# DallinClark/RealTimeRaytracer

Hardware: AMD Instinct MI355X
Metric: Mrays/sec at 1920x1080 1spp (all rays: primary + shadow) (higher is better)
Workload: dtype f32

## Files before the change

### realtimeraytracer_amd/csrc/kernels/rtr_device.h

```cpp
#pragma once
#include <hip/hip_runtime.h>
#include <stdint.h>
#include "../../../include/rtr_types.h"
#include "../../../include/rtr_math.h"

namespace rtrdev {

struct DeviceTexture { const uint8_t* pixels; uint32_t width, height, channels, _pad; };

constexpr uint32_t kLightTriRecord = 4;

struct DeviceScene {
    const uint4* nodes;
    const RtrBvhGrid* grid;
    const uint4* nodes4;
    uint32_t numNodes4;
    const float4* tris;
    const RtrVertex* vertices;
    const uint32_t* indices;
    const RtrObjectInfo* objects;
    const RtrAreaLightInfo* lights;
    const float4* lightTris;
    const uint32_t* lightTriFirst;
    const float* xforms;
// ... 243 lines not shown
                        if (ALPHA && (__float_as_uint(q2.w) & 1u) && !alpha_pass<STATS>(sc, cu, pr, u, v, st)) continue;
                        bool take;
                        if (FLAT_TAKE) {
                            const bool idLess = (cu < best.custom) | ((cu == best.custom) & (pr < best.prim));
                            take = !found | (t < best.t) | ((t == best.t) & idLess);
                        } else if (!found) take = true;
                        else take = t < best.t || (t == best.t && (cu < best.custom || (cu == best.custom && pr < best.prim)));
                        if (take) {
                            found = true; best.t = t; best.u = u; best.v = v; best.custom = cu; best.prim = pr; best.leaf = cur;
                            limit = t;
                            if (ANY) return true;
                        }
                    }
                }
            }
        }
        if (sp == 0) break;
        --sp; cur = stack[sp * BLOCK];
    }
    if (LIMIT > 0 && over) { best.custom = RTR_STACK_OVERFLOW; best.prim = RTR_MISS; best.t = tmax; best.u = 0.f; best.v = 0.f; best.leaf = 0; return false; }
    return found;
}

#define RTR_PI_F 3.14159265359f
__device__ __forceinline__ float chiGGX(float v) { return v > 0.0f ? 1.0f : 0.0f; }
__device__ __forceinline__ float GGX_Distribution(rtr_v3 n, rtr_v3 h, float alpha) {
    const float NoH = rtr_dot(n, h);
    const float alpha2 = alpha * alpha;
    const float NoH2 = NoH * NoH;
    const float den = rtr_max(rtr_fma(NoH2, alpha2, 1.0f - NoH2), 0.001f);
    return (chiGGX(NoH) * alpha2) / (RTR_PI_F * den * den);
}
__device__ __forceinline__ float GGX_PartialGeometryTerm(rtr_v3 v, rtr_v3 n, rtr_v3 h, float alpha) {
    float VoH2 = rtr_clamp(rtr_dot(v, h), 0.001f, 1.0f);
    const float chi = chiGGX(VoH2 / rtr_clamp(rtr_dot(v, n), 0.001f, 1.0f));
    VoH2 = VoH2 * VoH2;
    const float tan2 = (1.0f - VoH2) / VoH2;
    return (chi * 2.0f) / (1.0f + rtr_sqrt(rtr_fma(alpha * alpha, tan2, 1.0f)));
}
__device__ __forceinline__ rtr_v3 Fresnel_Schlick(float cosT, rtr_v3 F0) {
    const float p = rtr_pow(1.0f - cosT, 5.0f);
    return rtr_mk(rtr_fma(1.0f - F0.x, p, F0.x), rtr_fma(1.0f - F0.y, p, F0.y), rtr_fma(1.0f - F0.z, p, F0.z));
}

#define RTR_LUT_SIZE 64.0f
#define RTR_LUT_SCALE ((RTR_LUT_SIZE - 1.0f) / RTR_LUT_SIZE)
#define RTR_LUT_BIAS (0.5f / RTR_LUT_SIZE)

__device__ __forceinline__ float4 sample_lut(const float* __restrict__ lut, float u, float v) {
    float x = rtr_fma(u, RTR_LUT_SIZE, -0.5f), y = rtr_fma(v, RTR_LUT_SIZE, -0.5f);
    if (!(x >= -1.0e6f && x <= 1.0e6f)) x = 0.0f;
    if (!(y >= -1.0e6f && y <= 1.0e6f)) y = 0.0f;
    const float x0f = __builtin_floorf(x), y0f = __builtin_floorf(y);
    const float fx = x - x0f, fy = y - y0f;
    const int x0 = ((int)x0f) & 63, y0 = ((int)y0f) & 63;
    const int x1 = (x0 + 1) & 63, y1 = (y0 + 1) & 63;
    const float4 t00 = *reinterpret_cast<const float4*>(lut + (y0 * 64 + x0) * 4);
    const float4 t10 = *reinterpret_cast<const float4*>(lut + (y0 * 64 + x1) * 4);
    const float4 t01 = *reinterpret_cast<const float4*>(lut + (y1 * 64 + x0) * 4);
    const float4 t11 = *reinterpret_cast<const float4*>(lut + (y1 * 64 + x1) * 4);
    float4 r;
    { const float a = rtr_fma(t10.x - t00.x, fx, t00.x), b = rtr_fma(t11.x - t01.x, fx, t01.x); r.x = rtr_fma(b - a, fy, a); }
    { const float a = rtr_fma(t10.y - t00.y, fx, t00.y), b = rtr_fma(t11.y - t01.y, fx, t01.y); r.y = rtr_fma(b - a, fy, a); }
    { const float a = rtr_fma(t10.z - t00.z, fx, t00.z), b = rtr_fma(t11.z - t01.z, fx, t01.z); r.z = rtr_fma(b - a, fy, a); }
    { const float a = rtr_fma(t10.w - t00.w, fx, t00.w), b = rtr_fma(t11.w - t01.w, fx, t01.w); r.w = rtr_fma(b - a, fy, a); }
    return r;
}

__device__ __forceinline__ rtr_v3 IntegrateEdgeVec(rtr_v3 v1, rtr_v3 v2) {
    const float x = rtr_dot(v1, v2);
    const float y = rtr_abs(x);
    const float a = rtr_fma(rtr_fma(0.0145206f, y, 0.4965155f), y, 0.8543985f);
    const float b = rtr_fma(4.1616724f + y, y, 3.4175940f);
    const float v = a / b;
    const float theta_sintheta = (x > 0.0f) ? v : 0.5f * (1.0f / rtr_sqrt(rtr_max(rtr_fma(-x, x, 1.0f), 1e-7f))) - v;
    return rtr_scale(rtr_cross(v1, v2), theta_sintheta);
}

__device__ __forceinline__ float LTC_Evaluate(rtr_v3 N, rtr_v3 V, rtr_v3 P, bool identity, float4 t1,
                                              const rtr_v3* points, rtr_v3 lightNormal, bool twoSided,
                                              const float* __restrict__ ltc2) {
    const rtr_v3 T1 = rtr_normalize(rtr_sub(V, rtr_scale(N, rtr_dot(V, N))));
    const rtr_v3 T2 = rtr_cross(N, T1);
    rtr_v3 L[3];
#pragma unroll
    for (int k = 0; k < 3; ++k) {
        const rtr_v3 w = rtr_sub(points[k], P);
        const rtr_v3 q = rtr_mk(rtr_dot(T1, w), rtr_dot(T2, w), rtr_dot(N, w));
        rtr_v3 l;
        if (identity) l = q;
        else l = rtr_mk(rtr_fma(t1.z, q.z, t1.x * q.x), q.y, rtr_fma(t1.w, q.z, t1.y * q.x));
        L[k] = rtr_normalize(l);
    }
    const rtr_v3 dir = rtr_sub(points[0], P);
    const bool behind = rtr_dot(dir, lightNormal) < 0.0f;
    rtr_v3 vsum = IntegrateEdgeVec(L[0], L[1]);
    vsum = rtr_add(vsum, IntegrateEdgeVec(L[1], L[2]));
    vsum = rtr_add(vsum, IntegrateEdgeVec(L[2], L[0]));
    const float len = rtr_length(vsum);
    float z = vsum.z / len;
    if (behind) z = -z;
    const float uvx = rtr_fma(rtr_fma(z, 0.5f, 0.5f), RTR_LUT_SCALE, RTR_LUT_BIAS);
    const float uvy = rtr_fma(len, RTR_LUT_SCALE, RTR_LUT_BIAS);
    const float4 tex = sample_lut(ltc2, uvx, uvy);
    float sum = len * tex.w;
    if (!behind && !twoSided) sum = 0.0f;
    return sum;
}

struct RenderArgs {
    RtrCameraData cam;
    RtrSceneInfo info;
    uint32_t width, height;
    uint32_t spp, numShadowRays;
    uint32_t bandRows, shardIndex, shardCount;
    uint32_t localRows;
    uint32_t tilesPerRow;
    uint32_t maxRaysPerSample;
    uint32_t images;
    uint32_t accumulate, accumulatedFrames;
    uint32_t directRows;
};

__device__ __forceinline__ bool pixel_of(const RenderArgs& ra, uint32_t q, uint32_t& x, uint32_t& lrow, uint32_t& gy) {
    const uint32_t lane = q & 63u, tile = q >> 6;
    const uint32_t tx = tile % ra.tilesPerRow, band8 = tile / ra.tilesPerRow;
    x = tx * 8u + (lane & 7u);
    lrow = band8 * 8u + (lane >> 3);
    const uint32_t lb = lrow / ra.bandRows, r = lrow % ra.bandRows;
    gy = (lb * ra.shardCount + ra.shardIndex) * ra.bandRows + r;
    return x < ra.width && lrow < ra.localRows && gy < ra.height;
}

__device__ __forceinline__ size_t out_index(const RenderArgs& ra, uint32_t px, uint32_t lrow, uint32_t gy) {
    return (size_t)(ra.directRows ? gy : lrow) * ra.width + px;
}

__device__ __forceinline__ rtr_v3 primary_dir(const RenderArgs& ra, uint32_t px, uint32_t py, uint32_t i) {
    const float jx = rtr_random(px + i), jy = rtr_random(px + i * 322u);
    const float offx = ((float)px + jx) - 0.5f, offy = ((float)py + jy) - 0.5f;
    const rtr_v3 pw = rtr_madd(rtr_madd(rtr_ld3(ra.cam.topLeftViewportCorner), rtr_ld3(ra.cam.horizontalViewportDelta), offx),
                               rtr_ld3(ra.cam.verticalViewportDelta), offy);
    return rtr_normalize(rtr_sub(pw, rtr_ld3(ra.cam.position)));
}

struct Accum { rtr_v3 analytic, shadowed, unshadowed, avgNormal, avgPosition; };

struct Surface {
    rtr_v3 hitPoint, hitNormal, viewDir, color, mDiffuse, mSpecular;
    float roughness, metallic, om;
    float4 t1, t2;
};

template <bool SHADE, bool STATS>
__device__ __forceinline__ bool fetch_surface(const DeviceScene& sc, const RenderArgs& ra, const HitRec& h, rtr_v3 rayDir,
                                              bool wantAnalytic, Accum& o, Surface& sf, LocalStats& st) {
    if (h.custom == RTR_MISS) {
        if (SHADE) {
            rtr_v3 sky = rtr_ld3(sc.skyLinear);
            if (sc.hdri.pixels) {
                const rtr_v3 dir = rtr_normalize(rayDir);
                const float hu = rtr_atan2(dir.z, dir.x) / (2.0f * 3.14159265f) + 0.5f;
                float hv = rtr_acos(rtr_clamp(dir.y, -1.0f, 1.0f)) / 3.14159265f;
                hv = 1.0f - hv;
                const float4 tx = sample_tex<STATS>(sc.hdri, hu, hv, st);
                sky = rtr_mk(rtr_to_linear(tx.x), rtr_to_linear(tx.y), rtr_to_linear(tx.z));
            }
            o.analytic = rtr_add(o.analytic, sky); o.unshadowed = rtr_add(o.unshadowed, sky); o.shadowed = rtr_add(o.shadowed, sky);
        }
        return false;
    }
    if (h.custom < sc.numLights) {
        if (SHADE) {
            const rtr_v3 lc = rtr_ld3(sc.lights[h.custom].color);
            o.analytic = rtr_add(o.analytic, lc); o.unshadowed = rtr_add(o.unshadowed, lc); o.shadowed = rtr_add(o.shadowed, lc);
        }
        return false;
    }
    const rtr_v3 camPos = rtr_ld3(ra.cam.position);
    if (STATS) st.hits++;
    const RtrObjectInfo* oi = sc.objects + (h.custom - sc.numLights);
    const uint32_t vOff = oi->vertexOffset, iOff = oi->indexOffset;
    const uint32_t i0 = sc.indices[3u * h.prim + 0u + iOff];
    const uint32_t i1 = sc.indices[3u * h.prim + 1u + iOff];
    const uint32_t i2 = sc.indices[3u * h.prim + 2u + iOff];
    const float4* va = reinterpret_cast<const float4*>(sc.vertices + (i0 + vOff));
    const float4* vb = reinterpret_cast<const float4*>(sc.vertices + (i1 + vOff));
    const float4* vc = reinterpret_cast<const float4*>(sc.vertices + (i2 + vOff));
    const rtr_v3 p0 = f4xyz(va[0]), p1 = f4xyz(vb[0]), p2 = f4xyz(vc[0]);
    const rtr_v3 n0 = f4xyz(va[1]), n1 = f4xyz(vb[1]), n2 = f4xyz(vc[1]);
    const float b0 = 1.0f - h.u - h.v, b1 = h.u, b2 = h.v;
    const rtr_v3 localPos = rtr_madd(rtr_madd(rtr_scale(p0, b0), p1, b1), p2, b2);
    const rtr_v3 hitPoint = rtr_xform_point34(sc.xforms + 12u * h.custom, localPos);
    const rtr_v3 nsum = rtr_madd(rtr_madd(rtr_scale(n0, b0), n1, b1), n2, b2);
    const float* nm = sc.nmats + 12u * h.custom;
    rtr_v3 hitNormal;
    if (rtr_dot(nsum, nsum) > 0.0f) {
        hitNormal = rtr_normalize(rtr_mul33(nm, rtr_normalize(nsum)));
    } else {
        const rtr_v3 g = rtr_cross(rtr_sub(p1, p0), rtr_sub(p2, p0));
        rtr_v3 n = rtr_normalize(rtr_mul33(nm, rtr_normalize(g)));
        if (rtr_dot(n, rayDir) > 0.0f) n = rtr_neg(n);
        hitNormal = n;
    }
    float metallic = oi->metallic;
    float rough = oi->specular;
    rtr_v3 color = rtr_mk(0, 0, 0);
    if (SHADE) {
        rtr_v3 col = rtr_ld3(oi->color);
        if (oi->usesColorMap | oi->usesSpecularMap | oi->usesMetallicMap) {
            const float4 ta = va[2], tb = vb[2], tc = vc[2];
            const float uu = rtr_fma(tc.x, b2, rtr_fma(tb.x, b1, ta.x * b0));
            const float vv = rtr_fma(tc.y, b2, rtr_fma(tb.y, b1, ta.y * b0));
            if (oi->usesColorMap != 0u) { const float4 t = sample_tex<STATS>(sc.textures[oi->colorIndex], uu, vv, st); col = rtr_mk(t.x, t.y, t.z); }
            if (oi->usesSpecularMap != 0u) rough = sample_tex<STATS>(sc.textures[oi->specularIndex], uu, vv, st).x;
            if (oi->usesMetallicMap != 0u) metallic = sample_tex<STATS>(sc.textures[oi->metallicIndex], uu, vv, st).x;
        }
        color = rtr_mk(rtr_to_linear(col.x), rtr_to_linear(col.y), rtr_to_linear(col.z));
    }
    const float roughness = 1.0f - rough;

    const rtr_v3 viewDir = rtr_normalize(rtr_sub(camPos, hitPoint));
    const float om = 1.0f - metallic;
    rtr_v3 mDiffuse = rtr_mk(0, 0, 0), mSpecular = rtr_mk(0, 0, 0);
    float4 t1 = make_float4(1, 0, 0, 1), t2 = make_float4(0, 0, 0, 0);
    if (SHADE) {
        o.avgNormal = rtr_add(o.avgNormal, hitNormal);
        o.avgPosition = rtr_add(o.avgPosition, hitPoint);
        mDiffuse = rtr_scale(color, om);
        mSpecular = rtr_mk(rtr_fma(color.x, metallic, 0.04f * om), rtr_fma(color.y, metallic, 0.04f * om),
                           rtr_fma(color.z, metallic, 0.04f * om));
        if (wantAnalytic) {
            const float dotNV = rtr_clamp(rtr_dot(hitNormal, viewDir), 0.0f, 1.0f);
            const float lu = rtr_fma(roughness, RTR_LUT_SCALE, RTR_LUT_BIAS);
            const float lv = rtr_fma(rtr_sqrt(1.0f - dotNV), RTR_LUT_SCALE, RTR_LUT_BIAS);
            t1 = sample_lut(sc.ltc1, lu, lv);
            t2 = sample_lut(sc.ltc2, lu, lv);
        }
    }
    sf.hitPoint = hitPoint; sf.hitNormal = hitNormal; sf.viewDir = viewDir; sf.color = color;
    sf.mDiffuse = mDiffuse; sf.mSpecular = mSpecular; sf.roughness = roughness; sf.metallic = metallic; sf.om = om;
    sf.t1 = t1; sf.t2 = t2;
    return true;
}

__device__ __forceinline__ rtr_v3 surface_diffuse(float om, rtr_v3 color) {
    return rtr_mk((om * color.x) / RTR_PI_F, (om * color.y) / RTR_PI_F, (om * color.z) / RTR_PI_F);
}
__device__ __forceinline__ rtr_v3 area_sample_contrib(rtr_v3 hitNormal, rtr_v3 viewDir, float roughness, rtr_v3 mSpecular, rtr_v3 currDiffuse,
                                                      rtr_v3 lcol, float lintensity, float pdf, rtr_v3 sampledLightDir, float lightDistance) {
    const rtr_v3 halfVector = rtr_normalize(rtr_add(viewDir, sampledLightDir));
    const float cosTheta = rtr_clamp(rtr_dot(viewDir, halfVector), 0.0f, 1.0f);
    const float Dg = GGX_Distribution(hitNormal, halfVector, roughness);
    const float G = GGX_PartialGeometryTerm(viewDir, hitNormal, halfVector, roughness) *
                    GGX_PartialGeometryTerm(sampledLightDir, hitNormal, halfVector, roughness);
    const rtr_v3 F = Fresnel_Schlick(cosTheta, mSpecular);
    const float NdotV = rtr_max(rtr_dot(hitNormal, viewDir), 0.1f);
    const float NdotL = rtr_max(rtr_dot(hitNormal, sampledLightDir), 0.1f);
    const float den = 4.0f * NdotV * NdotL;
    const rtr_v3 currSpecular = rtr_mk(((Dg * F.x) * G) / den, ((Dg * F.y) * G) / den, ((Dg * F.z) * G) / den);
    const float attenuation = 1.0f / (lightDistance * lightDistance);
    const rtr_v3 BRDF = rtr_add(currSpecular, currDiffuse);
    const rtr_v3 Lr = rtr_mk((((lcol.x * lintensity) * NdotL) * attenuation) * 10.0f, (((lcol.y * lintensity) * NdotL) * attenuation) * 10.0f,
                             (((lcol.z * lintensity) * NdotL) * attenuation) * 10.0f);
    return rtr_mk((BRDF.x * Lr.x) / pdf, (BRDF.y * Lr.y) / pdf, (BRDF.z * Lr.z) / pdf);
}
__device__ __forceinline__ rtr_v3 directional_light_dir() { return rtr_normalize(rtr_mk(-1.0f, 1.0f, -0.5f)); }
__device__ __forceinline__ rtr_v3 directional_contrib(rtr_v3 hitNormal, rtr_v3 viewDir, float roughness, rtr_v3 mSpecular, rtr_v3 currDiffuse) {
    const rtr_v3 directLightDir = directional_light_dir();
    const rtr_v3 directLightColor = rtr_mk(1.0f, 1.0f, 0.5f);
    const float directLightIntensity = 0.2f;
    const rtr_v3 halfVector = rtr_normalize(rtr_add(viewDir, directLightDir));
    const float cosTheta = rtr_clamp(rtr_dot(viewDir, halfVector), 0.0f, 1.0f);
    const float Dg = GGX_Distribution(hitNormal, halfVector, roughness);
    const float G = GGX_PartialGeometryTerm(viewDir, hitNormal, halfVector, roughness) *
                    GGX_PartialGeometryTerm(directLightDir, hitNormal, halfVector, roughness);
    const rtr_v3 F = Fresnel_Schlick(cosTheta, mSpecular);
    const float NdotV = rtr_max(rtr_dot(hitNormal, viewDir), 5.0f);
    const float NdotL = rtr_max(rtr_dot(hitNormal, directLightDir), 0.0001f);
    const float den = 4.0f * NdotV * NdotL;
    const rtr_v3 currSpecular = rtr_mk(((Dg * F.x) * G) / den, ((Dg * F.y) * G) / den, ((Dg * F.z) * G) / den);
    const rtr_v3 BRDF = rtr_add(currSpecular, currDiffuse);
    const rtr_v3 Lr = rtr_mk(((directLightColor.x * directLightIntensity) * NdotL) * 20.0f, ((directLightColor.y * directLightIntensity) * NdotL) * 20.0f,
                             ((directLightColor.z * directLightIntensity) * NdotL) * 20.0f);
    return rtr_mul(BRDF, Lr);
}
struct SamplePair { float r1, r2; };
__device__ __forceinline__ uint32_t light_sample_seed0(uint32_t px, uint32_t py, uint32_t frame) { return px * 733u + py * 1933u + frame; }
__device__ __forceinline__ SamplePair light_sample_pair(uint32_t seed) {
    float r1 = rtr_random(seed), r2 = rtr_random(seed + 100u);
    if (r1 + r2 > 1.0f) { r1 = 1.0f - r1; r2 = 1.0f - r2; }
    return SamplePair{r1, r2};
}
__device__ __forceinline__ rtr_v3 light_sample_at(const rtr_v3* P, SamplePair r) {
    return rtr_madd(rtr_madd(P[0], rtr_sub(P[1], P[0]), r.r1), rtr_sub(P[2], P[0]), r.r2);
}
__device__ __forceinline__ rtr_v3 light_sample_pos(const rtr_v3* P, uint32_t s, uint32_t px, uint32_t py, uint32_t frame) {
    return light_sample_at(P, light_sample_pair(s + light_sample_seed0(px, py, frame)));
}
struct DrawnSamples {
    uint32_t px, py, frame;
    __device__ __forceinline__ SamplePair pair(uint32_t s) const { return light_sample_pair(s + light_sample_seed0(px, py, frame)); }
};

constexpr uint32_t kDirectionalSlot = 0xffffffffu;
#ifndef RTR_INTO_EXPR
#define RTR_INTO_EXPR (rtr_dot(hitNormal, lightVec) < 0.0f)
#endif
template <class Policy, bool STATS, class Samples>
__device__ __forceinline__ void light_loops_from(const DeviceScene& sc, const RenderArgs& ra, const Samples& smp,
                                                 const Surface& sf, uint32_t want, Accum& o, Policy& pol, LocalStats& st) {
    const bool wantAnalytic = (want & 1u) != 0u, wantUnshadowed = (want & 2u) != 0u;
    const rtr_v3 hitPoint = sf.hitPoint, hitNormal = sf.hitNormal, viewDir = sf.viewDir, color = sf.color;
    const rtr_v3 mDiffuse = sf.mDiffuse, mSpecular = sf.mSpecular;
    const float roughness = sf.roughness, om = sf.om;
    const float4 t1 = sf.t1, t2 = sf.t2;
    const rtr_v3 shadowOrigin = rtr_madd(hitPoint, hitNormal, 0.01f);
    const rtr_v3 currDiffuse = surface_diffuse(om, color);

    for (uint32_t li = 0; li < ra.info.numAreaLights; ++li) {
        const RtrAreaLightInfo* L = sc.lights + li;
        if (STATS) st.lightFetch++;
        const rtr_v3 lcol = rtr_ld3(L->color);
        const float lintensity = L->intensity;
        const uint32_t lnt = L->numTriangles;
        const bool twoSided = L->isTwoSided != 0u;
        for (uint32_t ti = 0; ti < lnt; ++ti) {
            if (STATS) st.lightTriFetch++;
            const float4* rec = sc.lightTris + (size_t)(sc.lightTriFirst[li] + ti) * kLightTriRecord;
            const float4 r0 = rec[0], r1 = rec[1], r2 = rec[2], r3 = rec[3];
            rtr_v3 P[3];
            P[0] = rtr_mk(r0.x, r0.y, r0.z); P[1] = rtr_mk(r1.x, r1.y, r1.z); P[2] = rtr_mk(r2.x, r2.y, r2.z);
            const float pdf = r1.w;
            const rtr_v3 lightNormal = rtr_mk(r3.x, r3.y, r3.z);
            if (!twoSided) {
                if (rtr_dot(lightNormal, rtr_sub(hitPoint, P[0])) < 0.0f) continue;
            }
            rtr_v3 shadowedSample = rtr_mk(0, 0, 0), unshadowedSample = rtr_mk(0, 0, 0);
            pol.slots_at((sc.lightTriFirst[li] + ti) * ra.numShadowRays);
            for (uint32_t s = 0; s < ra.numShadowRays; ++s) {
                const rtr_v3 lightSamplePos = light_sample_at(P, smp.pair(s));
                const rtr_v3 lightVec = rtr_sub(lightSamplePos, hitPoint);
                const rtr_v3 sampledLightDir = rtr_normalize(lightVec);
                const float lightDistance = rtr_length(lightVec);
                const bool occ = pol.occluded(shadowOrigin, sampledLightDir, lightDistance - 0.5f, lightVec, RTR_INTO_EXPR);
                if (Policy::kShade && (wantUnshadowed || !occ)) {
                    const float currShadow = occ ? 0.0f : 1.0f;
                    const rtr_v3 contrib = area_sample_contrib(hitNormal, viewDir, roughness, mSpecular, currDiffuse, lcol, lintensity, pdf, sampledLightDir, lightDistance);
                    shadowedSample = rtr_madd(shadowedSample, contrib, currShadow);
                    unshadowedSample = rtr_add(unshadowedSample, contrib);
                }
            }
            if (Policy::kShade) {
                const float ns = (float)ra.numShadowRays;
                shadowedSample = rtr_mk(shadowedSample.x / ns, shadowedSample.y / ns, shadowedSample.z / ns);
                unshadowedSample = rtr_mk(unshadowedSample.x / ns, unshadowedSample.y / ns, unshadowedSample.z / ns);
                if (wantAnalytic) {
                    const float diffuse = LTC_Evaluate(hitNormal, viewDir, hitPoint, true, t1, P, lightNormal, twoSided, sc.ltc2);
                    const float spec = LTC_Evaluate(hitNormal, viewDir, hitPoint, false, t1, P, lightNormal, twoSided, sc.ltc2);
                    const rtr_v3 fres = rtr_mk(rtr_fma(1.0f - mSpecular.x, t2.y, mSpecular.x * t2.x),
                                               rtr_fma(1.0f - mSpecular.y, t2.y, mSpecular.y * t2.x),
                                               rtr_fma(1.0f - mSpecular.z, t2.y, mSpecular.z * t2.x));
                    o.analytic = rtr_add(o.analytic, rtr_mk(((lcol.x * lintensity) * rtr_fma(mDiffuse.x, diffuse, spec * fres.x)) * 5.0f,
                                                            ((lcol.y * lintensity) * rtr_fma(mDiffuse.y, diffuse, spec * fres.y)) * 5.0f,
                                                            ((lcol.z * lintensity) * rtr_fma(mDiffuse.z, diffuse, spec * fres.z)) * 5.0f));
                }
                o.shadowed = rtr_add(o.shadowed, shadowedSample);
                o.unshadowed = rtr_add(o.unshadowed, unshadowedSample);
            }
        }
    }
    const rtr_v3 directLightDir = directional_light_dir();
    if (rtr_dot(hitNormal, directLightDir) <= 0.0f) return;
    pol.slots_at(kDirectionalSlot);
    const bool occ = pol.occluded(shadowOrigin, directLightDir, 10000.0f, directLightDir, false);
    if (Policy::kShade && (wantUnshadowed || wantAnalytic || !occ)) {
        const float currShadow = occ ? 0.0f : 1.0f;
        const rtr_v3 contrib = directional_contrib(hitNormal, viewDir, roughness, mSpecular, currDiffuse);
        o.shadowed = rtr_madd(o.shadowed, contrib, currShadow);
        o.unshadowed = rtr_add(o.unshadowed, contrib);
        o.analytic = rtr_add(o.analytic, contrib);
    }
}
template <class Policy, bool STATS>
__device__ __forceinline__ void light_loops(const DeviceScene& sc, const RenderArgs& ra, uint32_t px, uint32_t py,
                                            const Surface& sf, uint32_t want, Accum& o, Policy& pol, LocalStats& st) {
    light_loops_from<Policy, STATS>(sc, ra, DrawnSamples{px, py, ra.info.frame}, sf, want, o, pol, st);
}

__device__ __forceinline__ void light_tri_record(const RtrAreaLightInfo* L, const RtrVertex* vertices, const uint32_t* indices,
                                                 uint32_t ti, float4* rec) {
    const uint32_t lvOff = L->vertexOffset, liOff = L->indexOffset;
    const uint32_t j0 = indices[ti * 3u + 0u + liOff];
    const uint32_t j1 = indices[ti * 3u + 1u + liOff];
    const uint32_t j2 = indices[ti * 3u + 2u + liOff];
    rtr_v3 P[3];
// ... 89 lines not shown
```

### realtimeraytracer_amd/csrc/kernels/rtr_kernels.h

```cpp
#pragma once
#include <hip/hip_runtime.h>
#include "rtr_device.h"

namespace rtrdev {

#ifndef RTR_SHADOW_FAR_FIRST
#define RTR_SHADOW_FAR_FIRST 1
#endif
#if RTR_SHADOW_FAR_FIRST
#define RTR_ANYHIT_KERNEL_REVISION "r05.3"
#else
#define RTR_ANYHIT_KERNEL_REVISION "r05.3-nearest-first"
#endif

constexpr uint32_t kQueueRegions = 8;
constexpr uint32_t kQueueLenWord = 0;
constexpr uint32_t kPrimaryRedoWord = 2;
constexpr uint32_t kOccludedWord = 3;
constexpr uint32_t kBatchCursorWord = 16;
static_assert(kOccludedWord < kBatchCursorWord && kPrimaryRedoWord < kOccludedWord, "the small counters sit below the first batch cursor");
constexpr uint32_t kQueueLists = kQueueRegions * kQueueRegions;
constexpr uint32_t kQueueListLens = kBatchCursorWord + 16 * kQueueLists;
constexpr uint32_t kPrimaryCursors = kQueueListLens + kQueueLists;
constexpr uint32_t kQueueCtrlWords = kPrimaryCursors + 16 * kQueueRegions;
static_assert(kQueueLists == 64, "k_shadow_gen_oct reserves the batch lists with one lane per list");

constexpr size_t kSpillInts = (size_t)64 * 64 * 256;

struct RayQueue {
    float4*   dt = nullptr;
    uint32_t* slot = nullptr;
    float4*   origin = nullptr;
    uint32_t  slotStride = 0;
    uint32_t  slotMask = 0;
    uint32_t  ownLeaf = 0;
};


struct Workspace {
    float4*   hitTuvp = nullptr;
    uint32_t* hitCustom = nullptr;
    RayQueue  rayQueue;
    uint8_t*  vis = nullptr;
    uint32_t  visFill = 1;
    size_t    visPlaneBytes = 0;
    uint32_t  visPlanes = 0;
    uint32_t* queueCount = nullptr;
    uint2*    batchLists = nullptr;
    uint32_t  listStride = 0;
    uint32_t* overflow = nullptr;
    uint32_t  overflowCap = 0;
    unsigned long long* clk = nullptr;
    int32_t*  spill = nullptr;
    size_t    capPixelSamples = 0;
    size_t    capRays = 0;
};

struct Tunables {
    uint32_t primary_packet = 0;
    uint32_t primary_wide = 0;
    uint32_t primary_persist = 0;
    uint32_t primary_persist_min_rays = 6u << 20;
    uint32_t primary_batch = 64, primary_refill = 24, primary_inner_min = 20, primary_wgs_per_cu = 8;
    uint32_t trace_bvh4 = 1;
    uint32_t trace_batch = 0;
    uint32_t trace_binned = 2;
    uint32_t queue_nt = 1;
    uint32_t trace_wgs_per_cu = 0;
    uint32_t trace_refill = 20, trace_inner_min = 28;
    uint32_t trace_octant_forms = 1;
    uint32_t trace_own_leaf = 1;
    uint32_t trace_top_nodes = 0xffffffffu;
    uint32_t resolve_row_waves = 0;
    uint32_t resolve_compact = 1;
    uint32_t split_priorities = 0;
};
Tunables tunables_from_env();
bool tunable_set(Tunables& t, const char* name, uint32_t value);
bool tunable_get(const Tunables& t, const char* name, uint32_t* value);

hipError_t launch_megakernel(const DeviceScene& sc, const RenderArgs& ra, const FrameOut& fo, int stackEntries,
                             Counters* stats, hipStream_t stream);

hipError_t launch_wavefront(const DeviceScene& sc, const FrameBatch& batch, const Workspace& ws, const Tunables& tun,
                            int stackEntries, Counters* stats, hipStream_t stream, hipEvent_t* ev, uint32_t numCus);

struct OcclusionArgs {
    const float4* rays;
    uint8_t* occluded;
    uint32_t n;
    uint32_t batch;
    uint32_t* ctrl;
    uint32_t* overflow;
    uint32_t overflowCap;
    uint32_t* queue;
    uint2* lists;
    uint32_t listStride;
    const int32_t* startLeaves;
    uint32_t numTris;
};
struct RayMaskArgs {
    const uint8_t* rayMasks = nullptr;
    uint32_t cullMask = 0xffu;
    uint32_t masked = 0;
};
hipError_t launch_occlusion_walk(const DeviceScene& sc, const OcclusionArgs& oa, const Tunables& tun, bool alpha, Counters* stats, hipStream_t stream, uint32_t numCus,
                                 const RayMaskArgs& rm = RayMaskArgs());

hipError_t launch_light_tris(const RtrAreaLightInfo* lights, const RtrVertex* vertices, const uint32_t* indices, const uint32_t* first,
                             uint32_t numLights, float4* out, hipStream_t stream);
hipError_t launch_deinterleave(const uint32_t* gathered, uint32_t* dst, uint32_t width, uint32_t height,
                               uint32_t bandRows, uint32_t shardCount, uint32_t localRows, hipStream_t stream);

}
```

### realtimeraytracer_amd/csrc/kernels/rtr_kernels.hip

```cpp
#include "rtr_kernels.h"

#include <algorithm>
#include <cstdlib>
#include <cstring>

namespace rtrdev {

constexpr int kBlock = 256;

template <bool STATS, int STACK>
struct InlinePolicy {
    static constexpr bool kShade = true;
    __device__ __forceinline__ void slots_at(uint32_t) {}
    const DeviceScene& sc; int32_t* stack; LocalStats& st;
    __device__ __forceinline__ bool occluded(rtr_v3 o, rtr_v3 d, float tmax, rtr_v3, bool) {
        HitRec h;
        return trace<true, STATS, kBlock>(sc, stack, o, d, 0.001f, tmax, h, st);
    }
};

__device__ __forceinline__ uint32_t wave_sum_u32(uint32_t v) {
#pragma unroll
    for (int o = 32; o > 0; o >>= 1) v += __shfl_xor(v, o);
    return v;
}
typedef float rtr_f4 __attribute__((ext_vector_type(4)));
constexpr uint32_t kRayIntoSurface = 0x80000000u;
__device__ __forceinline__ void queue_load(const RayQueue& q, uint32_t ray, rtr_v3& o, rtr_v3& d, float& tmax, uint32_t& slot, uint32_t nt) {
    float4 a;
    if (nt) {
        const rtr_f4 x = __builtin_nontemporal_load(reinterpret_cast<const rtr_f4*>(q.dt + ray));
        a = make_float4(x.x, x.y, x.z, x.w);
        slot = __builtin_nontemporal_load(q.slot + ray);
    } else { a = q.dt[ray]; slot = q.slot[ray]; }
    slot &= ~kRayIntoSurface;
    const float4 og = q.origin[slot & q.slotMask];
    o = rtr_mk(og.x, og.y, og.z); d = rtr_mk(a.x, a.y, a.z); tmax = a.w;
}
__device__ __forceinline__ void queue_store_origin(const RayQueue& q, size_t k, rtr_v3 hitPoint, rtr_v3 hitNormal) {
    const rtr_v3 o = rtr_madd(hitPoint, hitNormal, 0.01f);
    float* p = reinterpret_cast<float*>(q.origin + k);
    p[0] = o.x; p[1] = o.y; p[2] = o.z;
}
__device__ __forceinline__ void origin_leaf_store(float4* rayOrigin, size_t k, int32_t leaf) { reinterpret_cast<int32_t*>(rayOrigin + k)[3] = leaf; }
__device__ __forceinline__ void queue_store(const RayQueue& q, size_t idx, rtr_v3 d, float tmax, uint32_t slot, uint32_t nt, bool into) {
    const uint32_t word = slot | ((into && q.ownLeaf) ? kRayIntoSurface : 0u);
    if (nt) {
        __builtin_nontemporal_store(rtr_f4{d.x, d.y, d.z, tmax}, reinterpret_cast<rtr_f4*>(q.dt + idx));
        __builtin_nontemporal_store(word, q.slot + idx);
    } else { q.dt[idx] = make_float4(d.x, d.y, d.z, tmax); q.slot[idx] = word; }
}

struct CountPolicy {
    static constexpr bool kShade = false;
    __device__ __forceinline__ void slots_at(uint32_t) {}
    uint32_t n;
    __device__ __forceinline__ bool occluded(rtr_v3, rtr_v3, float, rtr_v3, bool) { ++n; return false; }
};

struct EmitPolicy {
    static constexpr bool kShade = false;
    __device__ __forceinline__ void slots_at(uint32_t) {}
    typedef volatile __attribute__((address_space(3))) uint32_t* lds_word;
    RayQueue queue; lds_word waveOffset; uint32_t base; uint32_t slot;
    __device__ __forceinline__ bool occluded(rtr_v3, rtr_v3 d, float tmax, rtr_v3, bool into) {
        const unsigned long long m = __ballot(1);
        const uint32_t prefix = __builtin_amdgcn_mbcnt_hi((uint32_t)(m >> 32), __builtin_amdgcn_mbcnt_lo((uint32_t)m, 0u));
        const uint32_t off = *waveOffset;
        if (prefix == 0) *waveOffset = off + (uint32_t)__popcll(m);
        queue_store(queue, (size_t)(base + off + prefix), d, tmax, slot, 0u, into);
        slot += queue.slotStride;
        return false;
    }
};

__device__ __forceinline__ uint32_t vis_mask32(const uint8_t* __restrict__ vis, uint32_t slot, uint32_t slotStride, uint32_t queries) {
    uint32_t m = 0;
    const uint32_t n = queries < 32u ? queries : 32u;
    for (uint32_t j0 = 0; j0 < n; j0 += 8u) {
        uint32_t b[8];
#pragma unroll
        for (uint32_t j = 0; j < 8u; ++j) { const uint32_t jj = j0 + j < n ? j0 + j : n - 1u; b[j] = vis[slot + jj * slotStride]; }
#pragma unroll
        for (uint32_t j = 0; j < 8u; ++j) m |= (b[j] != 0u && j0 + j < n ? 1u : 0u) << (j0 + j);
    }
    return m;
}

struct LookupPolicy {
    static constexpr bool kShade = true;
    __device__ __forceinline__ void slots_at(uint32_t) {}
    const uint8_t* vis; uint32_t slot, slotStride;
    uint32_t mask, j;
    __device__ __forceinline__ bool occluded(rtr_v3, rtr_v3, float, rtr_v3, bool) {
        const bool occ = j < 32u ? ((mask >> j) & 1u) != 0u : vis[slot] != 0;
        slot += slotStride; ++j;
        return occ;
    }
};

__device__ __forceinline__ uint32_t raw_octant(rtr_v3 r) {
    return (r.x < 0.f ? 1u : 0u) | (r.y < 0.f ? 2u : 0u) | (r.z < 0.f ? 4u : 0u);
}

struct CountOctPolicy {
    static constexpr bool kShade = false;
    __device__ __forceinline__ void slots_at(uint32_t) {}
    unsigned long long lo, hi;
    __device__ __forceinline__ void add(uint32_t oct, uint32_t n) {
        const unsigned long long v = (unsigned long long)n << ((oct & 3u) * 16u);
        if (oct < 4u) lo += v; else hi += v;
    }
    __device__ __forceinline__ bool occluded(rtr_v3, rtr_v3, float, rtr_v3 raw, bool) { add(raw_octant(raw), 1u); return false; }
};

struct EmitOctPolicy {
    static constexpr bool kShade = false;
    __device__ __forceinline__ void slots_at(uint32_t) {}
    typedef volatile __attribute__((address_space(3))) uint32_t* lds_word;
    RayQueue queue; lds_word run; uint32_t slot, nt;
    __device__ __forceinline__ bool occluded(rtr_v3, rtr_v3 d, float tmax, rtr_v3 raw, bool into) {
        const uint32_t oct = raw_octant(raw);
        unsigned long long rem = __ballot(1);
        while (rem != 0ull) {
            const uint32_t oo = (uint32_t)__builtin_amdgcn_readlane((int)oct, (int)__ffsll((long long)rem) - 1);
            const unsigned long long mo = __ballot(oct == oo);
            if (oct == oo) {
                const uint32_t prefix = __builtin_amdgcn_mbcnt_hi((uint32_t)(mo >> 32), __builtin_amdgcn_mbcnt_lo((uint32_t)mo, 0u));
                const uint32_t pos = run[oo];
                if (prefix == 0) run[oo] = pos + (uint32_t)__popcll(mo);
                queue_store(queue, (size_t)(pos + prefix), d, tmax, slot, nt, into);
            }
            rem &= ~mo;
        }
        slot += queue.slotStride;
        return false;
    }
};

__device__ __forceinline__ Accum zero_accum() {
    Accum a;
    a.analytic = a.shadowed = a.unshadowed = a.avgNormal = a.avgPosition = rtr_mk(0, 0, 0);
    return a;
}

template <int STACK, bool STATS>
__global__ __launch_bounds__(kBlock) void k_megakernel(DeviceScene sc, RenderArgs ra, FrameOut fo, Counters* stats) {
    __shared__ int32_t s_stack[STACK * kBlock];
    int32_t* stack = s_stack + threadIdx.x;
    const uint32_t q = blockIdx.x * kBlock + threadIdx.x;
    uint32_t px, lrow, py;
    if (!pixel_of(ra, q, px, lrow, py)) return;
    LocalStats st;
    Accum acc = zero_accum();
    const uint32_t want = (fo.img[0] != nullptr ? 1u : 0u) | (fo.img[2] != nullptr ? 2u : 0u);
    const rtr_v3 camPos = rtr_ld3(ra.cam.position);
    InlinePolicy<STATS, STACK> pol{sc, stack, st};
    for (uint32_t i = 0; i < ra.spp; ++i) {
        const rtr_v3 dir = primary_dir(ra, px, py, i);
        HitRec h;
        trace<false, STATS, kBlock>(sc, stack, camPos, dir, 0.001f, 10000.0f, h, st);
        shade_sample<InlinePolicy<STATS, STACK>, STATS>(sc, ra, px, py, h, dir, want, acc, pol, st);
    }
    write_pixel(ra, fo, out_index(ra, px, lrow, py), acc);
    if (STATS) st.flush(stats);
}

#ifndef RTR_PRIMARY_BLOCK
#define RTR_PRIMARY_BLOCK 64
#endif
constexpr int kPrimBlock = RTR_PRIMARY_BLOCK;
static_assert(kPrimBlock % 64 == 0 && kPrimBlock >= 64 && kPrimBlock <= kBlock && kBlock % kPrimBlock == 0,
              "RTR_PRIMARY_BLOCK: a multiple of 64 that divides the 256-lane tile group (the launcher's grid is blocks * (kBlock / kPrimBlock))");
template <int STACK, bool STATS>
__global__ __launch_bounds__(kPrimBlock) void k_primary(DeviceScene sc, FrameBatch fb, float4* hitTuvp, uint32_t* hitCustom, float4* rayOrigin,
                                                    Counters* stats, uint32_t* redoCount, uint32_t* redoList, uint32_t planeBlocks) {
    __shared__ int32_t s_stack[16 * kPrimBlock];
    int32_t* stack = s_stack + threadIdx.x;
    const uint32_t plane = blockIdx.x / planeBlocks;
    const RenderArgs& ra = fb.ra[plane / fb.ra[0].spp];
    const uint32_t i = plane % fb.ra[0].spp;
    const uint32_t q = (blockIdx.x - plane * planeBlocks) * kPrimBlock + threadIdx.x;
    uint32_t px, lrow, py;
    if (!pixel_of(ra, q, px, lrow, py)) return;
    LocalStats st;
    const rtr_v3 camPos = rtr_ld3(ra.cam.position);
    const rtr_v3 dir = primary_dir(ra, px, py, i);
    HitRec h;
    if (STATS) trace<false, true, kPrimBlock, 16, 8>(sc, stack, camPos, dir, 0.001f, 10000.0f, h, st);
    else {
        const uint32_t oct = ray_octant(sc, camPos, dir);
        const uint32_t woct = (uint32_t)__builtin_amdgcn_readfirstlane((int)oct);
        switch (__ballot(oct != woct) != 0ull ? 8u : woct) {
            case 0: trace<false, false, kPrimBlock, 16, 0>(sc, stack, camPos, dir, 0.001f, 10000.0f, h, st); break;
            case 1: trace<false, false, kPrimBlock, 16, 1>(sc, stack, camPos, dir, 0.001f, 10000.0f, h, st); break;
            case 2: trace<false, false, kPrimBlock, 16, 2>(sc, stack, camPos, dir, 0.001f, 10000.0f, h, st); break;
            case 3: trace<false, false, kPrimBlock, 16, 3>(sc, stack, camPos, dir, 0.001f, 10000.0f, h, st); break;
            case 4: trace<false, false, kPrimBlock, 16, 4>(sc, stack, camPos, dir, 0.001f, 10000.0f, h, st); break;
            case 5: trace<false, false, kPrimBlock, 16, 5>(sc, stack, camPos, dir, 0.001f, 10000.0f, h, st); break;
            case 6: trace<false, false, kPrimBlock, 16, 6>(sc, stack, camPos, dir, 0.001f, 10000.0f, h, st); break;
            case 7: trace<false, false, kPrimBlock, 16, 7>(sc, stack, camPos, dir, 0.001f, 10000.0f, h, st); break;
            default: trace<false, false, kPrimBlock, 16, 8>(sc, stack, camPos, dir, 0.001f, 10000.0f, h, st); break;
        }
    }
    const size_t k = (size_t)plane * planeBlocks * kPrimBlock + q;
    if (h.custom == RTR_STACK_OVERFLOW) redoList[atomicAdd(redoCount, 1u)] = (uint32_t)k;
    else {
        hitTuvp[k] = make_float4(h.t, h.u, h.v, __uint_as_float(h.prim));
        hitCustom[k] = h.custom;
        origin_leaf_store(rayOrigin, k, h.leaf);
    }
    if (STATS) st.flush(stats);
}

template <bool STATS>
__global__ __launch_bounds__(kBlock) void k_primary_packet(DeviceScene sc, FrameBatch fb, float4* hitTuvp, uint32_t* hitCustom, float4* rayOrigin, Counters* stats, uint32_t planeBlocks) {
    __shared__ uint4 s_stack[kBlock / 64][64];
    const uint32_t wave = threadIdx.x >> 6, lane = threadIdx.x & 63u;
    const uint32_t plane = blockIdx.x / planeBlocks;
    const RenderArgs& ra = fb.ra[plane / fb.ra[0].spp];
    const uint32_t i = plane % fb.ra[0].spp;
    const uint32_t q = (blockIdx.x - plane * planeBlocks) * kBlock + threadIdx.x;
    uint32_t px = 0, lrow = 0, py = 0;
    const bool valid = pixel_of(ra, q, px, lrow, py);
    unsigned long long active = __ballot(valid);
    if (active == 0ull) return;
    LocalStats st;
    const rtr_v3 o = rtr_ld3(ra.cam.position);
    const rtr_v3 d = valid ? primary_dir(ra, px, py, i) : rtr_mk(0.f, 0.f, 1.f);
    const float tmin = 0.001f, tmax = 10000.0f;
    if (STATS && valid) { st.rays++; st.primary++; }
    const rtr_v3 idir = rtr_mk(rtr_safe_rcp_dir(d.x), rtr_safe_rcp_dir(d.y), rtr_safe_rcp_dir(d.z));
    rtr_v3 ga, gb;
    rtr_ray_grid(o, idir, sc.grid->origin, sc.grid->scale, &ga, &gb);
    HitRec best; best.t = tmax; best.u = 0.f; best.v = 0.f; best.custom = RTR_MISS; best.prim = RTR_MISS; best.leaf = 0;
    const uint4* __restrict__ nodes = sc.nodes;
    const float4* __restrict__ tris = sc.tris;
    uint32_t sp = 0;
    int32_t cur = 0;
    for (;;) {
        const bool mine = ((active >> lane) & 1ull) != 0ull;
        bool pop = true;
        if (cur >= 0) {
            const uint4 a = nodes[2 * cur], b = nodes[2 * cur + 1];
            if (STATS && mine) st.nodes++;
            float tl = 0.f, tr = 0.f;
            const bool hl = mine && slab_pair(a.x, a.y, b.x, ga, gb, tmin, best.t, tl);
            const bool hr = mine && slab_pair(a.z, a.w, b.y, ga, gb, tmin, best.t, tr);
            const unsigned long long mL = __ballot(hl), mR = __ballot(hr);
            if ((mL | mR) != 0ull) {
                pop = false;
                if (mR == 0ull) { cur = (int32_t)b.z; active = mL; }
                else if (mL == 0ull) { cur = (int32_t)b.w; active = mR; }
                else {
                    const uint32_t rNear = (uint32_t)__popcll(__ballot(hl && hr && tr < tl)), lNear = (uint32_t)__popcll(__ballot(hl && hr && !(tr < tl)));
                    const bool rFirst = rNear > lNear;
                    if (lane == 0u) {
                        const unsigned long long m2 = rFirst ? mL : mR;
                        s_stack[wave][sp] = make_uint4(rFirst ? b.z : b.w, (uint32_t)m2, (uint32_t)(m2 >> 32), 0u);
                    }
                    ++sp;
                    cur = (int32_t)(rFirst ? b.w : b.z); active = rFirst ? mR : mL;
                }
            }
        } else {
            const uint32_t code = (uint32_t)~cur;
            const uint32_t first = code >> 3, cnt = (code & 7u) + 1u;
            for (uint32_t k = 0; k < cnt; ++k) {
                const float4 q0 = tris[3u * (first + k)], q1 = tris[3u * (first + k) + 1u], q2 = tris[3u * (first + k) + 2u];
                if (mine) {
                    if (STATS) st.tris++;
                    float t, u, v;
                    if (rtr_mt_intersect(o, d, f4xyz(q0), f4xyz(q1), f4xyz(q2), tmin, &t, &u, &v) && t < tmax) {
                        const uint32_t cu = __float_as_uint(q0.w), pr = __float_as_uint(q1.w);
                        if (!(__float_as_uint(q2.w) & 1u) || alpha_pass<STATS>(sc, cu, pr, u, v, st)) {
                            if (t < best.t || (t == best.t && (cu < best.custom || (cu == best.custom && pr < best.prim)))) {
                                best.t = t; best.u = u; best.v = v; best.custom = cu; best.prim = pr; best.leaf = cur;
                            }
                        }
                    }
                }
            }
        }
        if (pop) {
            if (sp == 0u) break;
            --sp;
            const uint4 e = s_stack[wave][sp];
            cur = __builtin_amdgcn_readfirstlane((int32_t)e.x);
            active = (unsigned long long)(uint32_t)__builtin_amdgcn_readfirstlane((int)e.y) | ((unsigned long long)(uint32_t)__builtin_amdgcn_readfirstlane((int)e.z) << 32);
        }
    }
    if (valid) {
        const size_t k = (size_t)plane * planeBlocks * kBlock + q;
        hitTuvp[k] = make_float4(best.t, best.u, best.v, __uint_as_float(best.prim));
        hitCustom[k] = best.custom;
        origin_leaf_store(rayOrigin, k, best.leaf);
    }
    if (STATS) st.flush(stats);
}

template <bool STATS>
__global__ __launch_bounds__(kBlock) void k_primary_tail(DeviceScene sc, FrameBatch fb, float4* hitTuvp, uint32_t* hitCustom, float4* rayOrigin,
                                                         const uint32_t* __restrict__ redoCount, const uint32_t* __restrict__ redoList,
                                                         int32_t* __restrict__ spill, uint32_t planeStride, Counters* stats) {
    const uint32_t n = *redoCount;
    if (n == 0) return;
    int32_t* stack = spill + blockIdx.x * kBlock + threadIdx.x;
    LocalStats st;
    for (uint32_t j = blockIdx.x * kBlock + threadIdx.x; j < n; j += gridDim.x * kBlock) {
        const uint32_t k = redoList[j];
        const uint32_t plane = k / planeStride, q = k % planeStride;
        const RenderArgs& ra = fb.ra[plane / fb.ra[0].spp];
        const uint32_t i = plane % fb.ra[0].spp;
        uint32_t px, lrow, py;
        if (!pixel_of(ra, q, px, lrow, py)) continue;
        HitRec h;
        trace<false, STATS, 64 * kBlock>(sc, stack, rtr_ld3(ra.cam.position), primary_dir(ra, px, py, i), 0.001f, 10000.0f, h, st);
        if (STATS) { st.rays--; st.primary--; }
        hitTuvp[k] = make_float4(h.t, h.u, h.v, __uint_as_float(h.prim));
        hitCustom[k] = h.custom;
        origin_leaf_store(rayOrigin, k, h.leaf);
    }
    if (STATS) st.flush(stats);
}

__device__ __forceinline__ uint32_t wave_sum(uint32_t v) {
#pragma unroll
    for (int o = 32; o > 0; o >>= 1) v += __shfl_xor(v, o);
    return v;
}
__device__ __forceinline__ uint32_t wave_total(uint32_t v) {
    v += (uint32_t)__builtin_amdgcn_update_dpp(0, (int)v, 0xB1, 0xf, 0xf, false);
    v += (uint32_t)__builtin_amdgcn_update_dpp(0, (int)v, 0x4E, 0xf, 0xf, false);
    v += (uint32_t)__builtin_amdgcn_update_dpp(0, (int)v, 0x141, 0xf, 0xf, false);
    v += (uint32_t)__builtin_amdgcn_update_dpp(0, (int)v, 0x140, 0xf, 0xf, false);
    v += (uint32_t)__builtin_amdgcn_update_dpp(0, (int)v, 0x142, 0xa, 0xf, false);
    v += (uint32_t)__builtin_amdgcn_update_dpp(0, (int)v, 0x143, 0xc, 0xf, false);
    return (uint32_t)__builtin_amdgcn_readlane((int)v, 63);
}

constexpr uint32_t kParkedPairs = 4;
typedef __attribute__((address_space(3))) uint32_t* lds_column;
template <uint32_t BLOCK>
struct ParkedSamples {
    lds_column pairs;
    uint32_t seed0;
    bool parked;
    __device__ __forceinline__ void draw(uint32_t ns) const {
        if (!parked) return;
        for (uint32_t s = 0; s < ns; ++s) {
            const SamplePair r = light_sample_pair(s + seed0);
            pairs[2u * s * BLOCK] = __float_as_uint(r.r1); pairs[(2u * s + 1u) * BLOCK] = __float_as_uint(r.r2);
        }
    }
    __device__ __forceinline__ SamplePair pair(uint32_t s) const {
        if (parked) return SamplePair{__uint_as_float(pairs[2u * s * BLOCK]), __uint_as_float(pairs[(2u * s + 1u) * BLOCK])};
        return light_sample_pair(s + seed0);
    }
};

constexpr uint32_t kGenBlock = 1024;
__global__ __launch_bounds__(kGenBlock) void k_shadow_gen(DeviceScene sc, FrameBatch fb, const float4* hitTuvp,
                                                          const uint32_t* hitCustom, RayQueue queue, uint32_t* count, uint32_t planeStride) {
    __shared__ uint32_t s_off[kGenBlock / 64], s_tot[kGenBlock / 64], s_base;
    __shared__ uint32_t s_pairs[2u * kParkedPairs * kGenBlock];
    uint32_t q;
    const uint32_t frame = batch_frame(blockIdx.x * kGenBlock + threadIdx.x, planeStride, q);
    const RenderArgs& ra = fb.ra[frame < fb.n ? frame : 0u];
    const size_t plane0 = (size_t)frame * ra.spp;
    const uint32_t wave = threadIdx.x >> 6;
    uint32_t px = 0, lrow = 0, py = 0;
    const bool live = frame < fb.n && pixel_of(ra, q, px, lrow, py);
    LocalStats st;
    Accum acc = zero_accum();
    const bool single = ra.spp == 1u;
    Surface sf0;
    bool surf0 = false;
    uint32_t n = 0;
    const ParkedSamples<kGenBlock> smp{(lds_column)&s_pairs[threadIdx.x], light_sample_seed0(px, py, ra.info.frame), ra.numShadowRays <= kParkedPairs};
    if (live) {
        CountPolicy cp{0};
        smp.draw(ra.numShadowRays);
        for (uint32_t i = 0; i < ra.spp; ++i) {
            const size_t k = (plane0 + i) * planeStride + q;
            const float4 r = hitTuvp[k];
            HitRec h; h.t = r.x; h.u = r.y; h.v = r.z; h.prim = __float_as_uint(r.w); h.custom = hitCustom[k];
            Surface sf;
            const bool surf = fetch_surface<false, false>(sc, ra, h, primary_dir(ra, px, py, i), false, acc, sf, st);
            if (surf) light_loops_from<CountPolicy, false>(sc, ra, smp, sf, 0u, acc, cp, st);
            if (i == 0) { sf0 = sf; surf0 = surf; }
        }
        n = cp.n;
    }
    const uint32_t total = wave_sum(n);
    if ((threadIdx.x & 63u) == 0) { s_tot[wave] = total; s_off[wave] = 0; }
    __syncthreads();
    if (threadIdx.x == 0) {
        uint32_t t = 0;
        for (uint32_t w = 0; w < kGenBlock / 64; ++w) t += s_tot[w];
        s_base = t ? atomicAdd(count, t) : 0u;
    }
    __syncthreads();
    uint32_t base = s_base;
    for (uint32_t w = 0; w < wave; ++w) base += s_tot[w];
    if (!live || n == 0) return;
    for (uint32_t i = 0; i < ra.spp; ++i) {
        const size_t k = (plane0 + i) * planeStride + q;
        EmitPolicy pol{queue, (EmitPolicy::lds_word)&s_off[wave], base, (uint32_t)k};
        if (single) {
            if (surf0) { queue_store_origin(queue, k, sf0.hitPoint, sf0.hitNormal); light_loops_from<EmitPolicy, false>(sc, ra, smp, sf0, 0u, acc, pol, st); }
        } else {
            const float4 r = hitTuvp[k];
            HitRec h; h.t = r.x; h.u = r.y; h.v = r.z; h.prim = __float_as_uint(r.w); h.custom = hitCustom[k];
            Surface sf;
            if (fetch_surface<false, false>(sc, ra, h, primary_dir(ra, px, py, i), false, acc, sf, st)) {
                queue_store_origin(queue, k, sf.hitPoint, sf.hitNormal);
                light_loops_from<EmitPolicy, false>(sc, ra, smp, sf, 0u, acc, pol, st);
            }
        }
    }
}

constexpr size_t kBinnedMinRays = (size_t)10 << 20;
constexpr uint32_t kBinnedMinNodes = 1u << 16;
#ifndef RTR_GEN_OCT_BLOCK
#define RTR_GEN_OCT_BLOCK 512
#endif
constexpr uint32_t kGenOctBlock = RTR_GEN_OCT_BLOCK;
constexpr uint32_t kParkSurface = 6, kParkWords = kParkSurface + 2u * kParkedPairs;
#ifndef RTR_GEN_OCT_WAVES
#define RTR_GEN_OCT_WAVES 7
#endif
#if RTR_GEN_OCT_WAVES > 0
#define RTR_GEN_OCT_ATTR __attribute__((amdgpu_waves_per_eu(RTR_GEN_OCT_WAVES, 8)))
#else
#define RTR_GEN_OCT_ATTR
#endif
__global__ __launch_bounds__(kGenOctBlock) RTR_GEN_OCT_ATTR void k_shadow_gen_oct(DeviceScene sc, FrameBatch fb, const float4* hitTuvp, const uint32_t* hitCustom,
                                                              RayQueue queue, uint32_t* ctrl, uint32_t planeStride, uint2* lists,
                                                              uint32_t listStride, uint32_t kBatch, uint32_t nt) {
    constexpr uint32_t kWaves = kGenOctBlock / 64;
    __shared__ uint32_t s_tot[kWaves][8], s_run[kWaves][8];
    __shared__ uint32_t s_park[kParkWords * kGenOctBlock];
    uint32_t q;
    const uint32_t frame = batch_frame(blockIdx.x * kGenOctBlock + threadIdx.x, planeStride, q);
    const RenderArgs& ra = fb.ra[frame < fb.n ? frame : 0u];
    const size_t plane0 = (size_t)frame * ra.spp;
    const uint32_t wave = threadIdx.x >> 6;
    uint32_t px = 0, lrow = 0, py = 0;
    const bool live = frame < fb.n && pixel_of(ra, q, px, lrow, py);
    LocalStats st;
    Accum acc = zero_accum();
    const bool single = ra.spp == 1u;
    const lds_column park = (lds_column)&s_park[threadIdx.x];
    const ParkedSamples<kGenOctBlock> smp{park + kParkSurface * kGenOctBlock, light_sample_seed0(px, py, ra.info.frame), ra.numShadowRays <= kParkedPairs};
    CountOctPolicy cp{0ull, 0ull};
    if (live) {
        smp.draw(ra.numShadowRays);
        for (uint32_t i = 0; i < ra.spp; ++i) {
            const size_t k = (plane0 + i) * planeStride + q;
            const float4 r = hitTuvp[k];
            HitRec h; h.t = r.x; h.u = r.y; h.v = r.z; h.prim = __float_as_uint(r.w); h.custom = hitCustom[k];
            Surface sf;
            bool surf = fetch_surface<false, false>(sc, ra, h, primary_dir(ra, px, py, i), false, acc, sf, st);
#if RTR_EXP_DOUBLE_FETCH_GEN
            if (surf) {
                HitRec h2 = h; h2.u = h.u + sf.hitPoint.x * (float)(ra.spp - 1u) * 1.0e-30f; h2.v = h.v + sf.hitNormal.y * (float)(ra.spp - 1u) * 1.0e-30f;
                h2.prim = h.prim + (__float_as_uint(sf.hitPoint.z) == 0x7fc12345u ? 1u : 0u);
                Surface sf2;
                if (fetch_surface<false, false>(sc, ra, h2, primary_dir(ra, px, py, i), false, acc, sf2, st)) sf = sf2;
            }
#endif
            if (surf) {
                if (single) {
                    park[0u * kGenOctBlock] = __float_as_uint(sf.hitPoint.x); park[1u * kGenOctBlock] = __float_as_uint(sf.hitPoint.y); park[2u * kGenOctBlock] = __float_as_uint(sf.hitPoint.z);
                    park[3u * kGenOctBlock] = __float_as_uint(sf.hitNormal.x); park[4u * kGenOctBlock] = __float_as_uint(sf.hitNormal.y); park[5u * kGenOctBlock] = __float_as_uint(sf.hitNormal.z);
                }
                light_loops_from<CountOctPolicy, false>(sc, ra, smp, sf, 0u, acc, cp, st);
            }
        }
    }
    uint32_t mine = 0;
#pragma unroll
    for (uint32_t o = 0; o < 8; ++o) {
        const uint32_t c = (uint32_t)(((o < 4 ? cp.lo : cp.hi) >> ((o & 3u) * 16u)) & 0xffffull);
        mine += c;
        const uint32_t t = wave_total(c);
        if ((threadIdx.x & 63u) == 0) s_tot[wave][o] = t;
    }
    __syncthreads();
    if (threadIdx.x < kQueueLists) {
        const uint32_t o = threadIdx.x / kQueueRegions, x = threadIdx.x % kQueueRegions;
        uint32_t before = 0, len = 0, total = 0;
        uint32_t tot[8] = {0u, 0u, 0u, 0u, 0u, 0u, 0u, 0u};
#pragma unroll
        for (uint32_t w0 = 0; w0 < kWaves; w0 += 4u) {
#pragma unroll
            for (uint32_t w = w0; w < w0 + 4u && w < kWaves; ++w) {
#pragma unroll
                for (uint32_t oo = 0; oo < 8; ++oo) tot[oo] += s_tot[w][oo];
            }
            asm volatile("" : "+v"(tot[0]), "+v"(tot[1]), "+v"(tot[2]), "+v"(tot[3]), "+v"(tot[4]), "+v"(tot[5]), "+v"(tot[6]), "+v"(tot[7]) : : "memory");
        }
#pragma unroll
        for (uint32_t oo = 0; oo < 8; ++oo) {
            before += oo < o ? tot[oo] : 0u;
            len = oo == o ? tot[oo] : len;
            total += tot[oo];
        }
        const uint32_t kB = (kBatch >= 512u && blockIdx.x * 8u >= gridDim.x * 7u) ? kBatch / 2u : kBatch;
        const uint32_t nb = (len + kB - 1) / kB;
        const uint32_t b0 = (x + kQueueRegions - blockIdx.x % kQueueRegions) % kQueueRegions;
        const uint32_t cnt = b0 < nb ? (nb - b0 + kQueueRegions - 1) / kQueueRegions : 0u;
        uint32_t at = 0, pos = 0;
        if (threadIdx.x == 0 && total) at = atomicAdd(ctrl, total);
        if (cnt) pos = atomicAdd(ctrl + kQueueListLens + threadIdx.x, cnt);
        const uint32_t first = (uint32_t)__builtin_amdgcn_readfirstlane((int)at) + before;
        if (x == 0) {
            uint32_t c = first;
            for (uint32_t w = 0; w < kWaves; ++w) { s_run[w][o] = c; c += s_tot[w][o]; }
        }
        for (uint32_t j = 0; j < cnt; ++j) {
            const uint32_t f = (b0 + j * kQueueRegions) * kB;
            lists[(size_t)threadIdx.x * listStride + pos + j] = make_uint2(first + f, len - f < kB ? len - f : kB);
        }
    }
    __syncthreads();
    if (mine == 0) return;
    for (uint32_t i = 0; i < ra.spp; ++i) {
        const size_t k = (plane0 + i) * planeStride + q;
        EmitOctPolicy pol{queue, (EmitOctPolicy::lds_word)&s_run[wave][0], (uint32_t)k, nt};
        if (single) {
            Surface sf0 = {};
            sf0.hitPoint = rtr_mk(__uint_as_float(park[0u * kGenOctBlock]), __uint_as_float(park[1u * kGenOctBlock]), __uint_as_float(park[2u * kGenOctBlock]));
            sf0.hitNormal = rtr_mk(__uint_as_float(park[3u * kGenOctBlock]), __uint_as_float(park[4u * kGenOctBlock]), __uint_as_float(park[5u * kGenOctBlock]));
            queue_store_origin(queue, k, sf0.hitPoint, sf0.hitNormal);
            light_loops_from<EmitOctPolicy, false>(sc, ra, smp, sf0, 0u, acc, pol, st);
        } else {
            const float4 r = hitTuvp[k];
            HitRec h; h.t = r.x; h.u = r.y; h.v = r.z; h.prim = __float_as_uint(r.w); h.custom = hitCustom[k];
            Surface sf;
            if (fetch_surface<false, false>(sc, ra, h, primary_dir(ra, px, py, i), false, acc, sf, st)) {
                queue_store_origin(queue, k, sf.hitPoint, sf.hitNormal);
                light_loops_from<EmitOctPolicy, false>(sc, ra, smp, sf, 0u, acc, pol, st);
            }
        }
    }
}

#ifndef RTR_REFILL_LDS
#define RTR_REFILL_LDS 1
#endif
#ifndef RTR_LIST_SHARE
#define RTR_LIST_SHARE 1
#endif
constexpr int kTailBlocks = 64;
constexpr int32_t kDone = (int32_t)0x80000000;
constexpr int32_t kAbandoned = (int32_t)0x80000001;
constexpr uint32_t kBatchDefault = 256, kBatchLong = 512;
constexpr size_t kBatchLongQueue = (size_t)100 << 20;

constexpr uint32_t kResNone = 3u;
#ifndef RTR_TRACE_BLOCK
#define RTR_TRACE_BLOCK 256
#endif
constexpr int kTraceBlock = RTR_TRACE_BLOCK;
#ifndef RTR_TRI_AUX
#define RTR_TRI_AUX 0
#endif
#ifndef RTR_NODE_AUX
#define RTR_NODE_AUX 0
#endif
#ifndef RTR_SHADOW_STACK
#define RTR_SHADOW_STACK RTR_WIDE_STACK
#endif
#ifndef RTR_TRACE_TOP
#define RTR_TRACE_TOP 40
#endif
constexpr uint32_t kTopNodes = (uint32_t)RTR_TRACE_TOP * (RTR_TRACE_BLOCK / 256);

template <int STACK>
__global__ __launch_bounds__(kBlock) void k_shadow_trace(DeviceScene sc, const RayQueue queue,
                                                              const uint32_t* __restrict__ count, uint32_t* nextBatch,
                                                              uint8_t* __restrict__ vis, uint32_t visFill, uint32_t kBatch, uint32_t kRefill,
                                                              uint32_t kInnerMin, uint32_t* overflow, uint32_t overflowCap) {
    __shared__ int32_t s_stack[(STACK + 1) * kBlock];
    int32_t* lds = s_stack + threadIdx.x;
    lds[0] = kDone;
    const uint32_t n = *count;
    uint32_t batchPos = 0, batchEnd = 0;
    bool exhausted = false;
    const uint32_t regionLen = ((n + kQueueRegions - 1) / kQueueRegions + kBatch - 1) / kBatch * kBatch;
    const uint32_t myRegion = blockIdx.x % kQueueRegions;
    uint32_t regionTry = 0;
    int32_t cur = kDone;
    int sp = 0;
    rtr_v3 o = rtr_mk(0, 0, 0), d = rtr_mk(0, 0, 0), ga = rtr_mk(0, 0, 0), gb = rtr_mk(0, 0, 0);
    float tmax = 0.f;
    uint32_t slot = 0, rayIndex = 0, res = kResNone, occ = 0;
    const float tmin = 0.001f;
    typedef uint32_t u32x4 __attribute__((ext_vector_type(4)));
    const __amdgpu_buffer_rsrc_t nodeBuf = __builtin_amdgcn_make_buffer_rsrc((void*)sc.nodes, 0, 0xffffffff, 0x00020000);
    const __amdgpu_buffer_rsrc_t triBuf = __builtin_amdgcn_make_buffer_rsrc((void*)sc.tris, 0, 0xffffffff, 0x00020000);

    for (;;) {
        const unsigned long long idle = __ballot(cur == kDone);
        const uint32_t nIdle = (uint32_t)__popcll(idle);
        if (nIdle >= kRefill || nIdle == 64u) {
            if (cur == kDone && res != kResNone) {
                if (res == 2u) { const uint32_t at = atomicAdd(overflow, 1u); if (at < overflowCap) overflow[1u + at] = rayIndex; }
                else { if (res != visFill) vis[slot] = (uint8_t)res; occ += res; }
                res = kResNone;
            }
            if (!exhausted) {
                if (batchPos == batchEnd) {
                    for (;;) {
                        if (regionTry >= kQueueRegions) { exhausted = true; break; }
                        const uint32_t r = (myRegion + regionTry) % kQueueRegions;
                        const uint32_t lo = r * regionLen;
                        uint32_t hi = lo + regionLen; if (hi > n) hi = n;
                        uint32_t b = hi;
                        if (lo < hi) {
                            uint32_t got = 0;
                            if ((threadIdx.x & 63u) == 0) got = atomicAdd(nextBatch + 16u * r, kBatch);
                            got = (uint32_t)__builtin_amdgcn_readfirstlane((int)got);
                            b = got < regionLen ? lo + got : hi;
                        }
                        if (b < hi) { batchPos = b; batchEnd = (b + kBatch < hi) ? b + kBatch : hi; break; }
                        ++regionTry;
                    }
                }
                if (!exhausted) {
                    const uint32_t avail = batchEnd - batchPos;
                    const uint32_t prefix = __builtin_amdgcn_mbcnt_hi((uint32_t)(idle >> 32), __builtin_amdgcn_mbcnt_lo((uint32_t)idle, 0u));
                    if (cur == kDone && prefix < avail) {
                        rayIndex = batchPos + prefix;
                        queue_load(queue, rayIndex, o, d, tmax, slot, 0u);
                        if (!(tmax > tmin)) {
                            if (visFill != 0u) vis[slot] = 0;
                        } else {
                            const rtr_v3 idir = rtr_mk(rtr_safe_rcp_dir(d.x), rtr_safe_rcp_dir(d.y), rtr_safe_rcp_dir(d.z));
                            rtr_ray_grid(o, idir, sc.grid->origin, sc.grid->scale, &ga, &gb);
                            cur = 0; sp = 0; res = 0u;
                        }
                    }
                    batchPos += (nIdle < avail) ? nIdle : avail;
                }
            }
        }
        if (__ballot(cur != kDone) == 0ull) {
            if (exhausted) break;
            continue;
        }
        for (;;) {
            const unsigned long long innerMask = __ballot(cur >= 0);
            if (innerMask == 0ull) break;
            if ((uint32_t)__popcll(innerMask) <= kInnerMin && __ballot(cur < 0 && cur != kDone) != 0ull) break;
            if (cur >= 0) {
                const int32_t nodeOff = cur << 5;
                const u32x4 a = __builtin_amdgcn_raw_buffer_load_b128(nodeBuf, nodeOff, 0, 0);
                const u32x4 b = __builtin_amdgcn_raw_buffer_load_b128(nodeBuf, nodeOff + 16, 0, 0);
                const int32_t top = lds[sp * kBlock];
                float tl, tr;
                const bool hl = slab_pair(a.x, a.y, b.x, ga, gb, tmin, tmax, tl);
                const bool hr = slab_pair(a.z, a.w, b.y, ga, gb, tmin, tmax, tr);
                const bool swap = tr < tl;
                const int32_t c0 = (int32_t)b.z, c1 = (int32_t)b.w;
                const bool both = hl && hr, none = !(hl || hr);
                const bool second = both ? swap : !hl;
                int32_t next = second ? c1 : c0;
                const bool push = both && sp < STACK;
                if (push) { ++sp; lds[sp * kBlock] = swap ? c0 : c1; }
                if (both && !push) { res = 2u; next = kDone; }
                if (none) { next = top; --sp; }
                cur = next;
            }
        }
        if (cur < 0 && cur != kDone) {
            const uint32_t code = (uint32_t)~cur;
            const uint32_t first = code >> 3, cnt = (code & 7u) + 1u;
            bool hit = false;
            for (uint32_t i = 0; i < cnt && !hit; ++i) {
                const int32_t triOff = (int32_t)((first + i) * 48u);
                const u32x4 r0 = __builtin_amdgcn_raw_buffer_load_b128(triBuf, triOff, 0, 0);
                const u32x4 r1 = __builtin_amdgcn_raw_buffer_load_b128(triBuf, triOff + 16, 0, 0);
                const u32x4 r2 = __builtin_amdgcn_raw_buffer_load_b128(triBuf, triOff + 32, 0, 0);
                const float4 q0 = make_float4(__uint_as_float(r0.x), __uint_as_float(r0.y), __uint_as_float(r0.z), __uint_as_float(r0.w));
                const float4 q1 = make_float4(__uint_as_float(r1.x), __uint_as_float(r1.y), __uint_as_float(r1.z), __uint_as_float(r1.w));
                const float4 q2 = make_float4(__uint_as_float(r2.x), __uint_as_float(r2.y), __uint_as_float(r2.z), __uint_as_float(r2.w));
                float t, u, v;
                if (rtr_mt_intersect(o, d, f4xyz(q0), f4xyz(q1), f4xyz(q2), tmin, &t, &u, &v) && t < tmax) {
                    hit = true;
                    if (__float_as_uint(q2.w) & 1u) {
                        LocalStats st;
                        hit = alpha_pass<false>(sc, __float_as_uint(q0.w), __float_as_uint(q1.w), u, v, st);
// ... 243 lines not shown
                    }
                }
                if (!exhausted) {
                    const uint32_t avail = batchEnd - batchPos;
                    const uint32_t prefix = __builtin_amdgcn_mbcnt_hi((uint32_t)(idle >> 32), __builtin_amdgcn_mbcnt_lo((uint32_t)idle, 0u));
                    if (cur == kDone && prefix < avail) {
                        rayIndex = batchPos + prefix;
                        bool into = false;
                        int32_t ownLeaf = 0;
                        if (CALLER) {
#if RTR_REFILL_LDS
                            const global_f4 qrays = (global_f4)rc.dt;
                            const global_u32 qslot = (global_u32)rc.slot;
                            slot = (octForms & 2u) ? __builtin_nontemporal_load(qslot + rayIndex) : qslot[rayIndex];
                            const rtr_f4 a = qrays[2 * (size_t)slot], b = qrays[2 * (size_t)slot + 1];
#else
                            slot = queue.slot[rayIndex];
                            const float4 a = queue.dt[2 * (size_t)slot], b = queue.dt[2 * (size_t)slot + 1];
#endif
                            o = rtr_mk(a.x, a.y, a.z); tmin = a.w; d = rtr_mk(b.x, b.y, b.z); tmax = b.w;
                            if (HINTS) {
#if RTR_REFILL_LDS
                                const global_i32 qhint = (global_i32)rc.origin;
                                const uint32_t numTris = rc.slotMask;
                                ownLeaf = (octForms & 2u) ? __builtin_nontemporal_load(qhint + slot) : qhint[slot];
#else
                                const uint32_t numTris = queue.slotMask;
                                ownLeaf = reinterpret_cast<const int32_t*>(queue.origin)[slot];
#endif
                                const uint32_t code = (uint32_t)~ownLeaf;
                                into = ownLeaf < 0 && (code >> 3) + (code & 7u) + 1u <= numTris;
                            }
                            if (MASKED) {
                                const uint8_t* __restrict__ qmask = reinterpret_cast<const uint8_t*>(count);
                                uint32_t m = queue.slotStride & 0xffu;
                                if (qmask) m &= (uint32_t)qmask[slot];
                                rayMask8 = m << kTriMaskShift;
                            }
                        } else
#if RTR_REFILL_LDS
                        {
                            const global_f4 qdt = (global_f4)rc.dt, qorg = (global_f4)rc.origin;
                            const global_u32 qslot = (global_u32)rc.slot;
                            rtr_f4 a;
                            if (octForms & 2u) { a = __builtin_nontemporal_load(qdt + rayIndex); slot = __builtin_nontemporal_load(qslot + rayIndex); }
                            else { a = qdt[rayIndex]; slot = qslot[rayIndex]; }
                            into = (slot & kRayIntoSurface) != 0u;
                            slot &= ~kRayIntoSurface;
                            const rtr_f4 og = qorg[slot & rc.slotMask];
                            o = rtr_mk(og.x, og.y, og.z); d = rtr_mk(a.x, a.y, a.z); tmax = a.w;
                            ownLeaf = __float_as_int(og.w);
                        }
#else
                        {
                            into = (queue.slot[rayIndex] & kRayIntoSurface) != 0u;
                            queue_load(queue, rayIndex, o, d, tmax, slot, octForms & 2u);
                            ownLeaf = __float_as_int(queue.origin[slot & queue.slotMask].w);
                        }
#endif
                        if (STATS) { st.rays++; st.shadow++; }
                        if (!(tmax > tmin)) {
                            if (fill != 0u) visOut[slot] = 0;
                        } else {
                            const rtr_v3 idir = rtr_mk(rtr_safe_rcp_dir(d.x), rtr_safe_rcp_dir(d.y), rtr_safe_rcp_dir(d.z));
#if RTR_REFILL_LDS
                            rtr_ray_grid_about(o, idir, rtr_mk(rc.sx, rc.sy, rc.sz), rtr_mk(rc.cx, rc.cy, rc.cz), &ga, &gb);
#else
                            rtr_ray_grid_centre(o, idir, sc.grid->origin, sc.grid->scale, sc.grid->wideCentreXY, sc.grid->wideCentreZ, &ga, &gb);
#endif
                            cur = 0; sp = lds; res = 0u;
                            if (into) { sp = lds + kTraceBlock; *sp = 0; cur = ownLeaf; }
                        }
                    }
                    batchPos += (nIdle < avail) ? nIdle : avail;
                }
            }
        }
        if (__ballot(cur != kDone) == 0ull) {
            if (exhausted) break;
            continue;
        }
        {
            const unsigned long long innerNow = __ballot(cur >= 0);
            if (innerNow != 0ull) {
                const uint32_t oct = (ga.x < 0.f ? 1u : 0u) | (ga.y < 0.f ? 2u : 0u) | (ga.z < 0.f ? 4u : 0u);
                const uint32_t woct = (uint32_t)__builtin_amdgcn_readlane((int)oct, (int)__ffsll((long long)innerNow) - 1);
                const bool mixed = __ballot(cur >= 0 && oct != woct) != 0ull;
                switch ((mixed || (octForms & 1u) == 0u) ? 8u : woct) {
                    case 0: inner_nodes4<STACK, 0, STATS>(nodeBuf, s_top, topCount, lds, cur, sp, ga, gb, tmin, tmax, kInnerMin, ws, st); break;
                    case 1: inner_nodes4<STACK, 1, STATS>(nodeBuf, s_top, topCount, lds, cur, sp, ga, gb, tmin, tmax, kInnerMin, ws, st); break;
                    case 2: inner_nodes4<STACK, 2, STATS>(nodeBuf, s_top, topCount, lds, cur, sp, ga, gb, tmin, tmax, kInnerMin, ws, st); break;
                    case 3: inner_nodes4<STACK, 3, STATS>(nodeBuf, s_top, topCount, lds, cur, sp, ga, gb, tmin, tmax, kInnerMin, ws, st); break;
                    case 4: inner_nodes4<STACK, 4, STATS>(nodeBuf, s_top, topCount, lds, cur, sp, ga, gb, tmin, tmax, kInnerMin, ws, st); break;
                    case 5: inner_nodes4<STACK, 5, STATS>(nodeBuf, s_top, topCount, lds, cur, sp, ga, gb, tmin, tmax, kInnerMin, ws, st); break;
                    case 6: inner_nodes4<STACK, 6, STATS>(nodeBuf, s_top, topCount, lds, cur, sp, ga, gb, tmin, tmax, kInnerMin, ws, st); break;
                    case 7: inner_nodes4<STACK, 7, STATS>(nodeBuf, s_top, topCount, lds, cur, sp, ga, gb, tmin, tmax, kInnerMin, ws, st); break;
                    default: inner_nodes4<STACK, 8, STATS>(nodeBuf, s_top, topCount, lds, cur, sp, ga, gb, tmin, tmax, kInnerMin, ws, st); break;
                }
                if (cur == kAbandoned) { res = 2u; cur = kDone; }
            }
        }
        if (STATS) {
            const bool atLeaf = cur < 0 && cur != kDone;
            const uint32_t code = (uint32_t)~cur;
            const uint32_t first = code >> 3, cnt = (code & 7u) + 1u;
            bool hit = false;
#if RTR_STATS_LEAF_PHASE
            { const uint32_t pairs = wave_sum_u32(atLeaf ? cnt : 0u); ws.triIters++; ws.triLanes += pairs; if (pairs > 64u) ws.over64++; ws.leafLanes += (uint32_t)__popcll(__ballot(atLeaf)); }
#endif
            for (uint32_t i = 0;; ++i) {
                const bool go = atLeaf && i < cnt && !hit;
                const unsigned long long m = __ballot(go);
                if (m == 0ull) break;
#if !RTR_STATS_LEAF_PHASE
                ws.triIters++; ws.triLanes += (uint32_t)__popcll(m);
#endif
                if (go) { st.tris++; st.shadowTris++; hit = tri_any<true, CALLER, MASKED>(sc, triBuf, first + i, o, d, tmin, tmax, st, (octForms & 4u) != 0u, rayMask8, cull); }
            }
            if (atLeaf) {
                if (hit) { res = 1u; cur = kDone; }
                else { cur = *sp; sp -= kTraceBlock; }
            }
        } else if (cur < 0 && cur != kDone) {
            const uint32_t code = (uint32_t)~cur;
            const uint32_t first = code >> 3, cnt = (code & 7u) + 1u;
            bool hit = false;
            for (uint32_t i = 0; i < cnt && !hit; ++i) hit = tri_any<false, CALLER, MASKED>(sc, triBuf, first + i, o, d, tmin, tmax, st, (octForms & 4u) != 0u, rayMask8, cull);
            if (hit) { res = 1u; cur = kDone; }
            else { cur = *sp; sp -= kTraceBlock; }
        }
    }
    {
        const uint32_t occWave = wave_sum_u32(occ);
        if ((threadIdx.x & 63u) == 0 && occWave) atomicAdd(nextBatch - kBatchCursorWord + kOccludedWord, occWave);
    }
    if (stamp || STATS) {
        const unsigned long long c1 = __builtin_amdgcn_s_memtime(), r1 = __builtin_amdgcn_s_memrealtime();
        if (stamp) { clk[2 * blockIdx.x] = c1 - c0; clk[2 * blockIdx.x + 1] = r1 - r0; }
        if (STATS && (threadIdx.x & 63u) == 0) {
            atomicAdd(&stats->innerIters, (unsigned long long)ws.innerIters); atomicAdd(&stats->innerLanes, (unsigned long long)ws.innerLanes);
            atomicAdd(&stats->triIters, (unsigned long long)ws.triIters); atomicAdd(&stats->triLanes, (unsigned long long)ws.triLanes);
#if RTR_STATS_LEAF_PHASE
            atomicAdd(&stats->refills, (unsigned long long)ws.over64 | ((unsigned long long)ws.leafLanes << 32));
#else
            atomicAdd(&stats->refills, (unsigned long long)ws.refills);
#endif
            atomicAdd(&stats->clockCycles, c1 - c0); atomicAdd(&stats->clockRef, r1 - r0);
        }
    }
    if (STATS) st.flush(stats);
}

template <bool STATS>
__global__ __launch_bounds__(kBlock) void k_primary4(DeviceScene sc, FrameBatch fb, float4* hitTuvp, uint32_t* hitCustom, float4* rayOrigin, Counters* stats,
                                                     uint32_t* redoCount, uint32_t* redoList, uint32_t planeBlocks) {
    __shared__ int32_t s_stack[RTR_WIDE_STACK * kBlock];
    typedef uint32_t u32x4 __attribute__((ext_vector_type(4)));
    const uint32_t plane = blockIdx.x / planeBlocks;
    const RenderArgs& ra = fb.ra[plane / fb.ra[0].spp];
    const uint32_t i = plane % fb.ra[0].spp;
    const uint32_t q = (blockIdx.x - plane * planeBlocks) * kBlock + threadIdx.x;
    uint32_t px, lrow, py;
    if (!pixel_of(ra, q, px, lrow, py)) return;
    LocalStats st;
    const rtr_v3 o = rtr_ld3(ra.cam.position);
    const rtr_v3 d = primary_dir(ra, px, py, i);
    const float tmin = 0.001f, tmax = 10000.0f;
    if (STATS) { st.rays++; st.primary++; }
    const rtr_v3 idir = rtr_mk(rtr_safe_rcp_dir(d.x), rtr_safe_rcp_dir(d.y), rtr_safe_rcp_dir(d.z));
    rtr_v3 ga, gb;
    rtr_ray_grid_centre(o, idir, sc.grid->origin, sc.grid->scale, sc.grid->wideCentreXY, sc.grid->wideCentreZ, &ga, &gb);
    const __amdgpu_buffer_rsrc_t nodeBuf = __builtin_amdgcn_make_buffer_rsrc((void*)sc.nodes4, 0, 0xffffffff, 0x00020000);
    const __amdgpu_buffer_rsrc_t triBuf = __builtin_amdgcn_make_buffer_rsrc((void*)sc.tris, 0, 0xffffffff, 0x00020000);
    HitRec best; best.t = tmax; best.u = 0.f; best.v = 0.f; best.custom = RTR_MISS; best.prim = RTR_MISS; best.leaf = 0;
    int32_t* const lds = s_stack + threadIdx.x;
    int sp = 0;
    int32_t cur = 0;
    bool over = false;
    for (;;) {
        if (cur >= 0) {
            if (STATS) st.nodes++;
            const int32_t nodeOff = cur << 6;
            const u32x4 q0 = __builtin_amdgcn_raw_buffer_load_b128(nodeBuf, nodeOff, 0, 0), q1 = __builtin_amdgcn_raw_buffer_load_b128(nodeBuf, nodeOff + 16, 0, 0);
            const u32x4 q2 = __builtin_amdgcn_raw_buffer_load_b128(nodeBuf, nodeOff + 32, 0, 0), q3 = __builtin_amdgcn_raw_buffer_load_b128(nodeBuf, nodeOff + 48, 0, 0);
            const int32_t c0 = (int32_t)q3.x, c1 = (int32_t)q3.y, c2 = (int32_t)q3.z, c3 = (int32_t)q3.w;
            const float lim = rtr_hwmin(best.t, best.t);
            float t0, t1, t2, t3;
            const bool h0 = slab_wide<8>(q0.x, q0.y, q0.z, ga, gb, tmin, lim, t0);
            const bool h1 = slab_wide<8>(q0.w, q1.x, q1.y, ga, gb, tmin, lim, t1);
            const bool h2 = slab_wide<8>(q1.z, q1.w, q2.x, ga, gb, tmin, lim, t2) & (c2 != kDone);
            const bool h3 = slab_wide<8>(q2.y, q2.z, q2.w, ga, gb, tmin, lim, t3) & (c3 != kDone);
            float tn = h0 ? t0 : 3.0e38f;
            const bool e1 = h1 & (t1 < tn); tn = e1 ? t1 : tn;
            const bool e2 = h2 & (t2 < tn); tn = e2 ? t2 : tn;
            const bool e3 = h3 & (t3 < tn);
            int32_t next = e3 ? c3 : (e2 ? c2 : (e1 ? c1 : c0));
            const bool any = h0 | h1 | h2 | h3;
            const bool p0 = h0 & (e1 | e2 | e3), p1 = h1 & !(e1 & !e2 & !e3), p2 = h2 & !(e2 & !e3), p3 = h3 & !e3;
            if (p0) { if (sp < RTR_WIDE_STACK) lds[sp++ * kBlock] = c0; else over = true; }
            if (p1) { if (sp < RTR_WIDE_STACK) lds[sp++ * kBlock] = c1; else over = true; }
            if (p2) { if (sp < RTR_WIDE_STACK) lds[sp++ * kBlock] = c2; else over = true; }
            if (p3) { if (sp < RTR_WIDE_STACK) lds[sp++ * kBlock] = c3; else over = true; }
            if (over) break;
            if (any) { cur = next; continue; }
        } else {
            const uint32_t code = (uint32_t)~cur;
            const uint32_t first = code >> 3, cnt = (code & 7u) + 1u;
            for (uint32_t k = 0; k < cnt; ++k) {
                const int32_t off = (int32_t)((first + k) * 48u);
                const rtr_f4 a0 = load_f4(triBuf, off), a1 = load_f4(triBuf, off + 16), a2 = load_f4(triBuf, off + 32);
                if (STATS) st.tris++;
                float t, u, v;
                if (rtr_mt_intersect(o, d, rtr_mk(a0.x, a0.y, a0.z), rtr_mk(a1.x, a1.y, a1.z), rtr_mk(a2.x, a2.y, a2.z), tmin, &t, &u, &v) && t < tmax) {
                    const uint32_t cu = __float_as_uint(a0.w), pr = __float_as_uint(a1.w);
                    if ((__float_as_uint(a2.w) & 1u) && !alpha_pass<STATS>(sc, cu, pr, u, v, st)) continue;
                    if (t < best.t || (t == best.t && (cu < best.custom || (cu == best.custom && pr < best.prim)))) {
                        best.t = t; best.u = u; best.v = v; best.custom = cu; best.prim = pr; best.leaf = cur;
                    }
                }
            }
        }
        if (sp == 0) break;
        cur = lds[--sp * kBlock];
    }
    const size_t k = (size_t)plane * planeBlocks * kBlock + q;
    if (over) redoList[atomicAdd(redoCount, 1u)] = (uint32_t)k;
    else { hitTuvp[k] = make_float4(best.t, best.u, best.v, __uint_as_float(best.prim)); hitCustom[k] = best.custom; origin_leaf_store(rayOrigin, k, best.leaf); }
    if (STATS) st.flush(stats);
}

template <int STACK, int OCT, bool STATS>
__device__ __forceinline__ void inner_nodes2(const __amdgpu_buffer_rsrc_t nodeBuf, int32_t* lds, int32_t& cur, int32_t*& sp, uint32_t& res,
                                             const rtr_v3 ga, const rtr_v3 gb, const float tmin, const float tmax, const uint32_t kInnerMin, LocalStats& st) {
    typedef uint32_t u32x4 __attribute__((ext_vector_type(4)));
    for (;;) {
        const unsigned long long innerMask = __ballot(cur >= 0);
        if (innerMask == 0ull) break;
        if ((uint32_t)__popcll(innerMask) <= kInnerMin && __ballot(cur < 0 && cur != kDone) != 0ull) break;
        if (cur >= 0) {
            if (STATS) st.nodes++;
            const int32_t nodeOff = cur << 5;
            const u32x4 a = __builtin_amdgcn_raw_buffer_load_b128(nodeBuf, nodeOff, 0, 0);
            const u32x4 b = __builtin_amdgcn_raw_buffer_load_b128(nodeBuf, nodeOff + 16, 0, 0);
            const int32_t top = *sp;
            float tl, tr;
            const bool hl = slab_oct<OCT>(a.x, a.y, b.x, ga, gb, tmin, tmax, tl);
            const bool hr = slab_oct<OCT>(a.z, a.w, b.y, ga, gb, tmin, tmax, tr);
            const bool swap = tr < tl;
            const int32_t c0 = (int32_t)b.z, c1 = (int32_t)b.w;
            const bool both = hl && hr, none = !(hl || hr);
            const bool second = both ? swap : !hl;
            int32_t next = second ? c1 : c0;
            if (both) { sp += kBlock; *sp = swap ? c0 : c1; }
            if (sp > lds + STACK * kBlock) { res = 2u; next = kDone; }
            else if (none) { next = top; sp -= kBlock; }
            cur = next;
        }
    }
}

template <int STACK, bool STATS>
__global__ __launch_bounds__(kBlock) __attribute__((amdgpu_waves_per_eu(8, 8))) void k_primary_persist(DeviceScene sc, RenderArgs ra, float4* hitTuvp, uint32_t* hitCustom, float4* rayOrigin,
                                                         Counters* stats, uint32_t* redoCount, uint32_t* redoList, uint32_t* cursors,
                                                         uint32_t planeStride, uint32_t kBatch, uint32_t kRefill, uint32_t kInnerMin) {
    __shared__ int32_t s_stack[(STACK + 1 + 1) * kBlock];
    int32_t* lds = s_stack + threadIdx.x;
    lds[0] = kDone;
    LocalStats st;
    uint32_t batchPos = 0, batchEnd = 0;
    bool exhausted = false;
    const uint32_t n = ra.spp * planeStride;
    const uint32_t regionLen = ((n + kQueueRegions - 1) / kQueueRegions + kBatch - 1) / kBatch * kBatch;
    const uint32_t myRegion = blockIdx.x % kQueueRegions;
    uint32_t regionTry = 0;
    int32_t cur = kDone;
    int32_t* sp = lds;
    const rtr_v3 o = rtr_ld3(ra.cam.position);
    rtr_v3 d = rtr_mk(0, 0, 0), ga = rtr_mk(0, 0, 0), gb = rtr_mk(0, 0, 0);
    HitRec best; best.t = 0.f; best.u = 0.f; best.v = 0.f; best.custom = RTR_MISS; best.prim = RTR_MISS; best.leaf = 0;
    uint32_t item = 0, res = kResNone;
    const float tmin = 0.001f, tmax = 10000.0f;
    const __amdgpu_buffer_rsrc_t nodeBuf = __builtin_amdgcn_make_buffer_rsrc((void*)sc.nodes, 0, 0xffffffff, 0x00020000);
    const __amdgpu_buffer_rsrc_t triBuf = __builtin_amdgcn_make_buffer_rsrc((void*)sc.tris, 0, 0xffffffff, 0x00020000);
    typedef uint32_t u32x4 __attribute__((ext_vector_type(4)));

    for (;;) {
        const unsigned long long idle = __ballot(cur == kDone);
        const uint32_t nIdle = (uint32_t)__popcll(idle);
        if (nIdle >= kRefill || nIdle == 64u) {
            if (cur == kDone && res != kResNone) {
                if (res == 2u) redoList[atomicAdd(redoCount, 1u)] = item;
                else { hitTuvp[item] = make_float4(best.t, best.u, best.v, __uint_as_float(best.prim)); hitCustom[item] = best.custom; origin_leaf_store(rayOrigin, item, best.leaf); }
                res = kResNone;
            }
            if (!exhausted) {
                if (batchPos == batchEnd) {
                    for (;;) {
                        if (regionTry >= kQueueRegions) { exhausted = true; break; }
                        const uint32_t r = (myRegion + regionTry) % kQueueRegions;
                        const uint32_t lo = r * regionLen;
                        uint32_t hi = lo + regionLen; if (hi > n) hi = n;
                        uint32_t b = hi;
                        if (lo < hi) {
                            uint32_t got = 0;
                            if ((threadIdx.x & 63u) == 0) got = atomicAdd(cursors + 16u * r, kBatch);
                            got = (uint32_t)__builtin_amdgcn_readfirstlane((int)got);
                            b = got < regionLen ? lo + got : hi;
                        }
                        if (b < hi) { batchPos = b; batchEnd = (b + kBatch < hi) ? b + kBatch : hi; break; }
                        ++regionTry;
                    }
                }
                if (!exhausted) {
                    const uint32_t avail = batchEnd - batchPos;
                    const uint32_t prefix = __builtin_amdgcn_mbcnt_hi((uint32_t)(idle >> 32), __builtin_amdgcn_mbcnt_lo((uint32_t)idle, 0u));
                    if (cur == kDone && prefix < avail) {
                        item = batchPos + prefix;
                        const uint32_t i = item / planeStride, q = item - i * planeStride;
                        uint32_t px, lrow, py;
                        if (pixel_of(ra, q, px, lrow, py)) {
                            d = primary_dir(ra, px, py, i);
                            if (STATS) { st.rays++; st.primary++; }
                            const rtr_v3 idir = rtr_mk(rtr_safe_rcp_dir(d.x), rtr_safe_rcp_dir(d.y), rtr_safe_rcp_dir(d.z));
                            rtr_ray_grid(o, idir, sc.grid->origin, sc.grid->scale, &ga, &gb);
                            best.t = tmax; best.u = 0.f; best.v = 0.f; best.custom = RTR_MISS; best.prim = RTR_MISS; best.leaf = 0;
                            cur = 0; sp = lds; res = 0u;
                        }
                    }
                    batchPos += (nIdle < avail) ? nIdle : avail;
                }
            }
        }
        if (__ballot(cur != kDone) == 0ull) {
            if (exhausted) break;
            continue;
        }
        {
            const unsigned long long innerNow = __ballot(cur >= 0);
            if (innerNow != 0ull) {
                const uint32_t oct = (ga.x < 0.f ? 1u : 0u) | (ga.y < 0.f ? 2u : 0u) | (ga.z < 0.f ? 4u : 0u);
                const uint32_t woct = (uint32_t)__builtin_amdgcn_readlane((int)oct, (int)__ffsll((long long)innerNow) - 1);
                const bool mixed = __ballot(cur >= 0 && oct != woct) != 0ull;
                const float limit = best.t;
                switch (mixed ? 8u : woct) {
                    case 0: inner_nodes2<STACK, 0, STATS>(nodeBuf, lds, cur, sp, res, ga, gb, tmin, limit, kInnerMin, st); break;
                    case 1: inner_nodes2<STACK, 1, STATS>(nodeBuf, lds, cur, sp, res, ga, gb, tmin, limit, kInnerMin, st); break;
                    case 2: inner_nodes2<STACK, 2, STATS>(nodeBuf, lds, cur, sp, res, ga, gb, tmin, limit, kInnerMin, st); break;
                    case 3: inner_nodes2<STACK, 3, STATS>(nodeBuf, lds, cur, sp, res, ga, gb, tmin, limit, kInnerMin, st); break;
                    case 4: inner_nodes2<STACK, 4, STATS>(nodeBuf, lds, cur, sp, res, ga, gb, tmin, limit, kInnerMin, st); break;
                    case 5: inner_nodes2<STACK, 5, STATS>(nodeBuf, lds, cur, sp, res, ga, gb, tmin, limit, kInnerMin, st); break;
                    case 6: inner_nodes2<STACK, 6, STATS>(nodeBuf, lds, cur, sp, res, ga, gb, tmin, limit, kInnerMin, st); break;
                    case 7: inner_nodes2<STACK, 7, STATS>(nodeBuf, lds, cur, sp, res, ga, gb, tmin, limit, kInnerMin, st); break;
                    default: inner_nodes2<STACK, 8, STATS>(nodeBuf, lds, cur, sp, res, ga, gb, tmin, limit, kInnerMin, st); break;
                }
            }
        }
        if (cur < 0 && cur != kDone) {
            const int32_t leafCode = cur;
            const uint32_t code = (uint32_t)~cur;
            const uint32_t first = code >> 3, cnt = (code & 7u) + 1u;
            for (uint32_t i = 0; i < cnt; ++i) {
                const int32_t triOff = (int32_t)((first + i) * 48u);
                const u32x4 r0 = __builtin_amdgcn_raw_buffer_load_b128(triBuf, triOff, 0, 0);
                const u32x4 r1 = __builtin_amdgcn_raw_buffer_load_b128(triBuf, triOff + 16, 0, 0);
                const u32x4 r2 = __builtin_amdgcn_raw_buffer_load_b128(triBuf, triOff + 32, 0, 0);
                if (STATS) st.tris++;
                float t, u, v;
                if (rtr_mt_intersect(o, d, rtr_mk(__uint_as_float(r0.x), __uint_as_float(r0.y), __uint_as_float(r0.z)),
                                     rtr_mk(__uint_as_float(r1.x), __uint_as_float(r1.y), __uint_as_float(r1.z)),
                                     rtr_mk(__uint_as_float(r2.x), __uint_as_float(r2.y), __uint_as_float(r2.z)), tmin, &t, &u, &v) && t < tmax) {
                    const uint32_t cu = r0.w, pr = r1.w;
                    if ((r2.w & 1u) && !alpha_pass<STATS>(sc, cu, pr, u, v, st)) continue;
                    if (t < best.t || (t == best.t && (cu < best.custom || (cu == best.custom && pr < best.prim)))) {
                        best.t = t; best.u = u; best.v = v; best.custom = cu; best.prim = pr; best.leaf = leafCode;
                    }
                }
            }
            cur = *sp; sp -= kBlock;
        }
    }
    if (STATS) st.flush(stats);
}

template <bool STATS>
__global__ __launch_bounds__(kBlock) void k_shadow_tail(DeviceScene sc, const RayQueue queue, const uint32_t* __restrict__ overflow, uint32_t overflowCap,
                                                        const uint32_t* __restrict__ count, uint8_t* __restrict__ vis, int32_t* __restrict__ spill, Counters* stats) {
    uint32_t n = overflow[0];
    if (n == 0) return;
    const bool all = n > overflowCap;
    if (all) n = *count;
    int32_t* stack = spill + blockIdx.x * kBlock + threadIdx.x;
    LocalStats st;
    for (uint32_t i = blockIdx.x * kBlock + threadIdx.x; i < n; i += kTailBlocks * kBlock) {
        const uint32_t r = all ? i : overflow[1u + i];
        rtr_v3 ro, rd; float rt; uint32_t rs;
        queue_load(queue, r, ro, rd, rt, rs, 0u);
        HitRec h;
        const bool occ = trace<true, STATS, kTailBlocks * kBlock>(sc, stack, ro, rd, 0.001f, rt, h, st);
        if (STATS) { st.rays--; st.shadow--; }
        vis[rs] = occ ? 1 : 0;
    }
    if (STATS) st.flush(stats);
}

#ifndef RTR_RESOLVE_WAVES
#define RTR_RESOLVE_WAVES 4
#endif
#ifndef RTR_RESOLVE_WAVES_FB
#define RTR_RESOLVE_WAVES_FB 6
#endif
#define RTR_RESOLVE_ATTR __attribute__((amdgpu_waves_per_eu(FULL ? RTR_RESOLVE_WAVES : RTR_RESOLVE_WAVES_FB, 8)))
template <bool STATS, bool FULL>
__global__ __launch_bounds__(kBlock) RTR_RESOLVE_ATTR void k_resolve(DeviceScene sc, FrameBatch fb, uint32_t planeStride, const float4* hitTuvp,
                                                    const uint32_t* hitCustom, const uint8_t* vis, uint32_t slotStride, Counters* stats, uint32_t rowWaves) {
    uint32_t q = blockIdx.x * kBlock + threadIdx.x;
    if (rowWaves) {
        const uint32_t row = (threadIdx.x >> 6) + 4u * (blockIdx.x & 1u), col = threadIdx.x & 63u;
        q = (blockIdx.x >> 1) * (2u * kBlock) + (col >> 3) * 64u + row * 8u + (col & 7u);
    }
    const uint32_t frame = batch_frame(q, planeStride, q);
    if (frame >= fb.n) return;
    const RenderArgs& ra = fb.ra[frame];
    const FrameOut& fo = fb.fo[frame];
    uint32_t px, lrow, py;
    if (!pixel_of(ra, q, px, lrow, py)) return;
    LocalStats st;
    Accum acc = zero_accum();
    const uint32_t want = FULL ? ((fo.img[0] != nullptr ? 1u : 0u) | (fo.img[2] != nullptr ? 2u : 0u)) : 0u;
    for (uint32_t i = 0; i < ra.spp; ++i) {
        const size_t k = ((size_t)frame * ra.spp + i) * planeStride + q;
        const float4 r = hitTuvp[k];
        HitRec h; h.t = r.x; h.u = r.y; h.v = r.z; h.prim = __float_as_uint(r.w); h.custom = hitCustom[k];
        const rtr_v3 dir = primary_dir(ra, px, py, i);
        LookupPolicy pol{vis, (uint32_t)k, slotStride, vis_mask32(vis, (uint32_t)k, slotStride, ra.maxRaysPerSample), 0u};
        shade_sample<LookupPolicy, STATS>(sc, ra, px, py, h, dir, want, acc, pol, st);
    }
    if (FULL) write_pixel(ra, fo, out_index(ra, px, lrow, py), acc);
    else write_pixel_framebuffer(ra, fo, out_index(ra, px, lrow, py), acc.shadowed);
    if (STATS) st.flush(stats);
}

#ifndef RTR_EXP_DOUBLE_FETCH_GEN
#define RTR_EXP_DOUBLE_FETCH_GEN 0
#endif
#ifndef RTR_EXP_DOUBLE_FETCH
#define RTR_EXP_DOUBLE_FETCH 0
#endif
#ifndef RTR_RESOLVE_CAP
#define RTR_RESOLVE_CAP 192
#endif
#ifndef RTR_RESOLVE_COMPACT_WAVES
#define RTR_RESOLVE_COMPACT_WAVES 5
#endif
constexpr uint32_t kResolveCap = RTR_RESOLVE_CAP;
static_assert(kResolveCap % 32 == 0 && kResolveCap >= 128 && kResolveCap <= 1024, "RTR_RESOLVE_CAP");
constexpr uint32_t kResolveMaxLights = 255u, kResolveMaxLightTris = 4094u, kResolveMaxSamples = 63u;
constexpr uint32_t kItemDirectional = 0xfffu;

__device__ __forceinline__ void wave_lds_sync() {
    __builtin_amdgcn_fence(__ATOMIC_RELEASE, "wavefront");
    __builtin_amdgcn_wave_barrier();
    __builtin_amdgcn_fence(__ATOMIC_ACQUIRE, "wavefront");
}

__global__ __launch_bounds__(kBlock) __attribute__((amdgpu_waves_per_eu(RTR_RESOLVE_COMPACT_WAVES, 8)))
void k_resolve_compact(DeviceScene sc, FrameBatch fb, uint32_t planeStride, const float4* __restrict__ hitTuvp, const uint32_t* __restrict__ hitCustom,
                       const uint8_t* __restrict__ vis, uint32_t slotStride) {
    constexpr uint32_t kWaves = kBlock / 64;
    __shared__ float4 s_surf[kWaves][4][64];
    __shared__ uint32_t s_item[kWaves][kResolveCap];
    __shared__ float s_con[kWaves][3][kResolveCap];
    const uint32_t wave = threadIdx.x >> 6, lane = threadIdx.x & 63u;
    uint32_t q = blockIdx.x * kBlock + threadIdx.x;
    const uint32_t frame = batch_frame(q, planeStride, q);
    if (frame >= fb.n) return;
    const RenderArgs& ra = fb.ra[frame];
    const FrameOut& fo = fb.fo[frame];
    uint32_t px, lrow, py;
    const bool valid = pixel_of(ra, q, px, lrow, py);
    if (__ballot(valid) == 0ull) return;
    const uint32_t pxBase = (uint32_t)__builtin_amdgcn_readfirstlane((int)(px - (lane & 7u))), pyBase = (uint32_t)__builtin_amdgcn_readfirstlane((int)(py - (lane >> 3)));
    const uint32_t ns = ra.numShadowRays;
    const float nsf = (float)ns;
    const rtr_v3 directLightDir = directional_light_dir();
    LocalStats st;
    Accum acc = zero_accum();
    for (uint32_t i = 0; i < ra.spp; ++i) {
        const size_t k = ((size_t)frame * ra.spp + i) * planeStride + q;
        bool has = false;
        Surface sf;
        sf.hitPoint = sf.hitNormal = rtr_mk(0, 0, 0);
        if (valid) {
            const float4 r = hitTuvp[k];
            HitRec h; h.t = r.x; h.u = r.y; h.v = r.z; h.prim = __float_as_uint(r.w); h.custom = hitCustom[k];
            has = fetch_surface<true, false>(sc, ra, h, primary_dir(ra, px, py, i), false, acc, sf, st);
#if RTR_EXP_DOUBLE_FETCH
            if (has) {
                HitRec h2 = h; h2.u = h.u + (float)(ra.spp - 1u) * 1.0e-30f; h2.v = h.v + (float)(ra.spp - 1u) * 1.0e-30f;
                Surface sf2; Accum acc2 = zero_accum();
                const bool has2 = fetch_surface<true, false>(sc, ra, h2, primary_dir(ra, px, py, i), false, acc2, sf2, st);
                if (has2 && sf2.roughness == 12345.0f && sf2.hitPoint.x == 4321.0f && sf2.color.y == 777.0f && sf2.viewDir.z == 55.0f && sf2.hitNormal.y == 99.0f) sf = sf2;
            }
#endif
        }
        wave_lds_sync();
        if (has) {
            const rtr_v3 cd = surface_diffuse(sf.om, sf.color);
            s_surf[wave][0][lane] = make_float4(sf.hitPoint.x, sf.hitPoint.y, sf.hitPoint.z, sf.roughness);
            s_surf[wave][1][lane] = make_float4(sf.hitNormal.x, sf.hitNormal.y, sf.hitNormal.z, cd.x);
            s_surf[wave][2][lane] = make_float4(sf.viewDir.x, sf.viewDir.y, sf.viewDir.z, cd.y);
            s_surf[wave][3][lane] = make_float4(sf.mSpecular.x, sf.mSpecular.y, sf.mSpecular.z, cd.z);
        }
        const rtr_v3 hitPoint = sf.hitPoint, hitNormal = sf.hitNormal;
        uint32_t qdone = 0;
        rtr_v3 shadowedSample = rtr_mk(0, 0, 0);
        uint32_t e0 = 0, total = 0;
        do {
            uint32_t count = 0, e = 0, e1 = e0;
            uint32_t vmask = 0, imask = 0;
            bool full = false;
            const uint32_t occ = has ? vis_mask32(vis, (uint32_t)k + qdone * slotStride, slotStride, ra.maxRaysPerSample - qdone) : 0xffffffffu;
            uint32_t nq = 0;
            for (uint32_t li = 0; li < ra.info.numAreaLights; ++li) {
                const RtrAreaLightInfo* L = sc.lights + li;
                const uint32_t lnt = L->numTriangles, first = sc.lightTriFirst[li];
                const bool twoSided = L->isTwoSided != 0u;
                for (uint32_t ti = 0; ti < lnt; ++ti) {
                    if (full || e + ns <= e0) { e += ns; continue; }
                    const float4* rec = sc.lightTris + (size_t)(first + ti) * kLightTriRecord;
                    const float4 r0 = rec[0], r3 = rec[3];
                    const bool culled = !twoSided && rtr_dot(rtr_mk(r3.x, r3.y, r3.z), rtr_sub(hitPoint, rtr_mk(r0.x, r0.y, r0.z))) < 0.0f;
                    const bool issued = has && !culled;
                    for (uint32_t s = 0; s < ns; ++s, ++e) {
                        if (e < e0 || full) continue;
                        bool v = false;
                        if (issued) { v = ((occ >> nq) & 1u) == 0u; ++nq; }
                        const unsigned long long m = __ballot(v);
                        if (v) s_item[wave][count + __builtin_amdgcn_mbcnt_hi((uint32_t)(m >> 32), __builtin_amdgcn_mbcnt_lo((uint32_t)m, 0u))] = lane | (s << 6) | ((first + ti) << 12) | (li << 24);
                        const uint32_t bit = e - e0;
                        vmask |= (v ? 1u : 0u) << bit; imask |= (issued ? 1u : 0u) << bit;
                        count += (uint32_t)__popcll(m);
                        e1 = e + 1u;
                        full = count + 64u > kResolveCap || e1 - e0 == 32u;
                    }
                }
            }
            if (!full && e >= e0) {
                const bool issued = has && rtr_dot(hitNormal, directLightDir) > 0.0f;
                bool v = false;
                if (issued) { v = ((occ >> nq) & 1u) == 0u; ++nq; }
                const unsigned long long m = __ballot(v);
                if (v) s_item[wave][count + __builtin_amdgcn_mbcnt_hi((uint32_t)(m >> 32), __builtin_amdgcn_mbcnt_lo((uint32_t)m, 0u))] = lane | (kItemDirectional << 12);
                const uint32_t bit = e - e0;
                vmask |= (v ? 1u : 0u) << bit; imask |= (issued ? 1u : 0u) << bit;
                count += (uint32_t)__popcll(m);
                e1 = e + 1u;
            }
            total = e + 1u;
            qdone += nq;
            wave_lds_sync();
            for (uint32_t c = lane; c < count; c += 64u) {
                const uint32_t item = s_item[wave][c];
                const uint32_t src = item & 63u, s = (item >> 6) & 63u, tri = (item >> 12) & 0xfffu, li = item >> 24;
                const float4 a0 = s_surf[wave][0][src], a1 = s_surf[wave][1][src], a2 = s_surf[wave][2][src], a3 = s_surf[wave][3][src];
                const rtr_v3 hp = rtr_mk(a0.x, a0.y, a0.z), hn = rtr_mk(a1.x, a1.y, a1.z), vd = rtr_mk(a2.x, a2.y, a2.z), ms = rtr_mk(a3.x, a3.y, a3.z), cd = rtr_mk(a1.w, a2.w, a3.w);
                rtr_v3 con;
                if (tri == kItemDirectional) con = directional_contrib(hn, vd, a0.w, ms, cd);
                else {
                    const float4* rec = sc.lightTris + (size_t)tri * kLightTriRecord;
                    const float4 r0 = rec[0], r1 = rec[1], r2 = rec[2];
                    rtr_v3 P[3];
                    P[0] = rtr_mk(r0.x, r0.y, r0.z); P[1] = rtr_mk(r1.x, r1.y, r1.z); P[2] = rtr_mk(r2.x, r2.y, r2.z);
                    const RtrAreaLightInfo* L = sc.lights + li;
                    const rtr_v3 lightVec = rtr_sub(light_sample_pos(P, s, pxBase + (src & 7u), pyBase + (src >> 3), ra.info.frame), hp);
                    con = area_sample_contrib(hn, vd, a0.w, ms, cd, rtr_ld3(L->color), L->intensity, r1.w, rtr_normalize(lightVec), rtr_length(lightVec));
                }
                s_con[wave][0][c] = con.x; s_con[wave][1][c] = con.y; s_con[wave][2][c] = con.z;
            }
            wave_lds_sync();
            uint32_t base = 0;
            e = 0;
            for (uint32_t li = 0; li < ra.info.numAreaLights; ++li) {
                const uint32_t lnt = sc.lights[li].numTriangles;
                for (uint32_t ti = 0; ti < lnt; ++ti) {
                    if (e >= e1 || e + ns <= e0) { e += ns; continue; }
                    for (uint32_t s = 0; s < ns; ++s, ++e) {
                        if (e < e0 || e >= e1) continue;
                        const uint32_t bit = e - e0;
                        const bool v = ((vmask >> bit) & 1u) != 0u;
                        const unsigned long long m = __ballot(v);
                        if (v) {
                            const uint32_t at = base + __builtin_amdgcn_mbcnt_hi((uint32_t)(m >> 32), __builtin_amdgcn_mbcnt_lo((uint32_t)m, 0u));
                            shadowedSample = rtr_madd(shadowedSample, rtr_mk(s_con[wave][0][at], s_con[wave][1][at], s_con[wave][2][at]), 1.0f);
                        }
                        base += (uint32_t)__popcll(m);
                        if (s + 1u == ns) {
                            if ((imask >> bit) & 1u) acc.shadowed = rtr_add(acc.shadowed, rtr_mk(shadowedSample.x / nsf, shadowedSample.y / nsf, shadowedSample.z / nsf));
                            shadowedSample = rtr_mk(0, 0, 0);
                        }
                    }
                }
            }
            if (e >= e0 && e < e1) {
                const uint32_t bit = e - e0;
                const bool v = ((vmask >> bit) & 1u) != 0u;
                const unsigned long long m = __ballot(v);
                if (v) {
                    const uint32_t at = base + __builtin_amdgcn_mbcnt_hi((uint32_t)(m >> 32), __builtin_amdgcn_mbcnt_lo((uint32_t)m, 0u));
                    acc.shadowed = rtr_madd(acc.shadowed, rtr_mk(s_con[wave][0][at], s_con[wave][1][at], s_con[wave][2][at]), 1.0f);
                }
            }
            e0 = e1;
        } while (e0 < total);
    }
    if (valid) write_pixel_framebuffer(ra, fo, out_index(ra, px, lrow, py), acc.shadowed);
}

__global__ __launch_bounds__(kBlock) void k_deinterleave(const uint32_t* __restrict__ gathered, uint32_t* __restrict__ dst,
                                                         uint32_t width, uint32_t height, uint32_t bandRows,
                                                         uint32_t shardCount, uint32_t localRows) {
    const size_t total = (size_t)width * height;
    for (size_t p = (size_t)blockIdx.x * kBlock + threadIdx.x; p < total; p += (size_t)gridDim.x * kBlock) {
        const uint32_t y = (uint32_t)(p / width), x = (uint32_t)(p % width);
        const uint32_t band = y / bandRows, r = y % bandRows;
        const uint32_t shard = band % shardCount, lb = band / shardCount;
        dst[p] = gathered[((size_t)shard * localRows + (size_t)lb * bandRows + r) * width + x];
    }
}

__global__ __launch_bounds__(64) void k_light_tris(const RtrAreaLightInfo* __restrict__ lights, const RtrVertex* __restrict__ vertices,
                                                   const uint32_t* __restrict__ indices, const uint32_t* __restrict__ first,
                                                   uint32_t numLights, float4* __restrict__ out) {
    const uint32_t l = blockIdx.x * 64u + threadIdx.x;
    if (l >= numLights) return;
    const RtrAreaLightInfo* L = lights + l;
    for (uint32_t ti = 0; ti < L->numTriangles; ++ti) light_tri_record(L, vertices, indices, ti, out + (size_t)(first[l] + ti) * kLightTriRecord);
}

__global__ __launch_bounds__(kBlock) void k_fill_planes(uint4* __restrict__ vis, uint32_t word, uint32_t planeVec, uint32_t pitchVec,
                                                        uint32_t* __restrict__ ctrl, uint32_t ctrlWords, uint32_t* __restrict__ overflowCount) {
    if (blockIdx.x == 0 && blockIdx.y == 0) {
        for (uint32_t i = threadIdx.x; i < ctrlWords; i += kBlock) ctrl[i] = 0u;
        if (threadIdx.x == 0) overflowCount[0] = 0u;
    }
    const uint4 v = make_uint4(word, word, word, word);
    uint4* plane = vis + (size_t)blockIdx.y * pitchVec;
    for (uint32_t i = blockIdx.x * kBlock + threadIdx.x; i < planeVec; i += gridDim.x * kBlock) plane[i] = v;
}

namespace {
struct TunableField { const char* name; uint32_t Tunables::* field; uint32_t lo, hi; };
const TunableField kTunables[] = {
    {"primary_packet", &Tunables::primary_packet, 0u, 1u}, {"primary_wide", &Tunables::primary_wide, 0u, 1u}, {"primary_persist", &Tunables::primary_persist, 0u, 2u}, {"primary_persist_min_rays", &Tunables::primary_persist_min_rays, 0u, 0xffffffffu},
    {"primary_batch", &Tunables::primary_batch, 64u, 1u << 16}, {"primary_refill", &Tunables::primary_refill, 1u, 64u},
    {"primary_inner_min", &Tunables::primary_inner_min, 0u, 63u}, {"primary_wgs_per_cu", &Tunables::primary_wgs_per_cu, 1u, 8u},
    {"trace_bvh4", &Tunables::trace_bvh4, 0u, 1u}, {"trace_batch", &Tunables::trace_batch, 0u, 1u << 20}, {"trace_binned", &Tunables::trace_binned, 0u, 2u},
    {"queue_nt", &Tunables::queue_nt, 0u, 3u}, {"trace_wgs_per_cu", &Tunables::trace_wgs_per_cu, 0u, 8u}, {"trace_refill", &Tunables::trace_refill, 1u, 64u},
    {"trace_inner_min", &Tunables::trace_inner_min, 0u, 63u}, {"trace_octant_forms", &Tunables::trace_octant_forms, 0u, 1u}, {"trace_own_leaf", &Tunables::trace_own_leaf, 0u, 1u},
    {"trace_top_nodes", &Tunables::trace_top_nodes, 0u, 0xffffffffu}, {"resolve_row_waves", &Tunables::resolve_row_waves, 0u, 1u}, {"resolve_compact", &Tunables::resolve_compact, 0u, 1u}, {"split_priorities", &Tunables::split_priorities, 0u, 1u},
};
}

bool tunable_set(Tunables& t, const char* name, uint32_t value) {
    for (const TunableField& f : kTunables)
        if (name && !strcmp(name, f.name)) { if (value < f.lo || value > f.hi) return false; t.*(f.field) = value; return true; }
    return false;
}
bool tunable_get(const Tunables& t, const char* name, uint32_t* value) {
    for (const TunableField& f : kTunables) if (name && !strcmp(name, f.name)) { if (value) *value = t.*(f.field); return true; }
    return false;
}
Tunables tunables_from_env() {
    Tunables t;
    for (const TunableField& f : kTunables) {
        char env[64] = "RTR_"; size_t n = 4;
        for (const char* c = f.name; *c && n + 1 < sizeof env; ++c) env[n++] = (char)(*c >= 'a' && *c <= 'z' ? *c - 32 : *c);
        env[n] = 0;
        const char* v = getenv(env);
        if (!v || !*v) continue;
        char* end = nullptr;
        const unsigned long x = strtoul(v, &end, 10);
        if (end == v) continue;
        t.*(f.field) = x < f.lo ? f.lo : (x > f.hi ? f.hi : (uint32_t)x);
    }
    return t;
}

static uint32_t padded_pixels(const RenderArgs& ra) {
    const uint32_t band8 = (ra.localRows + 7u) / 8u;
    return band8 * ra.tilesPerRow * 64u;
}

template <int STACK>
static hipError_t mega_t(const DeviceScene& sc, const RenderArgs& ra, const FrameOut& fo, Counters* stats, hipStream_t s) {
    const uint32_t blocks = (padded_pixels(ra) + kBlock - 1) / kBlock;
    if (stats) hipLaunchKernelGGL((k_megakernel<STACK, true>), dim3(blocks), dim3(kBlock), 0, s, sc, ra, fo, stats);
    else hipLaunchKernelGGL((k_megakernel<STACK, false>), dim3(blocks), dim3(kBlock), 0, s, sc, ra, fo, stats);
    return hipGetLastError();
}

hipError_t launch_megakernel(const DeviceScene& sc, const RenderArgs& ra, const FrameOut& fo, int stackEntries,
                             Counters* stats, hipStream_t stream) {
    switch (stackEntries) {
        case 16: return mega_t<16>(sc, ra, fo, stats, stream);
        case 32: return mega_t<32>(sc, ra, fo, stats, stream);
        case 64: return mega_t<64>(sc, ra, fo, stats, stream);
        default: return hipErrorInvalidValue;
    }
}

template <int STACK>
static hipError_t wave_t(const DeviceScene& sc, const FrameBatch& fb, const Workspace& ws, const Tunables& tun,
                         Counters* stats, hipStream_t s, hipEvent_t* ev, uint32_t numCus) {
    const RenderArgs& ra = fb.ra[0];
    const uint32_t nb = fb.n;
    const uint32_t blocks = (padded_pixels(ra) + kBlock - 1) / kBlock;
    {
        const uint32_t planeVec = (uint32_t)(ws.visPlaneBytes / 16u), pitchVec = ws.rayQueue.slotStride / 16u;
        uint32_t fblocks = std::min<uint32_t>((planeVec + kBlock - 1) / kBlock, std::max<uint32_t>(4096u / std::max<uint32_t>(ws.visPlanes, 1u), 64u));
        if (fblocks == 0) fblocks = 1;
        hipLaunchKernelGGL(k_fill_planes, dim3(fblocks, ws.visPlanes ? ws.visPlanes : 1u), dim3(kBlock), 0, s, reinterpret_cast<uint4*>(ws.vis), ws.visFill * 0x01010101u, planeVec, pitchVec,
                           ws.queueCount, kQueueCtrlWords, ws.overflow);
    }
    if (ev) hipEventRecord(ev[0], s);
    const uint32_t kPersist = tun.primary_persist;
    const uint32_t kPersistMinRays = tun.primary_persist_min_rays;
    const uint32_t kPBatch = tun.primary_batch, kPRefill = tun.primary_refill, kPInnerMin = tun.primary_inner_min, kPWgsPerCu = tun.primary_wgs_per_cu;
    const uint32_t planeStride = blocks * kBlock;
    const unsigned long long camRays = (unsigned long long)planeStride * ra.spp;
    bool packet = false;
    if ((kPersist == 1u || (kPersist == 2u && camRays >= kPersistMinRays)) && nb == 1u && camRays < 0xffffffffull) {
        uint32_t pblocks = numCus * kPWgsPerCu;
        const uint32_t pneeded = (uint32_t)(((unsigned long long)planeStride * ra.spp + kBlock - 1) / kBlock);
        if (pblocks > pneeded) pblocks = pneeded;
        if (pblocks == 0) pblocks = 1;
        if (stats) hipLaunchKernelGGL((k_primary_persist<16, true>), dim3(pblocks), dim3(kBlock), 0, s, sc, fb.ra[0], ws.hitTuvp, ws.hitCustom, ws.rayQueue.origin, stats, ws.queueCount + kPrimaryRedoWord, ws.overflow + 1, ws.queueCount + kPrimaryCursors, planeStride, kPBatch, kPRefill, kPInnerMin);
        else hipLaunchKernelGGL((k_primary_persist<16, false>), dim3(pblocks), dim3(kBlock), 0, s, sc, fb.ra[0], ws.hitTuvp, ws.hitCustom, ws.rayQueue.origin, stats, ws.queueCount + kPrimaryRedoWord, ws.overflow + 1, ws.queueCount + kPrimaryCursors, planeStride, kPBatch, kPRefill, kPInnerMin);
    } else if (tun.primary_wide && sc.nodes4) {
        if (stats) hipLaunchKernelGGL((k_primary4<true>), dim3(blocks * ra.spp * nb), dim3(kBlock), 0, s, sc, fb, ws.hitTuvp, ws.hitCustom, ws.rayQueue.origin, stats, ws.queueCount + kPrimaryRedoWord, ws.overflow + 1, blocks);
        else hipLaunchKernelGGL((k_primary4<false>), dim3(blocks * ra.spp * nb), dim3(kBlock), 0, s, sc, fb, ws.hitTuvp, ws.hitCustom, ws.rayQueue.origin, stats, ws.queueCount + kPrimaryRedoWord, ws.overflow + 1, blocks);
    } else if (tun.primary_packet) {
        packet = true;
        if (stats) hipLaunchKernelGGL((k_primary_packet<true>), dim3(blocks * ra.spp * nb), dim3(kBlock), 0, s, sc, fb, ws.hitTuvp, ws.hitCustom, ws.rayQueue.origin, stats, blocks);
        else hipLaunchKernelGGL((k_primary_packet<false>), dim3(blocks * ra.spp * nb), dim3(kBlock), 0, s, sc, fb, ws.hitTuvp, ws.hitCustom, ws.rayQueue.origin, stats, blocks);
    } else if (stats) hipLaunchKernelGGL((k_primary<STACK, true>), dim3(blocks * (kBlock / kPrimBlock) * ra.spp * nb), dim3(kPrimBlock), 0, s, sc, fb, ws.hitTuvp, ws.hitCustom, ws.rayQueue.origin, stats, ws.queueCount + kPrimaryRedoWord, ws.overflow + 1, blocks * (kBlock / kPrimBlock));
    else hipLaunchKernelGGL((k_primary<STACK, false>), dim3(blocks * (kBlock / kPrimBlock) * ra.spp * nb), dim3(kPrimBlock), 0, s, sc, fb, ws.hitTuvp, ws.hitCustom, ws.rayQueue.origin, stats, ws.queueCount + kPrimaryRedoWord, ws.overflow + 1, blocks * (kBlock / kPrimBlock));
    if (!packet) {
        if (stats) hipLaunchKernelGGL(k_primary_tail<true>, dim3(kTailBlocks), dim3(kBlock), 0, s, sc, fb, ws.hitTuvp, ws.hitCustom, ws.rayQueue.origin, ws.queueCount + kPrimaryRedoWord, ws.overflow + 1, ws.spill, planeStride, stats);
        else hipLaunchKernelGGL(k_primary_tail<false>, dim3(kTailBlocks), dim3(kBlock), 0, s, sc, fb, ws.hitTuvp, ws.hitCustom, ws.rayQueue.origin, ws.queueCount + kPrimaryRedoWord, ws.overflow + 1, ws.spill, planeStride, stats);
    }
    if (ev) hipEventRecord(ev[1], s);
    const uint32_t kBatchEnv = tun.trace_batch;
    const uint32_t kBatch = kBatchEnv >= 64u ? kBatchEnv : ((size_t)nb * blocks * kBlock * ra.spp * ra.maxRaysPerSample >= kBatchLongQueue ? kBatchLong : kBatchDefault);
    const uint32_t kWide = tun.trace_bvh4;
    const uint32_t genBlocks = (nb * blocks * kBlock + kGenBlock - 1) / kGenBlock, genOctBlocks = (nb * blocks * kBlock + kGenOctBlock - 1) / kGenOctBlock;
    const uint32_t binMode = tun.trace_binned;
    const size_t maxRaysQ = (size_t)nb * blocks * kBlock * ra.spp * ra.maxRaysPerSample;
    const bool wide = kWide && sc.nodes4;
    const bool binned = wide && ws.batchLists && (size_t)ra.spp * ra.maxRaysPerSample <= 65535u &&
                        (size_t)ws.capRays / kBatch / kQueueRegions + genOctBlocks <= ws.listStride &&
                        (binMode == 1u || (binMode == 2u && maxRaysQ >= kBinnedMinRays && sc.numNodes4 >= kBinnedMinNodes));
    const uint32_t kNtQueue = tun.queue_nt;
    RayQueue rq = ws.rayQueue;
    rq.ownLeaf = (wide && tun.trace_own_leaf) ? 1u : 0u;
    if (binned) hipLaunchKernelGGL(k_shadow_gen_oct, dim3(genOctBlocks), dim3(kGenOctBlock), 0, s, sc, fb, ws.hitTuvp, ws.hitCustom, rq, ws.queueCount, blocks * kBlock, ws.batchLists, ws.listStride, kBatch, kNtQueue >> 1);
    else hipLaunchKernelGGL(k_shadow_gen, dim3(genBlocks), dim3(kGenBlock), 0, s, sc, fb, ws.hitTuvp, ws.hitCustom, rq, ws.queueCount, blocks * kBlock);
    if (ev) hipEventRecord(ev[2], s);
    const size_t maxRays = (size_t)nb * blocks * kBlock * ra.spp * ra.maxRaysPerSample;
    const uint32_t kWgsPerCu = tun.trace_wgs_per_cu;
    uint32_t tblocks = numCus * (kWgsPerCu ? kWgsPerCu : (maxRays >= kBinnedMinRays ? 8u : 6u));
    const uint32_t needed = (uint32_t)((maxRays + kBlock - 1) / kBlock);
    if (tblocks > needed) tblocks = needed;
    if (tblocks == 0) tblocks = 1;
    const uint32_t kRefill = tun.trace_refill, kInnerMin = tun.trace_inner_min;
    (void)sizeof(STACK);
    const uint32_t kOct = tun.trace_octant_forms | ((kNtQueue & 1u) << 1);
    const uint32_t kTop = tun.trace_top_nodes < kTopNodes ? tun.trace_top_nodes : kTopNodes;
    const uint32_t top = kTop < sc.numNodes4 ? kTop : sc.numNodes4;
    uint32_t tblocks4 = tblocks * (uint32_t)kBlock / (uint32_t)kTraceBlock;
    if (tblocks4 == 0) tblocks4 = 1;
    if (wide) {
        if (stats) {
            if (binned) hipLaunchKernelGGL((k_shadow_trace4<RTR_SHADOW_STACK, true, true>), dim3(tblocks4), dim3(kTraceBlock), 0, s, sc, ws.rayQueue, ws.queueCount, ws.queueCount + kBatchCursorWord, ws.vis, ws.visFill, kBatch, kRefill, kInnerMin, ws.overflow, ws.overflowCap, kOct, top, ws.batchLists, ws.listStride, stats, ws.clk);
            else hipLaunchKernelGGL((k_shadow_trace4<RTR_SHADOW_STACK, false, true>), dim3(tblocks4), dim3(kTraceBlock), 0, s, sc, ws.rayQueue, ws.queueCount, ws.queueCount + kBatchCursorWord, ws.vis, ws.visFill, kBatch, kRefill, kInnerMin, ws.overflow, ws.overflowCap, kOct, top, ws.batchLists, ws.listStride, stats, ws.clk);
        } else {
            if (binned) hipLaunchKernelGGL((k_shadow_trace4<RTR_SHADOW_STACK, true, false>), dim3(tblocks4), dim3(kTraceBlock), 0, s, sc, ws.rayQueue, ws.queueCount, ws.queueCount + kBatchCursorWord, ws.vis, ws.visFill, kBatch, kRefill, kInnerMin, ws.overflow, ws.overflowCap, kOct, top, ws.batchLists, ws.listStride, stats, ws.clk);
            else hipLaunchKernelGGL((k_shadow_trace4<RTR_SHADOW_STACK, false, false>), dim3(tblocks4), dim3(kTraceBlock), 0, s, sc, ws.rayQueue, ws.queueCount, ws.queueCount + kBatchCursorWord, ws.vis, ws.visFill, kBatch, kRefill, kInnerMin, ws.overflow, ws.overflowCap, kOct, top, ws.batchLists, ws.listStride, stats, ws.clk);
        }
    } else hipLaunchKernelGGL((k_shadow_trace<16>), dim3(tblocks), dim3(kBlock), 0, s, sc, ws.rayQueue, ws.queueCount, ws.queueCount + kBatchCursorWord, ws.vis, ws.visFill, kBatch, kRefill, kInnerMin, ws.overflow, ws.overflowCap);
    if (ev) hipEventRecord(ev[5], s);
    if (stats) hipLaunchKernelGGL((k_shadow_tail<true>), dim3(kTailBlocks), dim3(kBlock), 0, s, sc, ws.rayQueue, ws.overflow, ws.overflowCap, ws.queueCount, ws.vis, ws.spill, stats);
    else hipLaunchKernelGGL((k_shadow_tail<false>), dim3(kTailBlocks), dim3(kBlock), 0, s, sc, ws.rayQueue, ws.overflow, ws.overflowCap, ws.queueCount, ws.vis, ws.spill, stats);
    if (ev) hipEventRecord(ev[3], s);
    const uint32_t kRowWaves = tun.resolve_row_waves;
    const uint32_t rowWaves = (kRowWaves && ra.tilesPerRow % 8u == 0u && blocks % 2u == 0u) ? 1u : 0u;
    const bool full = (ra.images & ~((1u << 1) | (1u << 16))) != 0u;
    const bool compact = !stats && !full && tun.resolve_compact && !rowWaves && ra.numShadowRays >= 1u && ra.numShadowRays <= kResolveMaxSamples &&
                         sc.numLights <= kResolveMaxLights && sc.numLightTris <= kResolveMaxLightTris;
    if (compact) hipLaunchKernelGGL(k_resolve_compact, dim3(blocks * nb), dim3(kBlock), 0, s, sc, fb, blocks * kBlock, ws.hitTuvp, ws.hitCustom, ws.vis, ws.rayQueue.slotStride);
    else if (stats) {
        if (full) hipLaunchKernelGGL((k_resolve<true, true>), dim3(blocks * nb), dim3(kBlock), 0, s, sc, fb, blocks * kBlock, ws.hitTuvp, ws.hitCustom, ws.vis, ws.rayQueue.slotStride, stats, rowWaves);
        else hipLaunchKernelGGL((k_resolve<true, false>), dim3(blocks * nb), dim3(kBlock), 0, s, sc, fb, blocks * kBlock, ws.hitTuvp, ws.hitCustom, ws.vis, ws.rayQueue.slotStride, stats, rowWaves);
    } else {
        if (full) hipLaunchKernelGGL((k_resolve<false, true>), dim3(blocks * nb), dim3(kBlock), 0, s, sc, fb, blocks * kBlock, ws.hitTuvp, ws.hitCustom, ws.vis, ws.rayQueue.slotStride, stats, rowWaves);
        else hipLaunchKernelGGL((k_resolve<false, false>), dim3(blocks * nb), dim3(kBlock), 0, s, sc, fb, blocks * kBlock, ws.hitTuvp, ws.hitCustom, ws.vis, ws.rayQueue.slotStride, stats, rowWaves);
    }
    if (ev) hipEventRecord(ev[4], s);
    return hipGetLastError();
}

hipError_t launch_wavefront(const DeviceScene& sc, const FrameBatch& fb, const Workspace& ws, const Tunables& tun,
                            int stackEntries, Counters* stats, hipStream_t stream, hipEvent_t* ev, uint32_t numCus) {
    if (numCus == 0) numCus = 256;
    if (fb.n < 1 || fb.n > kMaxBatch) return hipErrorInvalidValue;
    switch (stackEntries) {
        case 16: return wave_t<16>(sc, fb, ws, tun, stats, stream, ev, numCus);
        case 32: return wave_t<32>(sc, fb, ws, tun, stats, stream, ev, numCus);
        case 64: return wave_t<64>(sc, fb, ws, tun, stats, stream, ev, numCus);
        default: return hipErrorInvalidValue;
    }
}

hipError_t launch_occlusion_walk(const DeviceScene& sc, const OcclusionArgs& oa, const Tunables& tun, bool alpha, Counters* stats, hipStream_t s, uint32_t numCus,
                                 const RayMaskArgs& rm) {
    if (numCus == 0) numCus = 256;
    if (!sc.nodes4) return hipErrorInvalidValue;
    RayQueue rq;
    rq.dt = const_cast<float4*>(oa.rays); rq.slot = oa.queue;
    const bool hinted = oa.startLeaves != nullptr;
    if (hinted) { rq.origin = reinterpret_cast<float4*>(const_cast<int32_t*>(oa.startLeaves)); rq.slotMask = oa.numTris; }
    uint32_t tblocks = numCus * (tun.trace_wgs_per_cu ? tun.trace_wgs_per_cu : (oa.n >= kBinnedMinRays ? 8u : 6u)) * (uint32_t)kBlock / (uint32_t)kTraceBlock;
    const uint32_t needed = (uint32_t)(((uint64_t)oa.n + kTraceBlock - 1) / kTraceBlock);
    if (tblocks > needed) tblocks = needed;
    if (tblocks == 0) tblocks = 1;
    const uint32_t kOct = tun.trace_octant_forms | ((tun.queue_nt & 1u) << 1) | (alpha ? 0u : 4u);
    const uint32_t kTop = tun.trace_top_nodes < kTopNodes ? tun.trace_top_nodes : kTopNodes;
    const uint32_t top = kTop < sc.numNodes4 ? kTop : sc.numNodes4;
    uint32_t* const ctrl = oa.ctrl;
    const bool masked = rm.masked != 0u;
    if (masked) rq.slotStride = (rm.cullMask & 0xffu) | ((rm.masked & kCullAll) << 4);
    const uint32_t* const cnt = masked ? reinterpret_cast<const uint32_t*>(rm.rayMasks) : ctrl;
#define RTR_OCC_WALK(STATS, HINTS, MASKED) hipLaunchKernelGGL((k_shadow_trace4<RTR_SHADOW_STACK, true, STATS, true, HINTS, MASKED>), dim3(tblocks), dim3(kTraceBlock), 0, s, sc, rq, cnt, ctrl + kBatchCursorWord, \
        oa.occluded, 0u, oa.batch, tun.trace_refill, tun.trace_inner_min, oa.overflow, oa.overflowCap, kOct, top, oa.lists, oa.listStride, stats, (unsigned long long*)nullptr)
    if (masked) {
        if (hinted) { if (stats) RTR_OCC_WALK(true, true, true); else RTR_OCC_WALK(false, true, true); }
        else { if (stats) RTR_OCC_WALK(true, false, true); else RTR_OCC_WALK(false, false, true); }
    } else if (hinted) { if (stats) RTR_OCC_WALK(true, true, false); else RTR_OCC_WALK(false, true, false); }
    else { if (stats) RTR_OCC_WALK(true, false, false); else RTR_OCC_WALK(false, false, false); }
#undef RTR_OCC_WALK
    return hipGetLastError();
}

hipError_t launch_light_tris(const RtrAreaLightInfo* lights, const RtrVertex* vertices, const uint32_t* indices, const uint32_t* first,
                             uint32_t numLights, float4* out, hipStream_t stream) {
    if (numLights == 0) return hipSuccess;
    hipLaunchKernelGGL(k_light_tris, dim3((numLights + 63u) / 64u), dim3(64), 0, stream, lights, vertices, indices, first, numLights, out);
    return hipGetLastError();
}

hipError_t launch_deinterleave(const uint32_t* gathered, uint32_t* dst, uint32_t width, uint32_t height,
                               uint32_t bandRows, uint32_t shardCount, uint32_t localRows, hipStream_t stream) {
    const size_t total = (size_t)width * height;
    uint32_t blocks = (uint32_t)((total + kBlock - 1) / kBlock);
    if (blocks > 2048u) blocks = 2048u;
    if (blocks == 0) blocks = 1;
    hipLaunchKernelGGL(k_deinterleave, dim3(blocks), dim3(kBlock), 0, stream, gathered, dst, width, height, bandRows, shardCount, localRows);
    return hipGetLastError();
}

}
```

### realtimeraytracer_amd/csrc/rtr_api.cpp

```cpp
#include "../../include/rtr.h"
#include "../../include/rtr_math.h"
#include "bvh_build.h"
#include "kernels/rtr_kernels.h"
#include "kernels/rtr_post.h"
#include "kernels/rtr_bvh.h"
#include "kernels/rtr_mirrored.h"
#include "kernels/rtr_tree_sah.h"
#include "kernels/rtr_query.h"
#include "kernels/rtr_bounce_launch.h"
#include "rtr_bounce_host.h"
#include "kernels/rtr_paths_launch.h"
#include "rtr_paths_host.h"
#include "rtr_pick_host.h"
#include "kernels/rtr_mis_launch.h"
#include "rtr_mis_host.h"

#include <hip/hip_runtime.h>

#include <algorithm>
#include <chrono>
#include <cstdarg>
#include <cstdio>
#include <cstring>
#include <string>
// ... 37 lines not shown
        if (count == 0) count = 1;
        hipError_t e = hipMalloc((void**)&p, count * sizeof(T));
        if (e == hipSuccess) n = count;
        return e;
    }
    hipError_t grow(size_t count) { return (p && n >= count) ? hipSuccess : alloc(count + count / 2); }
    hipError_t ensure(size_t count) { return (p && n >= count) ? hipSuccess : alloc(count); }
    hipError_t upload(const T* src, size_t count, hipStream_t s) {
        hipError_t e = alloc(count);
        if (e != hipSuccess) return e;
        if (count == 0 || !src) return hipSuccess;
        e = hipMemcpyAsync(p, src, count * sizeof(T), hipMemcpyHostToDevice, s);
        if (e != hipSuccess) return e;
        return hipStreamSynchronize(s);
    }
};

}

struct rtr_ctx {
    int device = 0;
    hipStream_t stream = nullptr;
    bool ownStream = false;
    hipDeviceProp_t prop;
    int numXccs = 0;
    int children = 0;
    bool destroyed = false;
    rtrdev::Tunables tun;
    DevBuf<uint32_t> qCtrl, qRedo;
    DevBuf<int32_t> qSpill;
    DevBuf<Counters> qCounters;
    hipEvent_t qEv[2] = {nullptr, nullptr};
    hipStream_t qLastStream = nullptr;
};

static void ctx_free(rtr_ctx* c) {
    (void)hipSetDevice(c->device);
    if (c->qLastStream) (void)hipEventSynchronize(c->qEv[1]);
    for (hipEvent_t e : c->qEv) if (e) (void)hipEventDestroy(e);
    if (c->ownStream && c->stream) (void)hipStreamDestroy(c->stream);
    delete c;
}
static void ctx_release_child(rtr_ctx* c) {
    if (--c->children == 0 && c->destroyed) ctx_free(c);
}

struct BuildScratch {
    DevBuf<float4> trisCanon, minCanon, maxCanon;
    DevBuf<unsigned long long> keysIn, keysOut;
    DevBuf<int2> range, rawChild;
    DevBuf<uint8_t> sortTemp;
    size_t sortTempBytes = 0;
};

struct TreeStage {
    DevBuf<uint4> nodes;
    DevBuf<float4> nodesF, tris, boxMin, boxMax;
    DevBuf<RtrBvhGrid> grid;
    DevBuf<int32_t> parent;
    DevBuf<uint32_t> slotOfPrim, red;
};

namespace {
struct SceneTree {
    DevBuf<uint4> nodes;
    DevBuf<float4> nodesF;
    DevBuf<RtrBvhGrid> grid;
    DevBuf<unsigned long long> wideSums;
    DevBuf<uint4> nodes4tmp;
    DevBuf<uint32_t> wideRemap;
    DevBuf<uint8_t> wideShape;
    std::vector<uint8_t> hostWideShape;
    uint32_t wideReached = 0;
    DevBuf<uint4> nodes4;
    DevBuf<float4> tris;
    std::vector<RtrBvhNode> hostNodes;
    std::vector<RtrBvhTri> hostTris;
    DevBuf<rtrdev::PrimRef> prims;
    DevBuf<rtrdev::InstanceRef> instRefs;
    DevBuf<float4> boxMin, boxMax;
    DevBuf<int32_t> parent;
    DevBuf<uint32_t> counters, depth, slotOfPrim, red;
    uint32_t numPrims = 0, numNodeSlots = 0;
    bool refitReady = false;
    mutable DevBuf<int32_t> leafTable;
    mutable bool leafReady = false;
    mutable DevBuf<int32_t> costParent;
    mutable int costParentState = 0;
    DevBuf<uint32_t> orderScratch;
    bool asyncReady = false;
    bool rebuildReady = false;
    bool rebuildIfReady = false;
    rtr_scene_stats stats{};
};
}

struct rtr_scene {
    rtr_ctx* ctx = nullptr;
    SceneTree tree;
    DevBuf<RtrVertex> vertices;
    DevBuf<uint32_t> indices;
    DevBuf<RtrObjectInfo> objects;
    DevBuf<RtrAreaLightInfo> lights;
    DevBuf<float4> lightTris;
    DevBuf<uint32_t> lightTriFirst;
    DevBuf<uint32_t> triCount;
    uint32_t numInstances = 0;
    std::vector<uint8_t> hostMasks;
    DevBuf<uint32_t> maskBits;
    std::vector<uint32_t> hostTriCount;
    mutable DevBuf<uint32_t> leafBase;
    DevBuf<float> xforms, nmats, ltc1, ltc2;
    std::vector<DevBuf<uint8_t>> texPixels;
    DevBuf<uint8_t> hdriPixels;
    DevBuf<rtrdev::DeviceTexture> texTable;
    std::vector<RtrAreaLightInfo> hostLights;
    std::vector<RtrInstance> hostInstances;
    std::vector<RtrMesh> hostMeshes;
    std::vector<RtrObjectInfo> hostObjects;
    DevBuf<rtrdev::VertexRange> vtxRanges;
    DevBuf<uint32_t> vtxPrefix, vtxStage;
    std::vector<uint32_t> vtxHost;
    BuildScratch buildScratch;
    TreeStage stage;
    mutable bool depthStale = false;
    DevBuf<unsigned long long> policy;
    DevBuf<uint32_t> asyncWords;
    mutable bool mirrorsStale = false;
    DevBuf<uint32_t> instCustom;
    mutable bool instancesStale = false;
    uint64_t asyncEnqueued = 0;
    mutable DevBuf<unsigned long long> costWords;
    DeviceScene dev{};
    uint32_t numLights = 0, numObjects = 0, numVertices = 0, numIndices = 0;
    bool hasLtc = false;
};

constexpr size_t kPolicyRecordAt = 12, kPolicyWords = kPolicyRecordAt + sizeof(rtrdev::RebuildIfRecord) / sizeof(unsigned long long);
static rtrdev::RebuildIfRecord* policy_record(const rtr_scene* s) { return reinterpret_cast<rtrdev::RebuildIfRecord*>(s->policy.p + kPolicyRecordAt); }

static bool scene_is_empty(const rtr_scene* s) { return s->tree.hostTris.empty() || s->tree.hostTris[0].customIndex == 0xffffffffu; }

struct rtr_frame {
    rtr_ctx* ctx = nullptr;
    uint32_t width = 0, rows = 0, images = 0;
    DevBuf<uint32_t> img[8];
    uint32_t* ext[8] = {nullptr, nullptr, nullptr, nullptr, nullptr, nullptr, nullptr, nullptr};
    DevBuf<float4> hdr;
    DevBuf<float4> hitTuvp, rayDT, rayOrigin;
    DevBuf<uint32_t> raySlot;
    uint32_t slotStride = 0;
    uint32_t visFill = 1;
    DevBuf<uint32_t> hitCustom, queueCount;
    DevBuf<uint8_t> vis;
    DevBuf<int32_t> spill;
    DevBuf<uint32_t> overflow;
    uint32_t overflowCap = 0;
    DevBuf<uint2> batchLists;
    DevBuf<unsigned long long> clk;
    uint32_t listStride = 0;
    DevBuf<Counters> counters;
    hipEvent_t ev[6] = {nullptr, nullptr, nullptr, nullptr, nullptr, nullptr};
    hipEvent_t evMega[2] = {nullptr, nullptr};
    rtr_frame_stats stats{};
    bool pendingStats = false, pendingWave = false, pendingCounters = false;
    uint32_t pendingImagesK = 0; bool pendingHdr = false, pendingAccum = false;
    hipEvent_t evDone = nullptr;
    bool viaBatch = false;
    hipStream_t batchStream = nullptr;
    bool ownPending = false;
    hipEvent_t evOwn = nullptr;
    std::vector<rtr_ctx*> partCtx;
    std::vector<rtr_frame*> parts;
    std::vector<hipEvent_t> evPart;
    hipEvent_t evSplit[2] = {nullptr, nullptr};
    uint32_t pendingSplit = 0;
    float4* extHdr = nullptr;
    uint32_t* image_ptr(int which) const { return ext[which] ? ext[which] : img[which].p; }
    float4* hdr_ptr() const { return extHdr ? extHdr : hdr.p; }
};

void rtrdev::set_last_error(const char* msg) { g_err = msg; }

extern "C" {

const char* rtr_last_error(void) { return g_err.c_str(); }

const char* rtr_status_string(int s) {
    switch (s) {
        case RTR_OK: return "RTR_OK";
        case RTR_ERR_INVALID_ARGUMENT: return "RTR_ERR_INVALID_ARGUMENT";
        case RTR_ERR_HIP: return "RTR_ERR_HIP";
        case RTR_ERR_NO_DEVICE: return "RTR_ERR_NO_DEVICE";
        case RTR_ERR_UNSUPPORTED: return "RTR_ERR_UNSUPPORTED";
        case RTR_ERR_OUT_OF_MEMORY: return "RTR_ERR_OUT_OF_MEMORY";
        case RTR_ERR_BVH_TOO_DEEP: return "RTR_ERR_BVH_TOO_DEEP";
        case RTR_ERR_IO: return "RTR_ERR_IO";
        default: return "RTR_ERR_UNKNOWN";
    }
}

int rtr_abi_version(void) { return RTR_ABI_VERSION; }

const char* rtr_kernel_revision(void) { return RTR_ANYHIT_KERNEL_REVISION; }

uint32_t rtr_shard_rows(uint32_t height, uint32_t bandRows, uint32_t shardCount) {
    if (bandRows == 0) bandRows = 8;
    if (shardCount <= 1) return height;
    uint32_t bands = (height + bandRows - 1) / bandRows;
    uint32_t per = (bands + shardCount - 1) / shardCount;
    return per * bandRows;
}

static int ctx_create_prio(int ordinal, int priorityRank, rtr_ctx** out) {
    if (!out) return fail(RTR_ERR_INVALID_ARGUMENT, "rtr_ctx_create: out is null");
    *out = nullptr;
    int count = 0;
    hipError_t e = hipGetDeviceCount(&count);
    if (e != hipSuccess || count <= 0)
        return fail(RTR_ERR_NO_DEVICE, "rtr_ctx_create: no HIP device (%s); this library has no CPU fallback",
                    e != hipSuccess ? hipGetErrorString(e) : "device count 0");
    if (ordinal < 0 || ordinal >= count) return fail(RTR_ERR_INVALID_ARGUMENT, "rtr_ctx_create: ordinal %d not in [0,%d)", ordinal, count);
    HIP_TRY(hipSetDevice(ordinal));
    rtr_ctx* c = new rtr_ctx();
    c->device = ordinal;
    e = hipGetDeviceProperties(&c->prop, ordinal);
    if (e != hipSuccess) { delete c; return fail(RTR_ERR_HIP, "hipGetDeviceProperties: %s", hipGetErrorString(e)); }
    if (hipDeviceGetAttribute(&c->numXccs, hipDeviceAttributeNumberOfXccs, ordinal) != hipSuccess) c->numXccs = 0;
    if (priorityRank >= 0) {
        int least = 0, greatest = 0;
        if (hipDeviceGetStreamPriorityRange(&least, &greatest) != hipSuccess) { least = greatest = 0; }
        int prio = greatest + priorityRank;
        if (prio > least) prio = least;
        e = hipStreamCreateWithPriority(&c->stream, hipStreamNonBlocking, prio);
    } else e = hipStreamCreateWithFlags(&c->stream, hipStreamNonBlocking);
    if (e != hipSuccess) { delete c; return fail(RTR_ERR_HIP, "hipStreamCreate: %s", hipGetErrorString(e)); }
    c->ownStream = true;
    c->tun = rtrdev::tunables_from_env();
    *out = c;
    return RTR_OK;
}

int rtr_ctx_create(int ordinal, rtr_ctx** out) { return ctx_create_prio(ordinal, -1, out); }

int rtr_ctx_set_tunable(rtr_ctx* c, const char* name, uint32_t value) {
    if (!c || !name) return fail(RTR_ERR_INVALID_ARGUMENT, "rtr_ctx_set_tunable: null argument");
    if (!rtrdev::tunable_set(c->tun, name, value)) return fail(RTR_ERR_INVALID_ARGUMENT, "rtr_ctx_set_tunable: no tunable '%s', or %u is outside its range", name, value);
    return RTR_OK;
}

int rtr_ctx_get_tunable(const rtr_ctx* c, const char* name, uint32_t* value) {
    if (!c || !name || !value) return fail(RTR_ERR_INVALID_ARGUMENT, "rtr_ctx_get_tunable: null argument");
    if (!rtrdev::tunable_get(c->tun, name, value)) return fail(RTR_ERR_INVALID_ARGUMENT, "rtr_ctx_get_tunable: no tunable '%s'", name);
    return RTR_OK;
}

void rtr_ctx_destroy(rtr_ctx* c) {
    if (!c || c->destroyed) return;
    if (c->children > 0) { (void)hipSetDevice(c->device); (void)hipStreamSynchronize(c->stream); c->destroyed = true; return; }
    ctx_free(c);
}

int rtr_ctx_set_stream(rtr_ctx* c, void* s) {
    if (!c) return fail(RTR_ERR_INVALID_ARGUMENT, "rtr_ctx_set_stream: ctx is null");
    HIP_TRY(hipSetDevice(c->device));
    if (c->ownStream && c->stream) { HIP_TRY(hipStreamSynchronize(c->stream)); (void)hipStreamDestroy(c->stream); }
    if (s) { c->stream = (hipStream_t)s; c->ownStream = false; }
    else { HIP_TRY(hipStreamCreateWithFlags(&c->stream, hipStreamNonBlocking)); c->ownStream = true; }
    return RTR_OK;
}

int rtr_ctx_get_stream(rtr_ctx* c, void** out) {
    if (!c || !out) return fail(RTR_ERR_INVALID_ARGUMENT, "rtr_ctx_get_stream: null argument");
    *out = (void*)c->stream;
    return RTR_OK;
}

int rtr_ctx_device_name(rtr_ctx* c, char* buf, size_t bytes) {
    if (!c || !buf || bytes == 0) return fail(RTR_ERR_INVALID_ARGUMENT, "rtr_ctx_device_name: bad argument");
    if (c->numXccs > 0) snprintf(buf, bytes, "%s (%s, %d CUs in %d XCDs)", c->prop.name, c->prop.gcnArchName, c->prop.multiProcessorCount, c->numXccs);
    else snprintf(buf, bytes, "%s (%s)", c->prop.name, c->prop.gcnArchName);
    return RTR_OK;
}

static int validate_desc(const rtr_scene_desc* d) {
    if (!d) return fail(RTR_ERR_INVALID_ARGUMENT, "scene desc is null");
    if ((d->numVertices && !d->vertices) || (d->numIndices && !d->indices) || (d->numMeshes && !d->meshes) ||
        (d->numInstances && !d->instances) || (d->numObjects && !d->objects) || (d->numLights && !d->lights))
        return fail(RTR_ERR_INVALID_ARGUMENT, "scene desc: null array with non-zero count");
    if ((d->ltc1 == nullptr) != (d->ltc2 == nullptr)) return fail(RTR_ERR_INVALID_ARGUMENT, "scene desc: ltc1 and ltc2 must both be given or both null");
    for (uint32_t m = 0; m < d->numMeshes; ++m) {
        const RtrMesh& me = d->meshes[m];
        if (me.indexCount % 3u) return fail(RTR_ERR_INVALID_ARGUMENT, "mesh %u: indexCount %u not a multiple of 3", m, me.indexCount);
        if ((uint64_t)me.indexOffset + me.indexCount > d->numIndices) return fail(RTR_ERR_INVALID_ARGUMENT, "mesh %u: index range exceeds the index array", m);
        if ((uint64_t)me.vertexOffset + me.vertexCount > d->numVertices) return fail(RTR_ERR_INVALID_ARGUMENT, "mesh %u: vertex range exceeds the vertex array", m);
        for (uint32_t i = 0; i < me.indexCount; ++i)
            if (d->indices[me.indexOffset + i] >= me.vertexCount)
                return fail(RTR_ERR_INVALID_ARGUMENT, "mesh %u: index %u (= %u) outside its %u vertices", m, i, d->indices[me.indexOffset + i], me.vertexCount);
    }
    std::vector<uint8_t> seen(d->numInstances, 0);
    for (uint32_t i = 0; i < d->numInstances; ++i) {
        const RtrInstance& in = d->instances[i];
        if (in.meshIndex >= d->numMeshes) return fail(RTR_ERR_INVALID_ARGUMENT, "instance %u: meshIndex %u >= %u", i, in.meshIndex, d->numMeshes);
        if (in.customIndex >= d->numInstances || seen[in.customIndex]) return fail(RTR_ERR_INVALID_ARGUMENT, "instance %u: customIndex %u out of range or duplicated", i, in.customIndex);
        seen[in.customIndex] = 1;
        if (in.customIndex >= d->numLights && in.customIndex - d->numLights >= d->numObjects)
// ... 1262 lines not shown
    delete f;
    ctx_release_child(c);
}

int rtr_frame_bind_external(rtr_frame* f, int which, void* dptr, size_t bytes) {
    if (!f || which < 0 || which > 7) return fail(RTR_ERR_INVALID_ARGUMENT, "rtr_frame_bind_external: bad argument");
    if (dptr && bytes != (size_t)f->width * f->rows * 4) return fail(RTR_ERR_INVALID_ARGUMENT, "rtr_frame_bind_external: %zu bytes given, image is %zu", bytes, (size_t)f->width * f->rows * 4);
    if (dptr && ((uintptr_t)dptr & 3u)) return fail(RTR_ERR_INVALID_ARGUMENT, "rtr_frame_bind_external: pointer not 4-byte aligned");
    f->ext[which] = (uint32_t*)dptr;
    if (dptr) f->images |= RTR_IMG_BIT(which);
    return RTR_OK;
}

int rtr_frame_device_ptr(const rtr_frame* f, int which, void** dptr, size_t* bytes) {
    if (!f || !dptr) return fail(RTR_ERR_INVALID_ARGUMENT, "rtr_frame_device_ptr: null argument");
    if (which == RTR_IMAGE_HDR) {
        if (!f->hdr.p) return fail(RTR_ERR_INVALID_ARGUMENT, "frame has no HDR image");
        *dptr = f->hdr.p; if (bytes) *bytes = (size_t)f->width * f->rows * 16; return RTR_OK;
    }
    if (which < 0 || which > 7 || !f->image_ptr(which)) return fail(RTR_ERR_INVALID_ARGUMENT, "frame has no image %d", which);
    *dptr = f->image_ptr(which); if (bytes) *bytes = (size_t)f->width * f->rows * 4;
    return RTR_OK;
}

int rtr_frame_download(const rtr_frame* f, int which, void* dst, size_t bytes) {
    if (!f || !dst) return fail(RTR_ERR_INVALID_ARGUMENT, "rtr_frame_download: null argument");
    void* src = nullptr; size_t need = 0;
    int rc = rtr_frame_device_ptr(f, which, &src, &need);
    if (rc != RTR_OK) return rc;
    if (bytes != need) return fail(RTR_ERR_INVALID_ARGUMENT, "rtr_frame_download: %zu bytes given, image %d is %zu", bytes, which, need);
    HIP_TRY(hipSetDevice(f->ctx->device));
    if (f->viaBatch) HIP_TRY(hipEventSynchronize(f->evDone));
    HIP_TRY(hipMemcpyAsync(dst, src, bytes, hipMemcpyDeviceToHost, f->ctx->stream));
    HIP_TRY(hipStreamSynchronize(f->ctx->stream));
    return RTR_OK;
}

static int order_on_own_stream(rtr_frame* f) {
    hipStream_t st = f->ctx->stream;
    if (f->batchStream && f->batchStream != st) HIP_TRY(hipStreamWaitEvent(st, f->evDone, 0));
    f->batchStream = nullptr;
    f->ownPending = true;
    return RTR_OK;
}

int rtr_frame_clear(rtr_frame* f) {
    if (!f) return fail(RTR_ERR_INVALID_ARGUMENT, "rtr_frame_clear: null frame");
    HIP_TRY(hipSetDevice(f->ctx->device));
    { const int rc = order_on_own_stream(f); if (rc != RTR_OK) return rc; }
    const size_t px = (size_t)f->width * f->rows;
    for (int i = 0; i < 8; ++i) if (f->image_ptr(i)) HIP_TRY(hipMemsetAsync(f->image_ptr(i), 0, px * 4, f->ctx->stream));
    if (f->hdr.p) HIP_TRY(hipMemsetAsync(f->hdr.p, 0, px * 16, f->ctx->stream));
    HIP_TRY(hipStreamSynchronize(f->ctx->stream));
    return RTR_OK;
}

static_assert(RTR_MAX_BATCH == rtrdev::kMaxBatch, "include/rtr.h and kernels/rtr_device.h disagree on the frames per launch");
static int enqueue_render(rtr_scene* s, const RtrCameraData* cams, const RtrSceneInfo* infos, const rtr_render_params* pin, rtr_frame* const* frames, uint32_t n, bool direct = false) {
    if (!s || !cams || !infos || !pin || !frames || n < 1 || !frames[0]) return fail(RTR_ERR_INVALID_ARGUMENT, "rtr_render: null argument");
    if (n > rtrdev::kMaxBatch) return fail(RTR_ERR_INVALID_ARGUMENT, "rtr_render_batch_async: %u frames, at most %u per launch", n, rtrdev::kMaxBatch);
    rtr_frame* f = frames[0];
    if (s->ctx->device != f->ctx->device) return fail(RTR_ERR_INVALID_ARGUMENT, "rtr_render: scene and frame live on different devices");
    rtr_render_params p = *pin;
    if (p.bandRows == 0) p.bandRows = 8;
    if (p.shardCount == 0) p.shardCount = 1;
    if (p.images == 0) p.images = RTR_IMAGES_FRAMEBUFFER;
    if (p.width == 0 || p.height == 0 || p.spp == 0 || p.spp > 1024 || p.numShadowRays > 1024)
        return fail(RTR_ERR_INVALID_ARGUMENT, "rtr_render: bad width/height/spp/numShadowRays (%u,%u,%u,%u)", p.width, p.height, p.spp, p.numShadowRays);
    if (p.bandRows % 8u) return fail(RTR_ERR_INVALID_ARGUMENT, "rtr_render: bandRows %u must be a multiple of 8 (one wave = one 8x8 tile)", p.bandRows);
    if (p.shardIndex >= p.shardCount) return fail(RTR_ERR_INVALID_ARGUMENT, "rtr_render: shardIndex %u >= shardCount %u", p.shardIndex, p.shardCount);
    const uint32_t rows = rtr_shard_rows(p.height, p.bandRows, p.shardCount);
    const uint32_t frameRows = direct ? p.height : rows;
    if (p.images & RTR_IMAGES_DENOISE) return fail(RTR_ERR_UNSUPPORTED, "rtr_render: denoise/combine images are produced by rtr_denoise_combine, not by the ray-gen dispatch");
    if ((p.images & RTR_IMG_BIT(RTR_IMAGE_ANALYTIC)) && !s->hasLtc) return fail(RTR_ERR_UNSUPPORTED, "rtr_render: RTR_IMAGE_ANALYTIC needs the LTC tables (rtr_scene_desc.ltc1/ltc2)");
    const bool wantHdr = (p.images & RTR_IMG_BIT(RTR_IMAGE_HDR)) != 0 || p.accumulate;
    if (n > 1 && p.pipeline == 1) return fail(RTR_ERR_UNSUPPORTED, "rtr_render_batch_async: the megakernel renders one frame per launch");

    rtrdev::FrameBatch fb{};
    fb.n = n;
    uint32_t k = 0;
    uint64_t maxRays = 1;
    for (uint32_t b = 0; b < n; ++b) {
        rtr_frame* fr = frames[b];
        if (!fr) return fail(RTR_ERR_INVALID_ARGUMENT, "rtr_render_batch_async: frame %u is null", b);
        for (uint32_t c = 0; c < b; ++c) if (frames[c] == fr) return fail(RTR_ERR_INVALID_ARGUMENT, "rtr_render_batch_async: frame %u given twice", b);
        if (fr->ctx->device != f->ctx->device) return fail(RTR_ERR_INVALID_ARGUMENT, "rtr_render_batch_async: frame %u lives on another device", b);
        if (infos[b].numAreaLights > s->numLights) return fail(RTR_ERR_INVALID_ARGUMENT, "rtr_render: SceneInfo.numAreaLights %u > scene lights %u", infos[b].numAreaLights, s->numLights);
        if (infos[b].numAreaLights != infos[0].numAreaLights) return fail(RTR_ERR_INVALID_ARGUMENT, "rtr_render_batch_async: the frames of a launch must use the same number of area lights");
        if (fr->width != p.width || fr->rows != frameRows) return fail(RTR_ERR_INVALID_ARGUMENT, "rtr_render: frame is %ux%u, this shard needs %ux%u", fr->width, fr->rows, p.width, frameRows);
        if (wantHdr && !fr->hdr_ptr()) return fail(RTR_ERR_INVALID_ARGUMENT, "rtr_render: HDR accumulation requested but the frame has no RTR_IMAGE_HDR");
        FrameOut& fo = fb.fo[b];
        k = 0;
        for (int i = 0; i < 8; ++i) {
            fo.img[i] = nullptr;
            if (p.images & RTR_IMG_BIT(i)) {
                if (!fr->image_ptr(i)) return fail(RTR_ERR_INVALID_ARGUMENT, "rtr_render: image %d requested but not in the frame", i);
                fo.img[i] = fr->image_ptr(i); ++k;
            }
        }
        fo.hdr = wantHdr ? fr->hdr_ptr() : nullptr;
        RenderArgs& ra = fb.ra[b];
        ra.cam = cams[b]; ra.info = infos[b];
        ra.width = p.width; ra.height = p.height; ra.spp = p.spp; ra.numShadowRays = p.numShadowRays;
        ra.bandRows = p.bandRows; ra.shardIndex = p.shardIndex; ra.shardCount = p.shardCount;
        ra.localRows = rows; ra.tilesPerRow = (p.width + 7u) / 8u;
        ra.images = p.images; ra.accumulate = p.accumulate; ra.accumulatedFrames = p.accumulatedFrames; ra.directRows = direct ? 1u : 0u;
        if (b == 0) for (uint32_t l = 0; l < infos[0].numAreaLights; ++l) maxRays += (uint64_t)s->hostLights[l].numTriangles * p.numShadowRays;
        ra.maxRaysPerSample = (uint32_t)maxRays;
    }
    const RenderArgs& ra = fb.ra[0];
    const FrameOut& fo = fb.fo[0];

    HIP_TRY(hipSetDevice(f->ctx->device));
    hipStream_t st = f->ctx->stream;
    Counters* dstats = nullptr;
    if (p.collectStats) { HIP_TRY(hipMemsetAsync(f->counters.p, 0, sizeof(Counters), st)); dstats = f->counters.p; }

    const uint64_t paddedPixels = (uint64_t)((rows + 7u) / 8u) * ra.tilesPerRow * 64u;
    const uint64_t blocks = (paddedPixels + 255u) / 256u;
    const uint64_t nPS = blocks * 256u * p.spp * n;
    const uint64_t nRays = nPS * maxRays;
    uint64_t slotStride = 256;
    while (slotStride < nPS) slotStride <<= 1;
    const uint64_t nSlots = slotStride * maxRays;
    bool wave = p.pipeline != 1;
    if (wave && (nSlots >= (1ull << 31) || maxRays > 4096)) {
        if (p.pipeline == 2 || n > 1) return fail(RTR_ERR_UNSUPPORTED, "rtr_render: wavefront scratch would need %llu visibility slots", (unsigned long long)nSlots);
        wave = false;
    }
    if (blocks * n >= (1ull << 31)) return fail(RTR_ERR_INVALID_ARGUMENT, "rtr_render: frame too large");

    if (wave && p.collectStats && f->ctx->tun.trace_bvh4 == 0u)
        return fail(RTR_ERR_UNSUPPORTED, "rtr_render: collectStats with the tunable trace_bvh4 = 0: the 2-wide comparison kernel has no counting form (set it back to 1, or render with pipeline 1)");
    f->pendingWave = wave; f->pendingCounters = p.collectStats != 0;
    f->pendingImagesK = k; f->pendingHdr = wantHdr; f->pendingAccum = p.accumulate != 0;
    memset(&f->stats, 0, sizeof f->stats);
    f->stats.localRows = rows; f->stats.localPixels = rows * p.width * n;
    f->viaBatch = false; f->pendingSplit = 0;
    if (f->batchStream && f->batchStream != st) HIP_TRY(hipStreamWaitEvent(st, f->evDone, 0));
    f->batchStream = nullptr;
    for (uint32_t b = 1; b < n; ++b) {
        rtr_frame* fr = frames[b];
        if (fr->ownPending && fr->ctx->stream != st) {
            if (!fr->evOwn) HIP_TRY(hipEventCreateWithFlags(&fr->evOwn, hipEventDisableTiming));
            HIP_TRY(hipEventRecord(fr->evOwn, fr->ctx->stream));
            HIP_TRY(hipStreamWaitEvent(st, fr->evOwn, 0));
        }
        if (fr->batchStream && fr->batchStream != st) HIP_TRY(hipStreamWaitEvent(st, fr->evDone, 0));
    }
    hipError_t e;
    if (wave) {
        uint64_t ovCap = std::max<uint64_t>(std::max<uint64_t>(nPS, nRays / 16), 1ull << 20);
        if (ovCap > nRays) ovCap = std::max<uint64_t>(nRays, nPS);
        if (f->hitTuvp.n < nPS) { HIP_TRY(f->hitTuvp.alloc(nPS)); HIP_TRY(f->hitCustom.alloc(nPS)); HIP_TRY(f->rayOrigin.alloc(nPS)); }
        if (f->vis.n < nSlots) HIP_TRY(f->vis.alloc(nSlots));
        if (f->rayDT.n < nRays) { HIP_TRY(f->rayDT.alloc(nRays)); HIP_TRY(f->raySlot.alloc(nRays)); }
        if (f->overflow.n < ovCap + 1) HIP_TRY(f->overflow.alloc(ovCap + 1));
        f->overflowCap = (uint32_t)std::min<uint64_t>(ovCap, f->overflow.n - 1);
#ifdef RTR_TEST_HOOKS
        if (const char* e = getenv("RTR_TRACE_OVERFLOW_CAP")) { const uint64_t v = strtoull(e, nullptr, 10); if (v >= 1 && v < f->overflowCap) f->overflowCap = (uint32_t)v; }
#endif
        {
            const uint64_t ls = nRays / 64 / rtrdev::kQueueRegions + nPS / 256 + 16;
            if ((uint64_t)f->listStride < ls) { HIP_TRY(f->batchLists.alloc((size_t)ls * rtrdev::kQueueLists)); f->listStride = (uint32_t)ls; }
        }
        f->slotStride = (uint32_t)slotStride;
        if (!f->queueCount.p) HIP_TRY(f->queueCount.alloc(rtrdev::kQueueCtrlWords));
        if (!f->clk.p) { HIP_TRY(f->clk.alloc(2 * rtrdev::kQueueRegions)); HIP_TRY(hipMemsetAsync(f->clk.p, 0, 2 * rtrdev::kQueueRegions * sizeof(unsigned long long), st)); }
        if (!f->spill.p) HIP_TRY(f->spill.alloc(rtrdev::kSpillInts));
        Workspace ws;
        ws.hitTuvp = f->hitTuvp.p; ws.hitCustom = f->hitCustom.p; ws.vis = f->vis.p; ws.visFill = f->visFill;
        ws.visPlaneBytes = (size_t)nPS; ws.visPlanes = (uint32_t)maxRays;
#ifdef RTR_TEST_HOOKS
        if (const char* e = getenv("RTR_TRACE_VIS_FILL")) if ((e[0] == '0' || e[0] == '1') && !e[1]) ws.visFill = (uint32_t)(e[0] - '0');
#endif
        ws.rayQueue.dt = f->rayDT.p; ws.rayQueue.slot = f->raySlot.p; ws.rayQueue.origin = f->rayOrigin.p; ws.rayQueue.slotStride = f->slotStride; ws.rayQueue.slotMask = f->slotStride - 1u;
        ws.queueCount = f->queueCount.p; ws.capPixelSamples = nPS; ws.capRays = nRays; ws.spill = f->spill.p; ws.overflow = f->overflow.p; ws.overflowCap = f->overflowCap; ws.batchLists = f->batchLists.p; ws.listStride = f->listStride; ws.clk = f->clk.p;
        e = rtrdev::launch_wavefront(s->dev, fb, ws, f->ctx->tun, (int)s->tree.stats.stackEntries, dstats, st, f->ev, (uint32_t)f->ctx->prop.multiProcessorCount);
    } else {
        (void)hipEventRecord(f->evMega[0], st);
        e = rtrdev::launch_megakernel(s->dev, ra, fo, (int)s->tree.stats.stackEntries, dstats, st);
        (void)hipEventRecord(f->evMega[1], st);
    }
    if (e != hipSuccess) return fail(RTR_ERR_HIP, "kernel launch: %s", hipGetErrorString(e));
    f->pendingStats = true;
    f->ownPending = true;
    for (uint32_t b = 1; b < n; ++b) {
        rtr_frame* fr = frames[b];
        if (!fr->evDone) HIP_TRY(hipEventCreateWithFlags(&fr->evDone, hipEventDisableTiming));
        HIP_TRY(hipEventRecord(fr->evDone, st));
        fr->batchStream = st;
        fr->viaBatch = true; fr->pendingStats = false;
        memset(&fr->stats, 0, sizeof fr->stats);
    }
    return RTR_OK;
}

int rtr_render_batch_limit(const rtr_scene* s, const rtr_render_params* pin, uint32_t numAreaLights, uint32_t* maxFrames) {
    if (!s || !pin || !maxFrames) return fail(RTR_ERR_INVALID_ARGUMENT, "rtr_render_batch_limit: null argument");
    if (numAreaLights > s->numLights) return fail(RTR_ERR_INVALID_ARGUMENT, "rtr_render_batch_limit: %u area lights, the scene has %u", numAreaLights, s->numLights);
    rtr_render_params p = *pin;
    if (p.bandRows == 0) p.bandRows = 8;
    if (p.shardCount == 0) p.shardCount = 1;
    if (p.width == 0 || p.height == 0 || p.spp == 0 || p.bandRows % 8u) return fail(RTR_ERR_INVALID_ARGUMENT, "rtr_render_batch_limit: bad width/height/spp/bandRows");
    *maxFrames = 1;
    if (p.pipeline == 1) return RTR_OK;
    uint64_t maxRays = 1;
    for (uint32_t l = 0; l < numAreaLights; ++l) maxRays += (uint64_t)s->hostLights[l].numTriangles * p.numShadowRays;
    const uint32_t rows = rtr_shard_rows(p.height, p.bandRows, p.shardCount);
    const uint64_t blocks = ((uint64_t)((rows + 7u) / 8u) * ((p.width + 7u) / 8u) * 64u + 255u) / 256u;
    for (uint32_t n = rtrdev::kMaxBatch; n > 1; --n) {
        const uint64_t nPS = blocks * 256u * p.spp * n;
        uint64_t slotStride = 256;
        while (slotStride < nPS) slotStride <<= 1;
        if (slotStride * maxRays < (1ull << 31) && maxRays <= 4096 && blocks * n < (1ull << 31)) { *maxFrames = n; break; }
    }
    return RTR_OK;
}

int rtr_render_split_async(rtr_scene* s, const RtrCameraData* cam, const RtrSceneInfo* info, const rtr_render_params* pin, rtr_frame* f, uint32_t parts) {
    if (!s || !cam || !info || !pin || !f) return fail(RTR_ERR_INVALID_ARGUMENT, "rtr_render_split_async: null argument");
    if (parts < 1 || parts > RTR_MAX_SPLIT) return fail(RTR_ERR_INVALID_ARGUMENT, "rtr_render_split_async: %u parts, 1 to %d", parts, RTR_MAX_SPLIT);
    if (pin->shardCount > 1) return fail(RTR_ERR_INVALID_ARGUMENT, "rtr_render_split_async: the frame must be whole (shardCount %u); a shard of a multi-GPU frame is not split again", pin->shardCount);
    if (f->extHdr) return fail(RTR_ERR_INVALID_ARGUMENT, "rtr_render_split_async: not a frame of the caller's");
    rtr_render_params p = *pin;
    if (p.bandRows == 0) p.bandRows = 8;
    if (p.bandRows % 8u) return fail(RTR_ERR_INVALID_ARGUMENT, "rtr_render_split_async: bandRows %u must be a multiple of 8", p.bandRows);
    if (p.height == 0 || p.width == 0) return fail(RTR_ERR_INVALID_ARGUMENT, "rtr_render_split_async: empty frame");
    const uint32_t bands = (p.height + p.bandRows - 1) / p.bandRows;
    if (parts > bands) parts = bands;
    if (parts <= 1) { p.shardIndex = 0; p.shardCount = 1; return enqueue_render(s, cam, info, &p, &f, 1); }
    if (f->width != p.width || f->rows != p.height) return fail(RTR_ERR_INVALID_ARGUMENT, "rtr_render_split_async: frame is %ux%u, the whole frame is %ux%u", f->width, f->rows, p.width, p.height);
    HIP_TRY(hipSetDevice(f->ctx->device));
    hipStream_t st = f->ctx->stream;
    while (f->parts.size() < parts) {
        rtr_ctx* pc = nullptr; rtr_frame* pf = nullptr;
        int rc = ctx_create_prio(f->ctx->device, f->ctx->tun.split_priorities ? (int)f->parts.size() : -1, &pc);
        if (rc != RTR_OK) return rc;
        rc = frame_new(pc, f->width, f->rows, f->images, false, &pf);
        if (rc != RTR_OK) { rtr_ctx_destroy(pc); return rc; }
        hipEvent_t ev = nullptr;
        hipError_t e = hipEventCreateWithFlags(&ev, hipEventDisableTiming);
        if (e != hipSuccess) { rtr_frame_destroy(pf); rtr_ctx_destroy(pc); return fail(RTR_ERR_HIP, "hipEventCreate: %s", hipGetErrorString(e)); }
        f->partCtx.push_back(pc); f->parts.push_back(pf); f->evPart.push_back(ev);
    }
    for (auto& e : f->evSplit) if (!e) HIP_TRY(hipEventCreate(&e));
    if (f->batchStream && f->batchStream != st) HIP_TRY(hipStreamWaitEvent(st, f->evDone, 0));
    f->batchStream = nullptr;
    HIP_TRY(hipEventRecord(f->evSplit[0], st));
    int rc = RTR_OK;
    uint32_t started = 0;
    auto hip_keep = [&](hipError_t e, const char* what) {
        if (e != hipSuccess && rc == RTR_OK) rc = fail(RTR_ERR_HIP, "rtr_render_split_async: %s: %s", what, hipGetErrorString(e));
        return e == hipSuccess;
    };
    for (uint32_t k = 0; k < parts && rc == RTR_OK; ++k) {
        rtr_frame* pf = f->parts[k];
        pf->ctx->tun = f->ctx->tun;
        pf->images = f->images;
        for (int i = 0; i < 8; ++i) pf->ext[i] = f->image_ptr(i);
        pf->extHdr = f->hdr.p;
        hipStream_t ps = pf->ctx->stream;
        if (!hip_keep(hipStreamWaitEvent(ps, f->evSplit[0], 0), "hipStreamWaitEvent (fork)")) break;
        p.shardIndex = k; p.shardCount = parts;
        const int prc = enqueue_render(s, cam, info, &p, &pf, 1, true);
        if (prc != RTR_OK) { rc = prc; break; }
        ++started;
        if (hip_keep(hipEventRecord(f->evPart[k], ps), "hipEventRecord (part)")) hip_keep(hipStreamWaitEvent(st, f->evPart[k], 0), "hipStreamWaitEvent (join)");
        else hip_keep(hipStreamSynchronize(ps), "hipStreamSynchronize (join of last resort)");
    }
    hip_keep(hipEventRecord(f->evSplit[1], st), "hipEventRecord (join)");
    f->ownPending = true; f->viaBatch = false;
    f->pendingSplit = started; f->pendingStats = started != 0;
    return rc;
}

int rtr_render_split(rtr_scene* s, const RtrCameraData* cam, const RtrSceneInfo* info, const rtr_render_params* p, rtr_frame* f, uint32_t parts) {
    int rc = rtr_render_split_async(s, cam, info, p, f, parts);
    if (rc != RTR_OK) return rc;
    return rtr_frame_wait(f);
}

static int wait_split(rtr_frame* f) {
    const uint32_t parts = f->pendingSplit;
    f->pendingSplit = 0; f->pendingStats = false;
    rtr_frame_stats t; memset(&t, 0, sizeof t);
    double clk = 0; uint32_t nclk = 0;
    for (uint32_t k = 0; k < parts; ++k) {
        int rc = rtr_frame_wait(f->parts[k]);
        if (rc != RTR_OK) return rc;
        const rtr_frame_stats& a = f->parts[k]->stats;
        t.numRays += a.numRays; t.numPrimaryRays += a.numPrimaryRays; t.numShadowRays += a.numShadowRays; t.numNodeVisits += a.numNodeVisits;
        t.numTriTests += a.numTriTests; t.numHits += a.numHits; t.numLightFetches += a.numLightFetches; t.numLightTriFetches += a.numLightTriFetches;
        t.numTexFetches += a.numTexFetches; t.numAlphaTests += a.numAlphaTests; t.algorithmicBytes += a.algorithmicBytes;
        t.numShadowNodeVisits += a.numShadowNodeVisits; t.numShadowTriTests += a.numShadowTriTests; t.shadowTraceBytes += a.shadowTraceBytes;
        t.primaryMs += a.primaryMs; t.shadowGenMs += a.shadowGenMs; t.shadowTraceMs += a.shadowTraceMs; t.resolveMs += a.resolveMs; t.shadowTailMs += a.shadowTailMs;
        t.localRows += a.localRows; t.localPixels += a.localPixels; t.pipelineUsed = a.pipelineUsed;
        t.shadowInnerIterations += a.shadowInnerIterations; t.shadowInnerActiveLanes += a.shadowInnerActiveLanes;
        t.shadowTriIterations += a.shadowTriIterations; t.shadowTriActiveLanes += a.shadowTriActiveLanes; t.shadowRefills += a.shadowRefills;
        t.primaryTailRays += a.primaryTailRays; t.shadowTailRays += a.shadowTailRays;
        if (a.shadowTraceClockMHz > 0.f) {
            clk += a.shadowTraceClockMHz; ++nclk;
            t.shadowTraceClockMinMHz = (t.shadowTraceClockMinMHz == 0.f || a.shadowTraceClockMinMHz < t.shadowTraceClockMinMHz) ? a.shadowTraceClockMinMHz : t.shadowTraceClockMinMHz;
            t.shadowTraceClockMaxMHz = a.shadowTraceClockMaxMHz > t.shadowTraceClockMaxMHz ? a.shadowTraceClockMaxMHz : t.shadowTraceClockMaxMHz;
        }
    }
    if (nclk) t.shadowTraceClockMHz = (float)(clk / nclk);
    float ms = 0;
    (void)hipEventElapsedTime(&ms, f->evSplit[0], f->evSplit[1]);
    t.totalMs = ms;
    f->stats = t;
    return RTR_OK;
}

int rtr_frame_wait(rtr_frame* f) {
    if (!f) return fail(RTR_ERR_INVALID_ARGUMENT, "rtr_frame_wait: null frame");
    HIP_TRY(hipSetDevice(f->ctx->device));
    HIP_TRY(hipStreamSynchronize(f->ctx->stream));
    f->ownPending = false;
    if (f->pendingSplit) return wait_split(f);
    if (f->viaBatch) { HIP_TRY(hipEventSynchronize(f->evDone)); f->batchStream = nullptr; return RTR_OK; }
    if (!f->pendingStats) return RTR_OK;
    f->pendingStats = false;
    rtr_frame_stats& s = f->stats;
// ... 819 lines not shown
```

Baseline: 16640.

## Split surface fetch into geometry and material, cache hit geometry between passes

```diff
diff --git a/realtimeraytracer_amd/csrc/kernels/rtr_device.h b/realtimeraytracer_amd/csrc/kernels/rtr_device.h
--- a/realtimeraytracer_amd/csrc/kernels/rtr_device.h
+++ b/realtimeraytracer_amd/csrc/kernels/rtr_device.h
@@ -419,14 +419,13 @@
     float4 t1, t2;
 };
 
-template <bool SHADE, bool STATS>
-__device__ __forceinline__ bool fetch_surface(const DeviceScene& sc, const RenderArgs& ra, const HitRec& h, rtr_v3 rayDir,
-                                              bool wantAnalytic, Accum& o, Surface& sf, LocalStats& st) {
-    if (h.custom == RTR_MISS) {
+template <bool SHADE, bool STATS, class DIR>
+__device__ __forceinline__ bool sample_ends(const DeviceScene& sc, uint32_t custom, DIR rayDir, Accum& o, LocalStats& st) {
+    if (custom == RTR_MISS) {
         if (SHADE) {
             rtr_v3 sky = rtr_ld3(sc.skyLinear);
             if (sc.hdri.pixels) {
-                const rtr_v3 dir = rtr_normalize(rayDir);
+                const rtr_v3 dir = rtr_normalize(rayDir());
                 const float hu = rtr_atan2(dir.z, dir.x) / (2.0f * 3.14159265f) + 0.5f;
                 float hv = rtr_acos(rtr_clamp(dir.y, -1.0f, 1.0f)) / 3.14159265f;
                 hv = 1.0f - hv;
@@ -435,48 +434,78 @@
             }
             o.analytic = rtr_add(o.analytic, sky); o.unshadowed = rtr_add(o.unshadowed, sky); o.shadowed = rtr_add(o.shadowed, sky);
         }
-        return false;
-    }
-    if (h.custom < sc.numLights) {
+        return true;
+    }
+    if (custom < sc.numLights) {
         if (SHADE) {
-            const rtr_v3 lc = rtr_ld3(sc.lights[h.custom].color);
+            const rtr_v3 lc = rtr_ld3(sc.lights[custom].color);
             o.analytic = rtr_add(o.analytic, lc); o.unshadowed = rtr_add(o.unshadowed, lc); o.shadowed = rtr_add(o.shadowed, lc);
         }
-        return false;
-    }
-    const rtr_v3 camPos = rtr_ld3(ra.cam.position);
-    if (STATS) st.hits++;
-    const RtrObjectInfo* oi = sc.objects + (h.custom - sc.numLights);
+        return true;
+    }
+    return false;
+}
+
+struct HitGeom { float4* point; float4* normal; };
+
+struct HitCorners { const float4 *a, *b, *c; float u, v; };
+
+#ifndef RTR_SURF_REFS
+#define RTR_SURF_REFS 0
+#endif
+#ifndef RTR_SURF_RECORD
+#define RTR_SURF_RECORD 0
+#endif
+__device__ __forceinline__ uint4 vertex_refs(const DeviceScene& sc, uint32_t custom, uint32_t prim) {
+    const RtrObjectInfo* oi = sc.objects + (custom - sc.numLights);
     const uint32_t vOff = oi->vertexOffset, iOff = oi->indexOffset;
-    const uint32_t i0 = sc.indices[3u * h.prim + 0u + iOff];
-    const uint32_t i1 = sc.indices[3u * h.prim + 1u + iOff];
-    const uint32_t i2 = sc.indices[3u * h.prim + 2u + iOff];
-    const float4* va = reinterpret_cast<const float4*>(sc.vertices + (i0 + vOff));
-    const float4* vb = reinterpret_cast<const float4*>(sc.vertices + (i1 + vOff));
-    const float4* vc = reinterpret_cast<const float4*>(sc.vertices + (i2 + vOff));
-    const rtr_v3 p0 = f4xyz(va[0]), p1 = f4xyz(vb[0]), p2 = f4xyz(vc[0]);
-    const rtr_v3 n0 = f4xyz(va[1]), n1 = f4xyz(vb[1]), n2 = f4xyz(vc[1]);
-    const float b0 = 1.0f - h.u - h.v, b1 = h.u, b2 = h.v;
+    const uint32_t i0 = sc.indices[3u * prim + 0u + iOff];
+    const uint32_t i1 = sc.indices[3u * prim + 1u + iOff];
+    const uint32_t i2 = sc.indices[3u * prim + 2u + iOff];
+    return make_uint4(i0 + vOff, i1 + vOff, i2 + vOff, 0u);
+}
+__device__ __forceinline__ void store_vertex_refs(const DeviceScene& sc, uint4* hitVerts, size_t k, uint32_t custom, uint32_t prim) {
+    if (!RTR_SURF_REFS) return;
+    if (custom == RTR_MISS || custom < sc.numLights) return;
+    hitVerts[k] = vertex_refs(sc, custom, prim);
+}
+__device__ __forceinline__ HitCorners corners_of(const DeviceScene& sc, uint4 refs, float u, float v) {
+    return HitCorners{reinterpret_cast<const float4*>(sc.vertices + refs.x), reinterpret_cast<const float4*>(sc.vertices + refs.y),
+                      reinterpret_cast<const float4*>(sc.vertices + refs.z), u, v};
+}
+
+template <class DIR>
+__device__ __forceinline__ void surface_geometry(const DeviceScene& sc, uint32_t custom, const HitCorners& c, DIR rayDir, rtr_v3& hitPoint, rtr_v3& hitNormal) {
+    const rtr_v3 p0 = f4xyz(c.a[0]), p1 = f4xyz(c.b[0]), p2 = f4xyz(c.c[0]);
+    const rtr_v3 n0 = f4xyz(c.a[1]), n1 = f4xyz(c.b[1]), n2 = f4xyz(c.c[1]);
+    const float b0 = 1.0f - c.u - c.v, b1 = c.u, b2 = c.v;
     const rtr_v3 localPos = rtr_madd(rtr_madd(rtr_scale(p0, b0), p1, b1), p2, b2);
-    const rtr_v3 hitPoint = rtr_xform_point34(sc.xforms + 12u * h.custom, localPos);
+    hitPoint = rtr_xform_point34(sc.xforms + 12u * custom, localPos);
     const rtr_v3 nsum = rtr_madd(rtr_madd(rtr_scale(n0, b0), n1, b1), n2, b2);
-    const float* nm = sc.nmats + 12u * h.custom;
-    rtr_v3 hitNormal;
+    const float* nm = sc.nmats + 12u * custom;
     if (rtr_dot(nsum, nsum) > 0.0f) {
         hitNormal = rtr_normalize(rtr_mul33(nm, rtr_normalize(nsum)));
     } else {
         const rtr_v3 g = rtr_cross(rtr_sub(p1, p0), rtr_sub(p2, p0));
         rtr_v3 n = rtr_normalize(rtr_mul33(nm, rtr_normalize(g)));
-        if (rtr_dot(n, rayDir) > 0.0f) n = rtr_neg(n);
+        if (rtr_dot(n, rayDir()) > 0.0f) n = rtr_neg(n);
         hitNormal = n;
     }
+}
+
+template <bool SHADE, bool STATS, class CORNERS>
+__device__ __forceinline__ void surface_material(const DeviceScene& sc, const RenderArgs& ra, const RtrObjectInfo* oi, CORNERS corners, rtr_v3 hitPoint, rtr_v3 hitNormal,
+                                                 bool wantAnalytic, Accum& o, Surface& sf, LocalStats& st) {
+    const rtr_v3 camPos = rtr_ld3(ra.cam.position);
     float metallic = oi->metallic;
     float rough = oi->specular;
     rtr_v3 color = rtr_mk(0, 0, 0);
     if (SHADE) {
         rtr_v3 col = rtr_ld3(oi->color);
         if (oi->usesColorMap | oi->usesSpecularMap | oi->usesMetallicMap) {
-            const float4 ta = va[2], tb = vb[2], tc = vc[2];
+            const HitCorners c = corners();
+            const float b0 = 1.0f - c.u - c.v, b1 = c.u, b2 = c.v;
+            const float4 ta = c.a[2], tb = c.b[2], tc = c.c[2];
             const float uu = rtr_fma(tc.x, b2, rtr_fma(tb.x, b1, ta.x * b0));
             const float vv = rtr_fma(tc.y, b2, rtr_fma(tb.y, b1, ta.y * b0));
             if (oi->usesColorMap != 0u) { const float4 t = sample_tex<STATS>(sc.textures[oi->colorIndex], uu, vv, st); col = rtr_mk(t.x, t.y, t.z); }
@@ -508,7 +537,36 @@
     sf.hitPoint = hitPoint; sf.hitNormal = hitNormal; sf.viewDir = viewDir; sf.color = color;
     sf.mDiffuse = mDiffuse; sf.mSpecular = mSpecular; sf.roughness = roughness; sf.metallic = metallic; sf.om = om;
     sf.t1 = t1; sf.t2 = t2;
+}
+
+template <bool SHADE, bool STATS>
+__device__ __forceinline__ bool fetch_surface(const DeviceScene& sc, const RenderArgs& ra, const HitRec& h, rtr_v3 rayDir,
+                                              bool wantAnalytic, Accum& o, Surface& sf, LocalStats& st) {
+    const auto dir = [&] { return rayDir; };
+    if (sample_ends<SHADE, STATS>(sc, h.custom, dir, o, st)) return false;
+    if (STATS) st.hits++;
+    const RtrObjectInfo* oi = sc.objects + (h.custom - sc.numLights);
+    const uint32_t vOff = oi->vertexOffset, iOff = oi->indexOffset;
+    const uint32_t i0 = sc.indices[3u * h.prim + 0u + iOff];
+    const uint32_t i1 = sc.indices[3u * h.prim + 1u + iOff];
+    const uint32_t i2 = sc.indices[3u * h.prim + 2u + iOff];
+    const HitCorners c = corners_of(sc, make_uint4(i0 + vOff, i1 + vOff, i2 + vOff, 0u), h.u, h.v);
+    rtr_v3 hitPoint, hitNormal;
+    surface_geometry(sc, h.custom, c, dir, hitPoint, hitNormal);
+    surface_material<SHADE, STATS>(sc, ra, oi, [&] { return c; }, hitPoint, hitNormal, wantAnalytic, o, sf, st);
     return true;
+}
+
+template <class DIR>
+__device__ __forceinline__ void surface_from_refs(const DeviceScene& sc, uint32_t custom, uint4 refs, float u, float v, DIR rayDir, Surface& sf) {
+    surface_geometry(sc, custom, corners_of(sc, refs, u, v), rayDir, sf.hitPoint, sf.hitNormal);
+}
+
+__device__ __forceinline__ void surface_from_record(const DeviceScene& sc, const RenderArgs& ra, uint32_t custom, size_t k, const float4* __restrict__ hitTuvp,
+                                                    const uint4* __restrict__ hitVerts, const HitGeom& hitGeom, Accum& o, Surface& sf, LocalStats& st) {
+    const float4 g0 = hitGeom.point[k], g1 = hitGeom.normal[k];
+    const auto corners = [&] { const float4 r = hitTuvp[k]; return corners_of(sc, RTR_SURF_REFS ? hitVerts[k] : vertex_refs(sc, custom, __float_as_uint(r.w)), r.y, r.z); };
+    surface_material<true, false>(sc, ra, sc.objects + (custom - sc.numLights), corners, f4xyz(g0), f4xyz(g1), false, o, sf, st);
 }
 
 __device__ __forceinline__ rtr_v3 surface_diffuse(float om, rtr_v3 color) {
diff --git a/realtimeraytracer_amd/csrc/kernels/rtr_kernels.h b/realtimeraytracer_amd/csrc/kernels/rtr_kernels.h
--- a/realtimeraytracer_amd/csrc/kernels/rtr_kernels.h
+++ b/realtimeraytracer_amd/csrc/kernels/rtr_kernels.h
@@ -40,6 +40,8 @@
 struct Workspace {
     float4*   hitTuvp = nullptr;
     uint32_t* hitCustom = nullptr;
+    uint4*    hitVerts = nullptr;
+    HitGeom   hitGeom = {nullptr, nullptr};
     RayQueue  rayQueue;
     uint8_t*  vis = nullptr;
     uint32_t  visFill = 1;
diff --git a/realtimeraytracer_amd/csrc/kernels/rtr_kernels.hip b/realtimeraytracer_amd/csrc/kernels/rtr_kernels.hip
--- a/realtimeraytracer_amd/csrc/kernels/rtr_kernels.hip
+++ b/realtimeraytracer_amd/csrc/kernels/rtr_kernels.hip
@@ -173,7 +173,7 @@
 static_assert(kPrimBlock % 64 == 0 && kPrimBlock >= 64 && kPrimBlock <= kBlock && kBlock % kPrimBlock == 0,
               "RTR_PRIMARY_BLOCK: a multiple of 64 that divides the 256-lane tile group (the launcher's grid is blocks * (kBlock / kPrimBlock))");
 template <int STACK, bool STATS>
-__global__ __launch_bounds__(kPrimBlock) void k_primary(DeviceScene sc, FrameBatch fb, float4* hitTuvp, uint32_t* hitCustom, float4* rayOrigin,
+__global__ __launch_bounds__(kPrimBlock) void k_primary(DeviceScene sc, FrameBatch fb, float4* hitTuvp, uint32_t* hitCustom, uint4* hitVerts, float4* rayOrigin,
                                                     Counters* stats, uint32_t* redoCount, uint32_t* redoList, uint32_t planeBlocks) {
     __shared__ int32_t s_stack[16 * kPrimBlock];
     int32_t* stack = s_stack + threadIdx.x;
@@ -209,12 +209,13 @@
         hitTuvp[k] = make_float4(h.t, h.u, h.v, __uint_as_float(h.prim));
         hitCustom[k] = h.custom;
         origin_leaf_store(rayOrigin, k, h.leaf);
+        store_vertex_refs(sc, hitVerts, k, h.custom, h.prim);
     }
     if (STATS) st.flush(stats);
 }
 
 template <bool STATS>
-__global__ __launch_bounds__(kBlock) void k_primary_packet(DeviceScene sc, FrameBatch fb, float4* hitTuvp, uint32_t* hitCustom, float4* rayOrigin, Counters* stats, uint32_t planeBlocks) {
+__global__ __launch_bounds__(kBlock) void k_primary_packet(DeviceScene sc, FrameBatch fb, float4* hitTuvp, uint32_t* hitCustom, uint4* hitVerts, float4* rayOrigin, Counters* stats, uint32_t planeBlocks) {
     __shared__ uint4 s_stack[kBlock / 64][64];
     const uint32_t wave = threadIdx.x >> 6, lane = threadIdx.x & 63u;
     const uint32_t plane = blockIdx.x / planeBlocks;
@@ -295,12 +296,13 @@
         hitTuvp[k] = make_float4(best.t, best.u, best.v, __uint_as_float(best.prim));
         hitCustom[k] = best.custom;
         origin_leaf_store(rayOrigin, k, best.leaf);
+        store_vertex_refs(sc, hitVerts, k, best.custom, best.prim);
     }
     if (STATS) st.flush(stats);
 }
 
 template <bool STATS>
-__global__ __launch_bounds__(kBlock) void k_primary_tail(DeviceScene sc, FrameBatch fb, float4* hitTuvp, uint32_t* hitCustom, float4* rayOrigin,
+__global__ __launch_bounds__(kBlock) void k_primary_tail(DeviceScene sc, FrameBatch fb, float4* hitTuvp, uint32_t* hitCustom, uint4* hitVerts, float4* rayOrigin,
                                                          const uint32_t* __restrict__ redoCount, const uint32_t* __restrict__ redoList,
                                                          int32_t* __restrict__ spill, uint32_t planeStride, Counters* stats) {
     const uint32_t n = *redoCount;
@@ -320,6 +322,7 @@
         hitTuvp[k] = make_float4(h.t, h.u, h.v, __uint_as_float(h.prim));
         hitCustom[k] = h.custom;
         origin_leaf_store(rayOrigin, k, h.leaf);
+        store_vertex_refs(sc, hitVerts, k, h.custom, h.prim);
     }
     if (STATS) st.flush(stats);
 }
@@ -360,8 +363,27 @@
 };
 
 constexpr uint32_t kGenBlock = 1024;
-__global__ __launch_bounds__(kGenBlock) void k_shadow_gen(DeviceScene sc, FrameBatch fb, const float4* hitTuvp,
-                                                          const uint32_t* hitCustom, RayQueue queue, uint32_t* count, uint32_t planeStride) {
+__device__ __forceinline__ bool gen_surface(const DeviceScene& sc, const RenderArgs& ra, uint32_t px, uint32_t py, uint32_t i, size_t k, const float4* hitTuvp,
+                                            const uint32_t* hitCustom, const uint4* hitVerts, HitGeom hitGeom, Surface& sf) {
+    const float4 r = hitTuvp[k];
+    const uint32_t custom = hitCustom[k];
+    if (custom == RTR_MISS || custom < sc.numLights) return false;
+    surface_from_refs(sc, custom, RTR_SURF_REFS ? hitVerts[k] : vertex_refs(sc, custom, __float_as_uint(r.w)), r.y, r.z, [&] { return primary_dir(ra, px, py, i); }, sf);
+    if (RTR_SURF_RECORD || ra.spp > 1u) {
+        hitGeom.point[k] = make_float4(sf.hitPoint.x, sf.hitPoint.y, sf.hitPoint.z, 0.0f);
+        hitGeom.normal[k] = make_float4(sf.hitNormal.x, sf.hitNormal.y, sf.hitNormal.z, 0.0f);
+    }
+    return true;
+}
+__device__ __forceinline__ bool gen_surface_again(const DeviceScene& sc, size_t k, const uint32_t* hitCustom, HitGeom hitGeom, Surface& sf) {
+    const uint32_t custom = hitCustom[k];
+    if (custom == RTR_MISS || custom < sc.numLights) return false;
+    sf.hitPoint = f4xyz(hitGeom.point[k]); sf.hitNormal = f4xyz(hitGeom.normal[k]);
+    return true;
+}
+
+__global__ __launch_bounds__(kGenBlock) void k_shadow_gen(DeviceScene sc, FrameBatch fb, const float4* hitTuvp, const uint32_t* hitCustom,
+                                                          const uint4* hitVerts, HitGeom hitGeom, RayQueue queue, uint32_t* count, uint32_t planeStride) {
     __shared__ uint32_t s_off[kGenBlock / 64], s_tot[kGenBlock / 64], s_base;
     __shared__ uint32_t s_pairs[2u * kParkedPairs * kGenBlock];
     uint32_t q;
@@ -383,10 +405,8 @@
         smp.draw(ra.numShadowRays);
         for (uint32_t i = 0; i < ra.spp; ++i) {
             const size_t k = (plane0 + i) * planeStride + q;
-            const float4 r = hitTuvp[k];
-            HitRec h; h.t = r.x; h.u = r.y; h.v = r.z; h.prim = __float_as_uint(r.w); h.custom = hitCustom[k];
-            Surface sf;
-            const bool surf = fetch_surface<false, false>(sc, ra, h, primary_dir(ra, px, py, i), false, acc, sf, st);
+            Surface sf = {};
+            const bool surf = gen_surface(sc, ra, px, py, i, k, hitTuvp, hitCustom, hitVerts, hitGeom, sf);
             if (surf) light_loops_from<CountPolicy, false>(sc, ra, smp, sf, 0u, acc, cp, st);
             if (i == 0) { sf0 = sf; surf0 = surf; }
         }
@@ -410,10 +430,8 @@
         if (single) {
             if (surf0) { queue_store_origin(queue, k, sf0.hitPoint, sf0.hitNormal); light_loops_from<EmitPolicy, false>(sc, ra, smp, sf0, 0u, acc, pol, st); }
         } else {
-            const float4 r = hitTuvp[k];
-            HitRec h; h.t = r.x; h.u = r.y; h.v = r.z; h.prim = __float_as_uint(r.w); h.custom = hitCustom[k];
-            Surface sf;
-            if (fetch_surface<false, false>(sc, ra, h, primary_dir(ra, px, py, i), false, acc, sf, st)) {
+            Surface sf = {};
+            if (gen_surface_again(sc, k, hitCustom, hitGeom, sf)) {
                 queue_store_origin(queue, k, sf.hitPoint, sf.hitNormal);
                 light_loops_from<EmitPolicy, false>(sc, ra, smp, sf, 0u, acc, pol, st);
             }
@@ -429,7 +447,7 @@
 constexpr uint32_t kGenOctBlock = RTR_GEN_OCT_BLOCK;
 constexpr uint32_t kParkSurface = 6, kParkWords = kParkSurface + 2u * kParkedPairs;
 #ifndef RTR_GEN_OCT_WAVES
-#define RTR_GEN_OCT_WAVES 7
+#define RTR_GEN_OCT_WAVES 8
 #endif
 #if RTR_GEN_OCT_WAVES > 0
 #define RTR_GEN_OCT_ATTR __attribute__((amdgpu_waves_per_eu(RTR_GEN_OCT_WAVES, 8)))
@@ -437,7 +455,7 @@
 #define RTR_GEN_OCT_ATTR
 #endif
 __global__ __launch_bounds__(kGenOctBlock) RTR_GEN_OCT_ATTR void k_shadow_gen_oct(DeviceScene sc, FrameBatch fb, const float4* hitTuvp, const uint32_t* hitCustom,
-                                                              RayQueue queue, uint32_t* ctrl, uint32_t planeStride, uint2* lists,
+                                                              const uint4* hitVerts, HitGeom hitGeom, RayQueue queue, uint32_t* ctrl, uint32_t planeStride, uint2* lists,
                                                               uint32_t listStride, uint32_t kBatch, uint32_t nt) {
     constexpr uint32_t kWaves = kGenOctBlock / 64;
     __shared__ uint32_t s_tot[kWaves][8], s_run[kWaves][8];
@@ -459,18 +477,8 @@
         smp.draw(ra.numShadowRays);
         for (uint32_t i = 0; i < ra.spp; ++i) {
             const size_t k = (plane0 + i) * planeStride + q;
-            const float4 r = hitTuvp[k];
-            HitRec h; h.t = r.x; h.u = r.y; h.v = r.z; h.prim = __float_as_uint(r.w); h.custom = hitCustom[k];
-            Surface sf;
-            bool surf = fetch_surface<false, false>(sc, ra, h, primary_dir(ra, px, py, i), false, acc, sf, st);
-#if RTR_EXP_DOUBLE_FETCH_GEN
-            if (surf) {
-                HitRec h2 = h; h2.u = h.u + sf.hitPoint.x * (float)(ra.spp - 1u) * 1.0e-30f; h2.v = h.v + sf.hitNormal.y * (float)(ra.spp - 1u) * 1.0e-30f;
-                h2.prim = h.prim + (__float_as_uint(sf.hitPoint.z) == 0x7fc12345u ? 1u : 0u);
-                Surface sf2;
-                if (fetch_surface<false, false>(sc, ra, h2, primary_dir(ra, px, py, i), false, acc, sf2, st)) sf = sf2;
-            }
-#endif
+            Surface sf = {};
+            const bool surf = gen_surface(sc, ra, px, py, i, k, hitTuvp, hitCustom, hitVerts, hitGeom, sf);
             if (surf) {
                 if (single) {
                     park[0u * kGenOctBlock] = __float_as_uint(sf.hitPoint.x); park[1u * kGenOctBlock] = __float_as_uint(sf.hitPoint.y); park[2u * kGenOctBlock] = __float_as_uint(sf.hitPoint.z);
@@ -537,10 +545,8 @@
             queue_store_origin(queue, k, sf0.hitPoint, sf0.hitNormal);
             light_loops_from<EmitOctPolicy, false>(sc, ra, smp, sf0, 0u, acc, pol, st);
         } else {
-            const float4 r = hitTuvp[k];
-            HitRec h; h.t = r.x; h.u = r.y; h.v = r.z; h.prim = __float_as_uint(r.w); h.custom = hitCustom[k];
-            Surface sf;
-            if (fetch_surface<false, false>(sc, ra, h, primary_dir(ra, px, py, i), false, acc, sf, st)) {
+            Surface sf = {};
+            if (gen_surface_again(sc, k, hitCustom, hitGeom, sf)) {
                 queue_store_origin(queue, k, sf.hitPoint, sf.hitNormal);
                 light_loops_from<EmitOctPolicy, false>(sc, ra, smp, sf, 0u, acc, pol, st);
             }
@@ -1090,7 +1096,7 @@
 }
 
 template <bool STATS>
-__global__ __launch_bounds__(kBlock) void k_primary4(DeviceScene sc, FrameBatch fb, float4* hitTuvp, uint32_t* hitCustom, float4* rayOrigin, Counters* stats,
+__global__ __launch_bounds__(kBlock) void k_primary4(DeviceScene sc, FrameBatch fb, float4* hitTuvp, uint32_t* hitCustom, uint4* hitVerts, float4* rayOrigin, Counters* stats,
                                                      uint32_t* redoCount, uint32_t* redoList, uint32_t planeBlocks) {
     __shared__ int32_t s_stack[RTR_WIDE_STACK * kBlock];
     typedef uint32_t u32x4 __attribute__((ext_vector_type(4)));
@@ -1163,7 +1169,7 @@
     }
     const size_t k = (size_t)plane * planeBlocks * kBlock + q;
     if (over) redoList[atomicAdd(redoCount, 1u)] = (uint32_t)k;
-    else { hitTuvp[k] = make_float4(best.t, best.u, best.v, __uint_as_float(best.prim)); hitCustom[k] = best.custom; origin_leaf_store(rayOrigin, k, best.leaf); }
+    else { hitTuvp[k] = make_float4(best.t, best.u, best.v, __uint_as_float(best.prim)); hitCustom[k] = best.custom; origin_leaf_store(rayOrigin, k, best.leaf); store_vertex_refs(sc, hitVerts, k, best.custom, best.prim); }
     if (STATS) st.flush(stats);
 }
 
@@ -1198,7 +1204,7 @@
 }
 
 template <int STACK, bool STATS>
-__global__ __launch_bounds__(kBlock) __attribute__((amdgpu_waves_per_eu(8, 8))) void k_primary_persist(DeviceScene sc, RenderArgs ra, float4* hitTuvp, uint32_t* hitCustom, float4* rayOrigin,
+__global__ __launch_bounds__(kBlock) __attribute__((amdgpu_waves_per_eu(8, 8))) void k_primary_persist(DeviceScene sc, RenderArgs ra, float4* hitTuvp, uint32_t* hitCustom, uint4* hitVerts, float4* rayOrigin,
                                                          Counters* stats, uint32_t* redoCount, uint32_t* redoList, uint32_t* cursors,
                                                          uint32_t planeStride, uint32_t kBatch, uint32_t kRefill, uint32_t kInnerMin) {
     __shared__ int32_t s_stack[(STACK + 1 + 1) * kBlock];
@@ -1228,7 +1234,7 @@
         if (nIdle >= kRefill || nIdle == 64u) {
             if (cur == kDone && res != kResNone) {
                 if (res == 2u) redoList[atomicAdd(redoCount, 1u)] = item;
-                else { hitTuvp[item] = make_float4(best.t, best.u, best.v, __uint_as_float(best.prim)); hitCustom[item] = best.custom; origin_leaf_store(rayOrigin, item, best.leaf); }
+                else { hitTuvp[item] = make_float4(best.t, best.u, best.v, __uint_as_float(best.prim)); hitCustom[item] = best.custom; origin_leaf_store(rayOrigin, item, best.leaf); store_vertex_refs(sc, hitVerts, item, best.custom, best.prim); }
                 res = kResNone;
             }
             if (!exhausted) {
@@ -1378,12 +1384,6 @@
     if (STATS) st.flush(stats);
 }
 
-#ifndef RTR_EXP_DOUBLE_FETCH_GEN
-#define RTR_EXP_DOUBLE_FETCH_GEN 0
-#endif
-#ifndef RTR_EXP_DOUBLE_FETCH
-#define RTR_EXP_DOUBLE_FETCH 0
-#endif
 #ifndef RTR_RESOLVE_CAP
 #define RTR_RESOLVE_CAP 192
 #endif
@@ -1403,7 +1403,7 @@
 
 __global__ __launch_bounds__(kBlock) __attribute__((amdgpu_waves_per_eu(RTR_RESOLVE_COMPACT_WAVES, 8)))
 void k_resolve_compact(DeviceScene sc, FrameBatch fb, uint32_t planeStride, const float4* __restrict__ hitTuvp, const uint32_t* __restrict__ hitCustom,
-                       const uint8_t* __restrict__ vis, uint32_t slotStride) {
+                       const uint4* __restrict__ hitVerts, HitGeom hitGeom, const uint8_t* __restrict__ vis, uint32_t slotStride) {
     constexpr uint32_t kWaves = kBlock / 64;
     __shared__ float4 s_surf[kWaves][4][64];
     __shared__ uint32_t s_item[kWaves][kResolveCap];
@@ -1429,16 +1429,14 @@
         Surface sf;
         sf.hitPoint = sf.hitNormal = rtr_mk(0, 0, 0);
         if (valid) {
+#if RTR_SURF_RECORD
+            const uint32_t custom = hitCustom[k];
+            has = !sample_ends<true, false>(sc, custom, [&] { return primary_dir(ra, px, py, i); }, acc, st);
+            if (has) surface_from_record(sc, ra, custom, k, hitTuvp, hitVerts, hitGeom, acc, sf, st);
+#else
             const float4 r = hitTuvp[k];
             HitRec h; h.t = r.x; h.u = r.y; h.v = r.z; h.prim = __float_as_uint(r.w); h.custom = hitCustom[k];
             has = fetch_surface<true, false>(sc, ra, h, primary_dir(ra, px, py, i), false, acc, sf, st);
-#if RTR_EXP_DOUBLE_FETCH
-            if (has) {
-                HitRec h2 = h; h2.u = h.u + (float)(ra.spp - 1u) * 1.0e-30f; h2.v = h.v + (float)(ra.spp - 1u) * 1.0e-30f;
-                Surface sf2; Accum acc2 = zero_accum();
-                const bool has2 = fetch_surface<true, false>(sc, ra, h2, primary_dir(ra, px, py, i), false, acc2, sf2, st);
-                if (has2 && sf2.roughness == 12345.0f && sf2.hitPoint.x == 4321.0f && sf2.color.y == 777.0f && sf2.viewDir.z == 55.0f && sf2.hitNormal.y == 99.0f) sf = sf2;
-            }
 #endif
         }
         wave_lds_sync();
@@ -1672,20 +1670,20 @@
         const uint32_t pneeded = (uint32_t)(((unsigned long long)planeStride * ra.spp + kBlock - 1) / kBlock);
         if (pblocks > pneeded) pblocks = pneeded;
         if (pblocks == 0) pblocks = 1;
-        if (stats) hipLaunchKernelGGL((k_primary_persist<16, true>), dim3(pblocks), dim3(kBlock), 0, s, sc, fb.ra[0], ws.hitTuvp, ws.hitCustom, ws.rayQueue.origin, stats, ws.queueCount + kPrimaryRedoWord, ws.overflow + 1, ws.queueCount + kPrimaryCursors, planeStride, kPBatch, kPRefill, kPInnerMin);
-        else hipLaunchKernelGGL((k_primary_persist<16, false>), dim3(pblocks), dim3(kBlock), 0, s, sc, fb.ra[0], ws.hitTuvp, ws.hitCustom, ws.rayQueue.origin, stats, ws.queueCount + kPrimaryRedoWord, ws.overflow + 1, ws.queueCount + kPrimaryCursors, planeStride, kPBatch, kPRefill, kPInnerMin);
+        if (stats) hipLaunchKernelGGL((k_primary_persist<16, true>), dim3(pblocks), dim3(kBlock), 0, s, sc, fb.ra[0], ws.hitTuvp, ws.hitCustom, ws.hitVerts, ws.rayQueue.origin, stats, ws.queueCount + kPrimaryRedoWord, ws.overflow + 1, ws.queueCount + kPrimaryCursors, planeStride, kPBatch, kPRefill, kPInnerMin);
+        else hipLaunchKernelGGL((k_primary_persist<16, false>), dim3(pblocks), dim3(kBlock), 0, s, sc, fb.ra[0], ws.hitTuvp, ws.hitCustom, ws.hitVerts, ws.rayQueue.origin, stats, ws.queueCount + kPrimaryRedoWord, ws.overflow + 1, ws.queueCount + kPrimaryCursors, planeStride, kPBatch, kPRefill, kPInnerMin);
     } else if (tun.primary_wide && sc.nodes4) {
-        if (stats) hipLaunchKernelGGL((k_primary4<true>), dim3(blocks * ra.spp * nb), dim3(kBlock), 0, s, sc, fb, ws.hitTuvp, ws.hitCustom, ws.rayQueue.origin, stats, ws.queueCount + kPrimaryRedoWord, ws.overflow + 1, blocks);
-        else hipLaunchKernelGGL((k_primary4<false>), dim3(blocks * ra.spp * nb), dim3(kBlock), 0, s, sc, fb, ws.hitTuvp, ws.hitCustom, ws.rayQueue.origin, stats, ws.queueCount + kPrimaryRedoWord, ws.overflow + 1, blocks);
+        if (stats) hipLaunchKernelGGL((k_primary4<true>), dim3(blocks * ra.spp * nb), dim3(kBlock), 0, s, sc, fb, ws.hitTuvp, ws.hitCustom, ws.hitVerts, ws.rayQueue.origin, stats, ws.queueCount + kPrimaryRedoWord, ws.overflow + 1, blocks);
+        else hipLaunchKernelGGL((k_primary4<false>), dim3(blocks * ra.spp * nb), dim3(kBlock), 0, s, sc, fb, ws.hitTuvp, ws.hitCustom, ws.hitVerts, ws.rayQueue.origin, stats, ws.queueCount + kPrimaryRedoWord, ws.overflow + 1, blocks);
     } else if (tun.primary_packet) {
         packet = true;
-        if (stats) hipLaunchKernelGGL((k_primary_packet<true>), dim3(blocks * ra.spp * nb), dim3(kBlock), 0, s, sc, fb, ws.hitTuvp, ws.hitCustom, ws.rayQueue.origin, stats, blocks);
-        else hipLaunchKernelGGL((k_primary_packet<false>), dim3(blocks * ra.spp * nb), dim3(kBlock), 0, s, sc, fb, ws.hitTuvp, ws.hitCustom, ws.rayQueue.origin, stats, blocks);
-    } else if (stats) hipLaunchKernelGGL((k_primary<STACK, true>), dim3(blocks * (kBlock / kPrimBlock) * ra.spp * nb), dim3(kPrimBlock), 0, s, sc, fb, ws.hitTuvp, ws.hitCustom, ws.rayQueue.origin, stats, ws.queueCount + kPrimaryRedoWord, ws.overflow + 1, blocks * (kBlock / kPrimBlock));
-    else hipLaunchKernelGGL((k_primary<STACK, false>), dim3(blocks * (kBlock / kPrimBlock) * ra.spp * nb), dim3(kPrimBlock), 0, s, sc, fb, ws.hitTuvp, ws.hitCustom, ws.rayQueue.origin, stats, ws.queueCount + kPrimaryRedoWord, ws.overflow + 1, blocks * (kBlock / kPrimBlock));
+        if (stats) hipLaunchKernelGGL((k_primary_packet<true>), dim3(blocks * ra.spp * nb), dim3(kBlock), 0, s, sc, fb, ws.hitTuvp, ws.hitCustom, ws.hitVerts, ws.rayQueue.origin, stats, blocks);
+        else hipLaunchKernelGGL((k_primary_packet<false>), dim3(blocks * ra.spp * nb), dim3(kBlock), 0, s, sc, fb, ws.hitTuvp, ws.hitCustom, ws.hitVerts, ws.rayQueue.origin, stats, blocks);
+    } else if (stats) hipLaunchKernelGGL((k_primary<STACK, true>), dim3(blocks * (kBlock / kPrimBlock) * ra.spp * nb), dim3(kPrimBlock), 0, s, sc, fb, ws.hitTuvp, ws.hitCustom, ws.hitVerts, ws.rayQueue.origin, stats, ws.queueCount + kPrimaryRedoWord, ws.overflow + 1, blocks * (kBlock / kPrimBlock));
+    else hipLaunchKernelGGL((k_primary<STACK, false>), dim3(blocks * (kBlock / kPrimBlock) * ra.spp * nb), dim3(kPrimBlock), 0, s, sc, fb, ws.hitTuvp, ws.hitCustom, ws.hitVerts, ws.rayQueue.origin, stats, ws.queueCount + kPrimaryRedoWord, ws.overflow + 1, blocks * (kBlock / kPrimBlock));
     if (!packet) {
-        if (stats) hipLaunchKernelGGL(k_primary_tail<true>, dim3(kTailBlocks), dim3(kBlock), 0, s, sc, fb, ws.hitTuvp, ws.hitCustom, ws.rayQueue.origin, ws.queueCount + kPrimaryRedoWord, ws.overflow + 1, ws.spill, planeStride, stats);
-        else hipLaunchKernelGGL(k_primary_tail<false>, dim3(kTailBlocks), dim3(kBlock), 0, s, sc, fb, ws.hitTuvp, ws.hitCustom, ws.rayQueue.origin, ws.queueCount + kPrimaryRedoWord, ws.overflow + 1, ws.spill, planeStride, stats);
+        if (stats) hipLaunchKernelGGL(k_primary_tail<true>, dim3(kTailBlocks), dim3(kBlock), 0, s, sc, fb, ws.hitTuvp, ws.hitCustom, ws.hitVerts, ws.rayQueue.origin, ws.queueCount + kPrimaryRedoWord, ws.overflow + 1, ws.spill, planeStride, stats);
+        else hipLaunchKernelGGL(k_primary_tail<false>, dim3(kTailBlocks), dim3(kBlock), 0, s, sc, fb, ws.hitTuvp, ws.hitCustom, ws.hitVerts, ws.rayQueue.origin, ws.queueCount + kPrimaryRedoWord, ws.overflow + 1, ws.spill, planeStride, stats);
     }
     if (ev) hipEventRecord(ev[1], s);
     const uint32_t kBatchEnv = tun.trace_batch;
@@ -1701,8 +1699,8 @@
     const uint32_t kNtQueue = tun.queue_nt;
     RayQueue rq = ws.rayQueue;
     rq.ownLeaf = (wide && tun.trace_own_leaf) ? 1u : 0u;
-    if (binned) hipLaunchKernelGGL(k_shadow_gen_oct, dim3(genOctBlocks), dim3(kGenOctBlock), 0, s, sc, fb, ws.hitTuvp, ws.hitCustom, rq, ws.queueCount, blocks * kBlock, ws.batchLists, ws.listStride, kBatch, kNtQueue >> 1);
-    else hipLaunchKernelGGL(k_shadow_gen, dim3(genBlocks), dim3(kGenBlock), 0, s, sc, fb, ws.hitTuvp, ws.hitCustom, rq, ws.queueCount, blocks * kBlock);
+    if (binned) hipLaunchKernelGGL(k_shadow_gen_oct, dim3(genOctBlocks), dim3(kGenOctBlock), 0, s, sc, fb, ws.hitTuvp, ws.hitCustom, ws.hitVerts, ws.hitGeom, rq, ws.queueCount, blocks * kBlock, ws.batchLists, ws.listStride, kBatch, kNtQueue >> 1);
+    else hipLaunchKernelGGL(k_shadow_gen, dim3(genBlocks), dim3(kGenBlock), 0, s, sc, fb, ws.hitTuvp, ws.hitCustom, ws.hitVerts, ws.hitGeom, rq, ws.queueCount, blocks * kBlock);
     if (ev) hipEventRecord(ev[2], s);
     const size_t maxRays = (size_t)nb * blocks * kBlock * ra.spp * ra.maxRaysPerSample;
     const uint32_t kWgsPerCu = tun.trace_wgs_per_cu;
@@ -1735,7 +1733,7 @@
     const bool full = (ra.images & ~((1u << 1) | (1u << 16))) != 0u;
     const bool compact = !stats && !full && tun.resolve_compact && !rowWaves && ra.numShadowRays >= 1u && ra.numShadowRays <= kResolveMaxSamples &&
                          sc.numLights <= kResolveMaxLights && sc.numLightTris <= kResolveMaxLightTris;
-    if (compact) hipLaunchKernelGGL(k_resolve_compact, dim3(blocks * nb), dim3(kBlock), 0, s, sc, fb, blocks * kBlock, ws.hitTuvp, ws.hitCustom, ws.vis, ws.rayQueue.slotStride);
+    if (compact) hipLaunchKernelGGL(k_resolve_compact, dim3(blocks * nb), dim3(kBlock), 0, s, sc, fb, blocks * kBlock, ws.hitTuvp, ws.hitCustom, ws.hitVerts, ws.hitGeom, ws.vis, ws.rayQueue.slotStride);
     else if (stats) {
         if (full) hipLaunchKernelGGL((k_resolve<true, true>), dim3(blocks * nb), dim3(kBlock), 0, s, sc, fb, blocks * kBlock, ws.hitTuvp, ws.hitCustom, ws.vis, ws.rayQueue.slotStride, stats, rowWaves);
         else hipLaunchKernelGGL((k_resolve<true, false>), dim3(blocks * nb), dim3(kBlock), 0, s, sc, fb, blocks * kBlock, ws.hitTuvp, ws.hitCustom, ws.vis, ws.rayQueue.slotStride, stats, rowWaves);
diff --git a/realtimeraytracer_amd/csrc/rtr_api.cpp b/realtimeraytracer_amd/csrc/rtr_api.cpp
--- a/realtimeraytracer_amd/csrc/rtr_api.cpp
+++ b/realtimeraytracer_amd/csrc/rtr_api.cpp
@@ -213,6 +213,8 @@
     uint32_t slotStride = 0;
     uint32_t visFill = 1;
     DevBuf<uint32_t> hitCustom, queueCount;
+    DevBuf<uint4> hitVerts;
+    DevBuf<float4> hitGeom;
     DevBuf<uint8_t> vis;
     DevBuf<int32_t> spill;
     DevBuf<uint32_t> overflow;
@@ -1781,7 +1783,11 @@
     if (wave) {
         uint64_t ovCap = std::max<uint64_t>(std::max<uint64_t>(nPS, nRays / 16), 1ull << 20);
         if (ovCap > nRays) ovCap = std::max<uint64_t>(nRays, nPS);
-        if (f->hitTuvp.n < nPS) { HIP_TRY(f->hitTuvp.alloc(nPS)); HIP_TRY(f->hitCustom.alloc(nPS)); HIP_TRY(f->rayOrigin.alloc(nPS)); }
+        if (f->hitTuvp.n < nPS || f->hitGeom.n < 2 * nPS) {
+            HIP_TRY(f->hitTuvp.alloc(nPS)); HIP_TRY(f->hitCustom.alloc(nPS)); HIP_TRY(f->rayOrigin.alloc(nPS));
+            if (RTR_SURF_REFS) { HIP_TRY(f->hitVerts.alloc(nPS)); }
+            HIP_TRY(f->hitGeom.alloc(2 * nPS));
+        }
         if (f->vis.n < nSlots) HIP_TRY(f->vis.alloc(nSlots));
         if (f->rayDT.n < nRays) { HIP_TRY(f->rayDT.alloc(nRays)); HIP_TRY(f->raySlot.alloc(nRays)); }
         if (f->overflow.n < ovCap + 1) HIP_TRY(f->overflow.alloc(ovCap + 1));
@@ -1798,7 +1804,7 @@
         if (!f->clk.p) { HIP_TRY(f->clk.alloc(2 * rtrdev::kQueueRegions)); HIP_TRY(hipMemsetAsync(f->clk.p, 0, 2 * rtrdev::kQueueRegions * sizeof(unsigned long long), st)); }
         if (!f->spill.p) HIP_TRY(f->spill.alloc(rtrdev::kSpillInts));
         Workspace ws;
-        ws.hitTuvp = f->hitTuvp.p; ws.hitCustom = f->hitCustom.p; ws.vis = f->vis.p; ws.visFill = f->visFill;
+        ws.hitTuvp = f->hitTuvp.p; ws.hitCustom = f->hitCustom.p; ws.hitVerts = f->hitVerts.p; ws.hitGeom.point = f->hitGeom.p; ws.hitGeom.normal = f->hitGeom.p + nPS; ws.vis = f->vis.p; ws.visFill = f->visFill;
         ws.visPlaneBytes = (size_t)nPS; ws.visPlanes = (uint32_t)maxRays;
 #ifdef RTR_TEST_HOOKS
         if (const char* e = getenv("RTR_TRACE_VIS_FILL")) if ((e[0] == '0' || e[0] == '1') && !e[1]) ws.visFill = (uint32_t)(e[0] - '0');
```

After: 16630. About the same (-0.1%).
